# szellmann/icon-ray-tracing

Hardware: AMD Instinct MI355X
Metric: Mray/s + ms/frame at 1024², R2B07 ICON grid, 1/2/4/8 MI355X vs host CPU (higher is better)
Workload: dtype f32; 1 GPU; C3: R2B07 (1,310,720 cells) x 90 levels, 1024x1024, framing camera --camera 0 0 1.4e7 0 0 0 0 1 0 -fovy 60, 8 consecutive progressive frames (accumID) per step, woodcockTrackingWithAccel, default TF; records=3932160, width=1024, height=1024, transfer_function=default, sampler=user, accel=sphere, parallelism=single GPU, frames_per_launch=8, slot_table_bytes=0

## Files before the change

icon-ray-tracing_amd/csrc/irt_context.h:

```cpp
#pragma once

#include <hip/hip_runtime.h>

#include <cmath>
#include <vector>

#include "irt_internal.h"
#include "irt_kernels.h"

int irt_hip_failed(const char *call, hipError_t e, const char *file, int line);

#define IRT_HIP(call)                                                           \
  do {                                                                          \
    hipError_t e_ = (call);                                                     \
    if (e_ != hipSuccess) return irt_hip_failed(#call, e_, __FILE__, __LINE__); \
  } while (0)

struct LaunchSlot {
  hipEvent_t ev0 = nullptr, ev1 = nullptr;
  hipEvent_t evDone = nullptr;
  bool pending = false;
  bool marked = false;
  bool timed = false;
  bool block = false;
  hipStream_t stream = nullptr;
  long long launch = 0;
  size_t numWG = 0;
  long long costsOf = -1;
};

struct irt_context {
  int device = 0;
  hipStream_t stream = nullptr;
  irt_volume_info info{};
  uint32_t n = 0;
  int G = 0;
  uint4 *d_binHdr = nullptr;
  float4 *d_fat = nullptr;
  float4 *d_blocks = nullptr;
  irt::SlotTable slot;
  bool slotAlways = false;
  bool slotLazy = false;
  bool slotTried = false;
  bool slotSparse = false;
  double tfSamples = 0.0;
  double *d_tfStat = nullptr;
  size_t binEntries = 0;
  uint32_t numSph = 0;
  uint32_t numSphRec = 0;
  float *d_sphR = nullptr;
  uint32_t *d_sphOff = nullptr;
  uint2 *d_sphRec = nullptr;
  uint32_t *d_sphBits = nullptr;
  uint32_t *h_wgCounts = nullptr, *dh_wgCounts = nullptr;
  size_t wgCap = 0;
  bool lastBlock = false;
  bool wgCountsOn = true;
  bool statsOff = false;
  int countersProbe = 0;
  uint32_t *d_probeCounts = nullptr;
  size_t probeCap = 0;
  float4 *d_samples = nullptr;
  size_t sampleCap = 0;
  float *d_srgb = nullptr;
  float *d_valueRanges = nullptr;
  float *d_maxOp = nullptr;
  ushort4 *d_rects = nullptr;
  unsigned long long *d_updStat = nullptr;
  hipEvent_t evUpd = nullptr;
  bool updPending = false;
  bool gridBuilt = false;
  uint32_t *d_meta = nullptr;
  float *d_gridVR = nullptr;
  float *d_gridMaxOp = nullptr;
  uint32_t *d_gridBits = nullptr;
  int wG = 0;
  uint32_t *d_wOff = nullptr, *d_wRec = nullptr;
  float4 *d_wBox = nullptr, *d_wTrig = nullptr;
  size_t numMCs = 0;
  float4 *d_lut = nullptr;
  int lutCap = 0;
  int lutSize = 0;
  float tfLo = 0.f, tfHi = 1.f, opScale = 1.f;
  bool tfSet = false;
  static constexpr int kSlots = 32;
  static constexpr int kDoneEvery = 8;
  LaunchSlot ring[kSlots];
  long long launches = 0;
  static constexpr size_t kWgCountsMax = size_t(1) << 18;
  size_t wgCountsMax = kWgCountsMax;
  unsigned long long *d_counters = nullptr;
  unsigned long long *d_counterBuckets = nullptr;
  unsigned long long *h_counters = nullptr;
  unsigned long long *dh_counters = nullptr;
  hipStream_t lastStream = nullptr;
  int timingEvery = 8;
  float lastMs = 0.f;
  double timedMs = 0.0;
  long long timedLaunches = 0;
  irt_render_stats stats{};
  unsigned long long h_last[16] = {};
  irt_render_stats total{};
  long long totalLaunches = 0;
  size_t bytes = 0;
  const irt::VariantForms *forms = irt::forms_of(irt::kDefaultVariant);
  uint32_t *d_schedOrder = nullptr, *d_schedCost = nullptr;
  uint32_t *h_schedCost = nullptr, *h_schedOrder = nullptr;
  uint32_t schedSplit[2] = {0, 0};
  uint32_t lastNumSplit = 0;
  int splitLg = 2;
  float splitFactor = 1.f;
  bool splitFixed = false;
  int schedBuf = 0;
  long long schedSwitch = 0;
  size_t schedCap = 0;
  bool schedOn = false;
  bool schedFixed = false;
  int coopMaxLg = 0;
  int coopRamp = 1;
  int probeExit = 0;
  uint32_t *wgTrace = nullptr;
  bool chainOn = true;
  uint32_t *d_chainFlag = nullptr;
  size_t chainCap = 0;
  uint32_t chainEpoch = 1;
  uint32_t *h_chainFail = nullptr, *dh_chainFail = nullptr;
  long long chainFailLaunches = 0;
  uint32_t chainSpins = 0;
  int chainWithhold = -1;
  float4 *d_frameCams = nullptr;
  float4 *h_frameCams = nullptr;
  size_t frameCamCap = 0;
  irt::VoidCache voidCache;
  uint32_t *d_voidList = nullptr;
  uint32_t *h_voidList = nullptr;
  size_t voidCap = 0;
  long long voidOnDevice = 0;
  bool voidOnDeviceList = false;
  long long lastVoid = 0;
  long long lastWorkgroups = 0;
  irt::RenderPlan lastPlan{};
  bool queueOn = false;
  uint32_t *d_queue = nullptr;
  int numCU = 0;
  int queuePerCU = 0;
  int lastQueueWG = 0;
  int schedPolicy = 2;
  bool schedOrderValid = false;
  bool schedLastApplied = false;
  long long schedApplied = 0;
  long long schedKey[8] = {};
  long long schedSrc = -1;
  long long schedLastCopy = -1000;
  hipEvent_t evSample = nullptr;
  bool samplePending = false;
  hipStream_t sampleStream = nullptr;
  float *d_sampleTab = nullptr, *h_sampleTab = nullptr;
  size_t sampleTabCap = 0;
  hipEvent_t evSampleTab = nullptr;
  bool sampleTabBusy = false;
  std::vector<irt_overlay *> overlays;
  bool building = false;
  size_t expected = 0, received = 0;
  float bottomMin = INFINITY, bottomMax = -INFINITY;
  bool voids = false;
  bool variantFixed = false;
  irt_icon_cell *d_cells = nullptr;
  float4 *d_trig = nullptr;
  irt::VolumeAcc vacc{};
  size_t numRuns = 0;
  irt_icon_cell last{};
  struct Sphere {
    float r;
    uint32_t rec;
    int32_t nl;
  };
  std::vector<Sphere> sph;
  struct TileTable {
    std::vector<int32_t> ids;
    int32_t *dev;
  };
  std::vector<TileTable> tileTables;
};

template <typename T>
int dalloc(irt_context *c, T **p, size_t count) {
  *p = nullptr;
  if (count == 0) count = 1;
  IRT_HIP(hipMalloc((void **)p, count * sizeof(T)));
  c->bytes += count * sizeof(T);
  return IRT_OK;
}

template <typename T>
int upload(irt_context *c, T **p, const T *src, size_t count) {
  int rc = dalloc(c, p, count);
  if (rc) return rc;
  if (count) IRT_HIP(hipMemcpyAsync(*p, src, count * sizeof(T), hipMemcpyHostToDevice, c->stream));
  return IRT_OK;
}

int update_pending(const char *what);
int ensure_grid(irt_context *c);
hipError_t wait_slot(irt_context *c, int i);
int finish_slot(irt_context *c, int i);
int finish_stats(irt_context *c);
int tile_table(irt_context *c, const int32_t *ids, size_t n, int lo, int total, const int32_t **out);
hipError_t wait_samples(irt_context *c);
void free_sample_state(irt_context *c);
void free_overlays(irt_context *c);

namespace irt {
void frame_args(const irt_context *c, const irt_launch_params *lp, uint32_t *fb, irt_vec4f *accum, RenderArgs &A);
void scene_args(const irt_context *c, int mode, RenderArgs &A);
int sample_check(const irt_context *c, int mode, const char *what);
int sample_begin(irt_context *c, hipStream_t s);
int sample_end(irt_context *c, hipStream_t s);
int sample_tab_reserve(irt_context *c, size_t need);
int sample_tab_upload(irt_context *c, size_t need, hipStream_t s);
}
```

icon-ray-tracing_amd/csrc/irt_debug_hooks.hip:

```cpp

#include <hip/hip_runtime.h>
#include <string.h>

#include <algorithm>

#include "icon_rt_hip_debug.h"
#include "irt_context.h"
#include "irt_device.h"

using namespace irt;

namespace {
__global__ void k_debug_math(const float *a, const float *y, const float *x, int n, float *oa,
                             float *ot) {
  const int i = blockIdx.x * blockDim.x + threadIdx.x;
  if (i >= n) return;
  oa[i] = glibc_asinf(a[i]);
  ot[i] = glibc_atan2f(y[i], x[i]);
}
}

extern "C" int irt_debug_device_math(int device, const float *a, const float *y, const float *x,
                                     int n, float *oa, float *ot) {
  if (n <= 0 || !a || !y || !x || !oa || !ot) {
// ... 128 lines not shown

extern "C" int irt_debug_device_srgb(int device, const float *x, uint32_t *out, int n) {
  if (!x || !out || n < 0) {
    set_error("irt_debug_device_srgb: bad argument");
    return IRT_E_INVALID;
  }
  IRT_HIP(hipSetDevice(device));
  float th[256];
  srgb_thresholds(th);
  float *d = nullptr;
  const size_t m = 256 + 2 * (size_t)n;
  IRT_HIP(hipMalloc((void **)&d, m * sizeof(float)));
  hipError_t e = hipMemcpy(d, th, sizeof(th), hipMemcpyHostToDevice);
  e = e == hipSuccess ? hipMemcpy(d + 256, x, n * sizeof(float), hipMemcpyHostToDevice) : e;
  if (e == hipSuccess && n > 0) {
    hipLaunchKernelGGL(k_debug_srgb, dim3((n + 255) / 256), dim3(256), 0, 0, d, d + 256,
                       reinterpret_cast<uint32_t *>(d + 256 + n), n);
    e = hipGetLastError();
  }
  e = e == hipSuccess ? hipMemcpy(out, d + 256 + n, n * sizeof(uint32_t), hipMemcpyDeviceToHost) : e;
  (void)hipFree(d);
  if (e != hipSuccess) {
    set_error("irt_debug_device_srgb: %s", hipGetErrorString(e));
    return IRT_E_HIP;
  }
  return IRT_OK;
}

static int debug_locate(irt_context *c, const float *xyz, int n, int *found, float *value, bool wave) {
  if (!c || !xyz || !found || !value || n < 0) {
    set_error("irt_debug_locate: bad argument");
    return IRT_E_INVALID;
  }
  IRT_HIP(hipSetDevice(c->device));
  RenderArgs A;
  memset(&A, 0, sizeof(A));
  A.numCells = c->n;
  A.G = c->G;
  A.binHdr = c->d_binHdr;
  A.fat = c->d_fat;
  A.blocks = c->d_blocks;
  A.slots = c->slot.slots;
  A.slotBins = c->slot.bins;
  A.slotSubs = c->slot.subs;
  for (int k = 0; k < 3; ++k) A.slotEdge[k] = c->slot.edges[k];
  A.numSph = c->numSph;
  A.sphR = c->d_sphR;
  A.sphOff = c->d_sphOff;
  A.sphRec = c->d_sphRec;
  A.sphBits = c->d_sphBits;
  float *d = nullptr;
  IRT_HIP(hipMalloc((void **)&d, (size_t)std::max(n, 1) * 5 * sizeof(float)));
  hipError_t e = hipMemcpy(d, xyz, (size_t)n * 3 * sizeof(float), hipMemcpyHostToDevice);
  int *dFound = reinterpret_cast<int *>(d + 3 * (size_t)n);
  float *dValue = d + 4 * (size_t)n;
  if (e == hipSuccess) {
    launch_debug_locate(A, d, n, dFound, dValue, 0, wave);
    e = hipGetLastError();
  }
  e = e == hipSuccess ? hipMemcpy(found, dFound, (size_t)n * sizeof(int), hipMemcpyDeviceToHost) : e;
  e = e == hipSuccess ? hipMemcpy(value, dValue, (size_t)n * sizeof(float), hipMemcpyDeviceToHost) : e;
  (void)hipFree(d);
  if (e != hipSuccess) {
    set_error("irt_debug_locate: %s", hipGetErrorString(e));
    return IRT_E_HIP;
  }
  return IRT_OK;
}

extern "C" int irt_debug_locate(irt_context *c, const float *xyz, int n, int *found, float *value) {
  return debug_locate(c, xyz, n, found, value, false);
}

extern "C" int irt_debug_locate_wave(irt_context *c, const float *xyz, int n, int *found, float *value) {
  return debug_locate(c, xyz, n, found, value, true);
}

extern "C" int irt_debug_locate_sampler(irt_context *c, int mode, const float *xyz, int n, int *found,
                                        float *value) {
  if (!c || c->building || n < 0 || (n && (!xyz || !found || !value))) {
    set_error("irt_debug_locate_sampler: bad argument");
    return IRT_E_INVALID;
  }
  if (mode != IRT_MODE_CUBQL && mode != IRT_MODE_TRIANGLES) {
    set_error("irt_debug_locate_sampler: sampler mode %d is neither IRT_MODE_CUBQL nor IRT_MODE_TRIANGLES", mode);
    return IRT_E_INVALID;
  }
  if (c->updPending) return update_pending("irt_debug_locate_sampler");
  if (c->wG == 0 && c->n != 0) {
    set_error("irt_debug_locate_sampler: sampler mode %d needs irt_build_wedge_accel first", mode);
    return IRT_E_INVALID;
  }
  if (n == 0) return IRT_OK;
  IRT_HIP(hipSetDevice(c->device));
  RenderArgs A;
  memset(&A, 0, sizeof(A));
  A.numCells = c->n;
  A.sampler = mode;
  A.wG = c->wG;
  A.wOff = c->d_wOff;
  A.wRec = c->d_wRec;
  A.wBox = c->d_wBox;
  A.wTrig = c->d_wTrig;
  A.blocks = c->d_blocks;
  float *d = nullptr;
  IRT_HIP(hipMalloc((void **)&d, (size_t)n * 5 * sizeof(float)));
  hipError_t e = hipMemcpy(d, xyz, (size_t)n * 3 * sizeof(float), hipMemcpyHostToDevice);
  int *dFound = reinterpret_cast<int *>(d + 3 * (size_t)n);
  float *dValue = d + 4 * (size_t)n;
  if (e == hipSuccess) {
    launch_debug_locate_sampler(A, d, n, dFound, dValue, 0);
    e = hipGetLastError();
  }
  e = e == hipSuccess ? hipMemcpy(found, dFound, (size_t)n * sizeof(int), hipMemcpyDeviceToHost) : e;
  e = e == hipSuccess ? hipMemcpy(value, dValue, (size_t)n * sizeof(float), hipMemcpyDeviceToHost) : e;
  (void)hipFree(d);
  if (e != hipSuccess) {
    set_error("irt_debug_locate_sampler: %s", hipGetErrorString(e));
    return IRT_E_HIP;
  }
  return IRT_OK;
}

extern "C" int irt_debug_sched(irt_context *c, int *policy, int *lastApplied, long long *applied) {
  if (!c || !policy || !lastApplied || !applied) {
    set_error("irt_debug_sched: null argument");
    return IRT_E_INVALID;
  }
  *policy = c->schedOn ? c->schedPolicy : 0;
  *lastApplied = c->schedLastApplied ? 1 : 0;
  *applied = c->schedApplied;
  return IRT_OK;
}

extern "C" int irt_debug_counters(irt_context *c, unsigned long long *out16) {
  if (!c || !out16) {
    set_error("irt_debug_counters: null argument");
    return IRT_E_INVALID;
  }
  int rc = finish_stats(c);
  if (rc) return rc;
  memcpy(out16, c->h_last, 16 * sizeof(unsigned long long));
  return IRT_OK;
}

extern "C" int irt_debug_default_variant(void) { return kDefaultVariant; }
extern "C" int irt_debug_slot_use(const irt_context *c, double *tfSamples) {
  if (!c) return -1;
  if (tfSamples) *tfSamples = c->tfSamples;
  return c->slot.slots && (c->slotAlways || c->slotSparse) ? 1 : 0;
}

extern "C" long long irt_debug_void_use(const irt_context *c) { return c ? c->lastVoid : -1; }
extern "C" long long irt_debug_last_workgroups(const irt_context *c) { return c ? c->lastWorkgroups : -1; }

extern "C" int irt_debug_context_array(const irt_context *c, int which, void *dst, size_t capacity,
                                       size_t *bytes) {
  if (!c || !bytes || c->building) {
    set_error("irt_debug_context_array: null argument or context not built");
    return IRT_E_INVALID;
  }
  const void *src = nullptr;
  size_t n = 0;
  switch (which) {
    case IRT_DEBUG_ARRAY_BIN_HDR: src = c->d_binHdr; n = (size_t)6 * c->G * c->G * kBinHdrWords * 4; break;
    case IRT_DEBUG_ARRAY_FAT: src = c->d_fat; n = c->binEntries * kFatStride4 * 16; break;
    case IRT_DEBUG_ARRAY_BLOCKS: src = c->d_blocks; n = (size_t)c->n * kBlk4 * 16; break;
    case IRT_DEBUG_ARRAY_SPH_R: src = c->d_sphR; n = (size_t)c->numSph * 4; break;
    case IRT_DEBUG_ARRAY_SPH_OFF: src = c->d_sphOff; n = c->numSph ? ((size_t)c->numSph + 1) * 4 : 4; break;
    case IRT_DEBUG_ARRAY_SPH_REC: src = c->d_sphRec; n = (size_t)c->numSphRec * 8; break;
    case IRT_DEBUG_ARRAY_SPH_BITS: src = c->d_sphBits; n = (size_t)kSphBitWords * 4; break;
    case IRT_DEBUG_ARRAY_SLOTS: src = c->slot.slots; n = c->slot.bytes; break;
    case IRT_DEBUG_ARRAY_GRID_BITS: src = c->d_gridBits; n = c->gridBuilt ? (size_t)kGridBitWords * 4 : 0; break;
    default:
      set_error("irt_debug_context_array: unknown array %d", which);
      return IRT_E_INVALID;
  }
  *bytes = n;
  if (dst && capacity >= n && n) {
    IRT_HIP(hipSetDevice(c->device));
    IRT_HIP(hipStreamSynchronize(c->stream));
    IRT_HIP(hipMemcpy(dst, src, n, hipMemcpyDeviceToHost));
  }
  return IRT_OK;
}

extern "C" int irt_debug_get_variant(const irt_context *c) { return c ? c->forms->variant : -1; }

extern "C" int irt_debug_variants(int *out, int capacity) { return render_variants(out, capacity); }

extern "C" int irt_debug_set_queue(irt_context *c, int on) {
  if (!c) {
    set_error("irt_debug_set_queue: null context");
    return IRT_E_INVALID;
  }
  if (on && !render_queue_compiled()) {
    set_error("irt_debug_set_queue: persistent launches are compiled into the A/B library only "
              "(make VARIANTS=all, libicon_rt_hip_all.so)");
    return IRT_E_INVALID;
  }
  c->queueOn = on != 0;
  return IRT_OK;
}

extern "C" int irt_debug_set_wg_trace(irt_context *c, uint32_t *trace) {
  if (!c) {
    set_error("irt_debug_set_wg_trace: null context");
    return IRT_E_INVALID;
  }
  c->wgTrace = trace;
  return IRT_OK;
}

extern "C" long long irt_debug_launch_workgroups(const irt_context *c, int numTiles, int numFrames) {
  if (!c || numTiles < 0 || numFrames < 1) {
    set_error("irt_debug_launch_workgroups: bad argument");
    return -1;
  }
  return irt_debug_variant_workgroups(c->forms->variant, c->schedOn ? 1 : 0, numTiles, numFrames);
}

extern "C" long long irt_debug_variant_workgroups(int variant, int sched, int numTiles, int numFrames) {
  if (numTiles < 0 || numFrames < 1) {
    set_error("irt_debug_variant_workgroups: bad argument");
    return -1;
  }
  const int per = 256 / render_forms(variant).plain.threads;
  const size_t extra = sched && numFrames == 1 && per == 4 ? (size_t)kMaxSplit : 0;
  return (long long)((size_t)numTiles * 16 * per * numFrames + extra);
}

namespace {
int plan_out(const RenderPlan &P, int out[5]) {
  out[0] = P.form.id;
  out[1] = P.form.threads;
  out[2] = (int)P.grid.x;
  out[3] = (int)P.grid.y;
  out[4] = P.accumBlocks;
  return IRT_OK;
}
}

extern "C" int irt_debug_plan(int variant, int sampler, int accelMode, int flags, int numTiles, int numFrames,
                              uint32_t numSplit, uint32_t voidLive, uint32_t voidRow, int queueWG, int out[5]) {
  const VariantForms *F = forms_of(variant);
  if (!F || !out || numTiles < 0 || numFrames < 1) {
    set_error("irt_debug_plan: variant %d not compiled, or bad argument", variant);
    return IRT_E_INVALID;
  }
  alignas(16) static uint32_t set[4];
  RenderArgs A;
  memset(&A, 0, sizeof(A));
  A.sampler = sampler;
  A.accelMode = accelMode;
  A.numTiles = numTiles;
  A.numSamples = numFrames;
  A.numSplit = numSplit;
  A.voidLive = voidLive;
  A.voidRow = voidRow;
  if (flags & IRT_DEBUG_PLAN_SLOTS) A.slots = reinterpret_cast<const float4 *>(set);
  if (flags & IRT_DEBUG_PLAN_VOID_BITS) A.voidBits = set;
  if (flags & IRT_DEBUG_PLAN_VOID_LIST) A.voidList = set;
  if (flags & IRT_DEBUG_PLAN_QUEUE) A.queue = set;
  A.chain = (flags & IRT_DEBUG_PLAN_CHAIN) ? 1 : 0;
  return plan_out(plan_render(*F, A, queueWG), out);
}

extern "C" int irt_debug_last_plan(const irt_context *c, int out[5]) {
  if (!c || !out) {
    set_error("irt_debug_last_plan: null argument");
    return IRT_E_INVALID;
  }
  return plan_out(c->lastPlan, out);
}

extern "C" int irt_debug_sched_split(const irt_context *c, int *numSplit, int *splitLg) {
  if (!c || !numSplit || !splitLg) {
    set_error("irt_debug_sched_split: null argument");
    return IRT_E_INVALID;
  }
  *numSplit = (int)c->lastNumSplit;
  *splitLg = c->splitLg;
  return IRT_OK;
}

extern "C" int irt_debug_set_chain(irt_context *c, int on) {
  if (!c) {
    set_error("irt_debug_set_chain: null context");
    return IRT_E_INVALID;
  }
  c->chainOn = on != 0;
  return IRT_OK;
}

extern "C" int irt_debug_chain_errors(irt_context *c) {
  if (!c) {
    set_error("irt_debug_chain_errors: null context");
    return -1;
  }
  for (long long j = c->launches - irt_context::kSlots; j < c->launches; ++j) {
    if (j < 0) continue;
    const int rc = finish_slot(c, (int)(j % irt_context::kSlots));
    if (rc && rc != IRT_E_CHAIN) return -1;
  }
  return (int)c->chainFailLaunches;
}
// ... 25 lines not shown
```

icon-ray-tracing_amd/csrc/irt_device.h:

```cpp
#pragma once

#include <hip/hip_runtime.h>
#include <stdint.h>

#include "irt_common.h"
#include "irt_kernels.h"

#define IRT_FLT_MAX 3.402823466e+38f

namespace irt {

struct Ray {
  float ox, oy, oz, tmin, dx, dy, dz, tmax;
};

struct Counts {
  uint32_t inBox, locate, found, cand;
  uint32_t steps, deg, rounds;
  uint32_t hops, locRounds, candHist[4];
};

__device__ __forceinline__ int opaque_u(int v) {
  v = __builtin_amdgcn_readfirstlane(v);
  asm volatile("" : "+s"(v));
  return v;
}
__device__ __forceinline__ float opaque_u(float v) { return __builtin_bit_cast(float, opaque_u(__builtin_bit_cast(int, v))); }
__device__ __forceinline__ float dot3(float ax, float ay, float az, float bx, float by, float bz) {
  return ax * bx + ay * by + az * bz;
}

__device__ __forceinline__ bool recip_ok(float b) {
  const float ab = __builtin_fabsf(b);
  return ab >= 0x1p-100f && ab <= 0x1p100f;
}
__device__ __forceinline__ double recip_d(float b) {
  const double r0 = (double)__builtin_amdgcn_rcpf(b);
  const double e = __builtin_fma(-(double)b, r0, 1.0);
  return __builtin_fma(r0, __builtin_fma(e, e, e), r0);
}
__device__ __forceinline__ float div_recip(float a, double r) { return (float)((double)a * r); }

__device__ __forceinline__ bool box_test(const Ray &r, const RenderArgs &A, float &t0, float &t1) {
  float lx, ly, lz, hx, hy, hz;
  if (recip_ok(r.dx) && recip_ok(r.dy) && recip_ok(r.dz)) {
    const double rx = recip_d(r.dx), ry = recip_d(r.dy), rz = recip_d(r.dz);
    lx = div_recip(A.bmin.x - r.ox, rx);
    ly = div_recip(A.bmin.y - r.oy, ry);
    lz = div_recip(A.bmin.z - r.oz, rz);
    hx = div_recip(A.bmax.x - r.ox, rx);
    hy = div_recip(A.bmax.y - r.oy, ry);
    hz = div_recip(A.bmax.z - r.oz, rz);
  } else {
    lx = (A.bmin.x - r.ox) / r.dx, ly = (A.bmin.y - r.oy) / r.dy, lz = (A.bmin.z - r.oz) / r.dz;
    hx = (A.bmax.x - r.ox) / r.dx, hy = (A.bmax.y - r.oy) / r.dy, hz = (A.bmax.z - r.oz) / r.dz;
  }
  const float nx = fminf(lx, hx), ny = fminf(ly, hy), nz = fminf(lz, hz);
  const float fx = fmaxf(lx, hx), fy = fmaxf(ly, hy), fz = fmaxf(lz, hz);
  t0 = fmaxf(r.tmin, fmaxf(fmaxf(nx, ny), nz));
  t1 = fminf(r.tmax, fminf(fminf(fx, fy), fz));
  return t0 < t1;
}

__device__ __forceinline__ bool intersect_sphere(const Ray &r, float radius, float &tnear, float &tfar) {
  const float A = dot3(r.dx, r.dy, r.dz, r.dx, r.dy, r.dz);
  const float B = dot3(r.dx, r.dy, r.dz, r.ox, r.oy, r.oz) * 2.f;
  const float C = dot3(r.ox, r.oy, r.oz, r.ox, r.oy, r.oz) - radius * radius;
  float d = B * B - 4.f * A * C;
  if (d < 0.f) return false;
  d = sqrtf(d);
  const float q = B < 0.f ? -0.5f * (B - d) : -0.5f * (B + d);
  const float t1 = q / A;
  const float t2 = C / q;
  tnear = fminf(t1, t2);
  tfar = fmaxf(t1, t2);
  return true;
}
__device__ __forceinline__ void intersect_spheres(const Ray &r, float radiusA, float radiusB, bool &hitA,
                                                  float &nearA, float &farA, bool &hitB, float &nearB,
                                                  float &farB) {
  const float A = dot3(r.dx, r.dy, r.dz, r.dx, r.dy, r.dz);
  const float B = dot3(r.dx, r.dy, r.dz, r.ox, r.oy, r.oz) * 2.f;
  const float OO = dot3(r.ox, r.oy, r.oz, r.ox, r.oy, r.oz);
  const bool okA = recip_ok(A);
  const double rA = okA ? recip_d(A) : 0.0;
  auto one = [&](float radius, float &tnear, float &tfar) {
    const float C = OO - radius * radius;
    float d = B * B - 4.f * A * C;
    if (d < 0.f) return false;
    d = sqrtf(d);
    const float q = B < 0.f ? -0.5f * (B - d) : -0.5f * (B + d);
    float t1, t2;
    if (okA && recip_ok(q)) {
      t1 = div_recip(q, rA);
      t2 = div_recip(C, recip_d(q));
    } else {
      t1 = q / A;
      t2 = C / q;
    }
    tnear = fminf(t1, t2);
    tfar = fmaxf(t1, t2);
    return true;
  };
  hitA = one(radiusA, nearA, farA);
  hitB = one(radiusB, nearB, farB);
}

__device__ __forceinline__ int project_axis(float s, float lo, float hi, int dim) {
  return f2i_x86((s - lo) / (hi - lo) * (float)(dim - 1));
}

__device__ __forceinline__ float div_uniform(float a, double invB) {
  return (float)((double)a * invB);
}
__device__ __forceinline__ int project_axis_inv(float s, float lo, double invSize, int dim) {
  return f2i_x86(div_uniform(s - lo, invSize) * (float)(opaque_u(dim) - 1));
}

__device__ __forceinline__ int wrap_coord(int c, int d) {
  if ((unsigned)c < (unsigned)d) return c;
  if (c >= -d && c < 2 * d) return c < 0 ? c + d : c - d;
  d = opaque_u(d);
  const int m = c % d;
  return m < 0 ? m + d : m;
}

__device__ __forceinline__ void to_spherical(float x, float y, float z, float &r, float &lat,
                                             float &lon) {
  r = sqrtf(dot3(x, y, z, x, y, z));
  lat = glibc_asinf(z / r);
  lon = glibc_atan2f(y, x);
}

constexpr float kLatErr = 1.0e-6f;
constexpr float kLonErr = 2.0e-6f;

__device__ __forceinline__ float fast_asin(float x) {
  const float a = __builtin_fabsf(x);
  const bool big = a >= 0.5f;
  const float t = big ? (1.f - a) * 0.5f : a * a;
  const float s = big ? __builtin_amdgcn_sqrtf(t) : a;
  const float p = t * __builtin_fmaf(
                          t, __builtin_fmaf(t, __builtin_fmaf(t, __builtin_fmaf(t, 4.216630880e-2f, 2.417951451e-2f),
                                                                4.547037598e-2f),
                                            7.495297643e-2f),
                          1.666675248e-1f);
  const float r = __builtin_fmaf(s, p, s);
  const float v = big ? __builtin_fmaf(-2.f, r, 1.57079637050628662109375f) : r;
  return __builtin_copysignf(v, x);
}
__device__ __forceinline__ float fast_atan(float q) {
  const bool big = q > 2.414213562373095f, mid = q > 0.4142135623730950f;
  const float num = big ? -1.f : (mid ? q - 1.f : q);
  const float den = big ? q : (mid ? q + 1.f : 1.f);
  const float x = num * __builtin_amdgcn_rcpf(den);
  const float base = big ? 1.57079637050628662109375f : (mid ? 0.785398185253143310546875f : 0.f);
  const float z = x * x;
  const float p = __builtin_fmaf(
      __builtin_fmaf(__builtin_fmaf(__builtin_fmaf(8.05374449538e-2f, z, -1.38776856032e-1f), z, 1.99777106478e-1f),
                     z, -3.33329491539e-1f),
      z * x, x);
  return base + p;
}
__device__ __forceinline__ bool fast_atan2(float y, float x, float &lon) {
  const float ax = __builtin_fabsf(x), ay = __builtin_fabsf(y);
  const float q = ay * __builtin_amdgcn_rcpf(ax);
  const bool ok = ax >= 0x1p-100f && ax <= 0x1p100f && ay >= 0x1p-100f && ay <= 0x1p100f && q >= 0x1p-58f &&
                  q <= 0x1p58f;
  const float z = fast_atan(q);
  const float pi = 3.1415927410e+00f, pi_lo = -8.7422776573e-08f;
  lon = y < 0.f ? (x < 0.f ? (z - pi_lo) - pi : -z) : (x < 0.f ? pi - (z - pi_lo) : z);
  return ok;
}
__device__ __forceinline__ bool cell_certified(float v, float err, float lo, double invSize, int dim, int &cell) {
  const int c0 = project_axis_inv(v - err, lo, invSize, dim), c1 = project_axis_inv(v + err, lo, invSize, dim);
  cell = c0;
  return c0 == c1 && v == v;
}
__device__ __forceinline__ int sign_certified(float a, float b, float err) {
  const float d = b - a, m = 2.f * err + 2.4e-7f;
  return d > m ? 1 : (-d > m ? -1 : 0);
}

__device__ __forceinline__ uint32_t make_8bit(float f) {
  return (uint32_t)fminf(255.f, fmaxf(0.f, (float)f2i_x86(f * 256.f)));
}

__device__ __forceinline__ uint32_t srgb_byte(const float *th, float x) {
  const float over = th[0];
  const float s = x <= 0.0031308f
                      ? 12.92f * x
                      : 1.055f * __builtin_amdgcn_exp2f(__builtin_amdgcn_logf(x) * (1.f / 2.4f)) - 0.055f;
  int b = (int)fminf(255.f, fmaxf(0.f, s * 256.f));
  const float up = th[b < 255 ? b + 1 : 255], at = th[b];
  if (b < 255 && up <= x) {
    ++b;
    while (b < 255 && th[b + 1] <= x) ++b;
  } else if (b > 0 && !(at <= x)) {
    --b;
    while (b > 0 && !(th[b] <= x)) --b;
  }
  return x >= over ? 0u : (uint32_t)b;
}

}
```

icon-ray-tracing_amd/csrc/irt_internal.h:

```cpp
#pragma once

#include <stddef.h>
#include <stdint.h>

#include <string>
#include <vector>

#include "icon_rt_hip.h"
#include "irt_common.h"

namespace irt {

void set_error(const char *fmt, ...) __attribute__((format(printf, 1, 2)));
void clear_error();


struct HostScene {
  size_t n = 0;
  irt_volume_info info{};
  std::vector<float> hv;
  std::vector<float> trig;
  std::vector<float> planes;
  std::vector<float> rng;
  std::vector<uint32_t> meta;
  std::vector<float> blocks;
  int G = 0;
  std::vector<uint32_t> offsets;
  std::vector<uint32_t> entryRec;
  std::vector<uint32_t> entrySub;
  std::vector<uint32_t> binHdr;
  std::vector<float> fat;
  size_t binEntries = 0;
  std::vector<float> sphR;
  std::vector<uint32_t> sphOff, sphRec, sphBits;
};

int build_bins(HostScene &S, int threads);
int locator_resolution(size_t numRuns);
float record_value_host(const HostScene &s, uint32_t rec, uint32_t path, float r);
int locate_bins_host(const HostScene &s, float px, float py, float pz, float &value,
                     uint32_t *record, uint32_t *tested);

int build_scene(const irt_icon_cell *cells, size_t n, HostScene &out, int threads = 0);


void compute_volume_info(const irt_icon_cell *cells, size_t n, irt_volume_info &info);
struct VolumeAcc {
  float vlo[3], vhi[3], slo[3], shi[3], dlo, dhi;
  size_t n;
};
void corner_trig(const irt_icon_cell &c, float *t12);
void cell_bounds(const irt_icon_cell &c, const float *t12, float lo[3], float hi[3]);
void volume_acc_init(VolumeAcc &a);
void volume_acc_add(VolumeAcc &a, const irt_icon_cell &c, const float blo[3], const float bhi[3]);
void volume_acc_merge(VolumeAcc &a, const VolumeAcc &b);
void volume_acc_finish(const VolumeAcc &a, irt_volume_info &info);

const std::vector<float> &logf_table();

void srgb_thresholds(float th[256]);

int sample_host(const HostScene &s, uint32_t rec, float px, float py, float pz, float &value);
int locate_host(const HostScene &s, float px, float py, float pz, float &value,
                uint32_t *record);

struct WedgeScene {
  int G = 0;
  std::vector<float> trig;
  std::vector<float> box;
  std::vector<uint32_t> offsets;
  std::vector<uint32_t> recs;
};
int build_wedges(const irt_icon_cell *cells, size_t n, WedgeScene &W, int threads = 0);
bool wedge_locate_host(const WedgeScene &W, const irt_icon_cell *cells, float px, float py,
                       float pz, float &value);
bool triangle_locate_host(const WedgeScene &W, const irt_icon_cell *cells, float px, float py,
                          float pz, float &value, uint32_t *record);

int default_threads();

inline bool update_range_ok(size_t first, size_t n, size_t numCells) {
  return first <= numCells && n <= numCells - first;
}

constexpr uint64_t kSampleMaxPoints = uint64_t(1) << 36;
void latlon_trig(const float *lat, int numLat, const float *lon, int numLon, float *latCS, float *lonCS);
int latlon_args(const char *what, const float *lat, int numLat, const float *lon, int numLon,
                const float *radius, int numLevels, size_t *total);

int levels_args(const char *what, const float *radius, int numLevels);
void levels_order(const float *radius, int numLevels, float *sorted, int32_t *index);

int column_weights(const char *what, const float *weight, int numLevels);
int column_levels_args(const char *what, const float *radius, const float *weight, int numLevels);

constexpr size_t kSectionTrigSplit = 1 << 14;
void section_trig(const float *lat, const float *lon, int numColumns, float *tab);
int section_args(const char *what, const float *lat, const float *lon, int numColumns, const float *radius,
                 int numLevels, size_t *total);

int hist_args(const char *what, irt_box1f valueRange, int numBins, int weighting, const float *bandEdges,
              int numBands);

uint32_t sched_order(const uint32_t *cost, int numBlocks, int tilesX, int tileStride, int policy,
                     int splitLg, float splitFactor, int numCU, bool wavewg, size_t cap,
                     uint32_t maxSplit, uint32_t *out);

struct VoidRequest {
  float cam[12];
  float bmin[3], bmax[3];
  float rOuter, rInner;
  int W, H, tileBegin, tileStride, numTiles;
  int raygen, accelMode, mode;
  const int32_t *tileList;
};
inline VoidRequest void_request(const irt_launch_params &lp, const irt_volume_info &info, int W, int H, int tileBegin,
                                int tileStride, int numTiles, const int32_t *tileList) {
  VoidRequest q;
  const irt_vec3f *cam[4] = {&lp.org, &lp.dir_00, &lp.dir_du, &lp.dir_dv};
  for (int k = 0; k < 4; ++k) {
    q.cam[3 * k] = cam[k]->x;
    q.cam[3 * k + 1] = cam[k]->y;
    q.cam[3 * k + 2] = cam[k]->z;
  }
  q.bmin[0] = info.bounds.lower.x, q.bmin[1] = info.bounds.lower.y, q.bmin[2] = info.bounds.lower.z;
  q.bmax[0] = info.bounds.upper.x, q.bmax[1] = info.bounds.upper.y, q.bmax[2] = info.bounds.upper.z;
  q.rOuter = info.sphericalBounds.upper.x;
  q.rInner = info.sphericalBounds.lower.x;
  q.W = W, q.H = H, q.tileBegin = tileBegin, q.tileStride = tileStride, q.numTiles = numTiles;
  q.raygen = lp.raygen, q.accelMode = lp.accelMode, q.mode = lp.mode;
  q.tileList = tileList;
  return q;
}
inline size_t void_words(int numTiles) { return ((size_t)(numTiles > 0 ? numTiles : 0) * 64 + 31) / 32; }
struct VoidLists {
  std::vector<uint32_t> items;
  uint32_t live = 0, count = 0;
};
constexpr uint32_t kVoidEmpty = ~0u;
inline uint32_t void_row(uint32_t count, int F) {
  return (uint32_t)((((uint64_t)count + (uint64_t)F - 1) / (uint64_t)F + 7) & ~(uint64_t)7);
}
uint32_t void_packets(const VoidRequest &q, uint32_t *bits, VoidLists *lists = nullptr);
struct VoidCache {
  std::vector<unsigned char> key;
  std::vector<uint32_t> bits;
  VoidLists lists;
  uint32_t count = 0;
  bool keyed = false, valid = false;
  long long generation = 0;
  bool lookup(const VoidRequest &q, bool defer = false);
};

int synth_open(int rootN, int bisections, int levels, float topHeight, float noise, uint32_t seed,
               float terrainHeight,
               void **gen, size_t *total);
void synth_fill(const void *gen, size_t first, size_t count, irt_icon_cell *out);
void synth_close(void *gen);

}
```

icon-ray-tracing_amd/csrc/irt_kernels.h:

```cpp
#pragma once

#include <hip/hip_runtime.h>
#include <stdint.h>

#include "icon_rt_hip.h"

namespace irt {

struct RenderArgs {
  float3 org, dir00, du, dv;
  int accumID;
  float accumW;
  float3 amb;
  float ambRad;
  float unitDistance;
  int raygen;
  float3 bmin, bmax;
  int3 dims;
  float3 sbLo, sbHi;
  const float *maxOp;
  int accelMode;
  const float *gridMaxOp;
  const uint32_t *gridBits;
  int sampler;
  int wG;
  const uint32_t *wOff, *wRec;
  const float4 *wBox;
  const float4 *wTrig;
  float tfLo, tfHi, opacityScale;
  double invTf;
  double invSb[3];
  const float4 *lut;
  int lutSize;
  uint32_t numCells;
  int G;
  const float *srgbTh;
  int W, H;
  uint32_t *fb;
  float4 *accum;
  int packed;
  int tileBegin, tileStride, numTiles, tilesX;
  const int32_t *tileList;
  unsigned long long *counters;
  unsigned long long *counterBuckets;
  const uint4 *binHdr;
  const float4 *fat;
  const float4 *blocks;
  uint32_t numSph;
  const float *sphR;
  const uint32_t *sphOff;
  const uint2 *sphRec;
  const uint32_t *sphBits;
  uint32_t *wgCounts;
  int numSamples;
  const uint32_t *schedOrder;
  uint32_t *schedCost;
  float4 *sampleBuf;
  int coopMaxLg;
  int coopRamp;
  int probeExit;
  uint32_t *queue;
  uint32_t numPackets;
  int chain;
  const float4 *frameCams;
  uint32_t chainEpoch;
  uint32_t *chainFlag;
  uint32_t *chainFail;
  uint32_t chainSpins;
  int chainWithhold;

  uint32_t *wgTrace;
  const uint32_t *splitList;
  const uint32_t *splitMask;
  uint32_t numSplit;
  const float4 *slots;
  float slotEdge[3];
  int slotBins;
  int slotSubs;
  const uint32_t *voidBits;
  const uint32_t *voidList;
  uint32_t voidLive, voidRow, voidCount;
};
constexpr int kQueueLine = 32;
constexpr uint32_t kChainSpinsDefault = 1u << 20;
constexpr int kQueueWords = 9 * kQueueLine;

constexpr int kCnt = 8;

enum : int {
  OPT_WEDGE = 16384,
  OPT_GRID = 8192,
  OPT_STATS = 32768,
  OPT_SERIAL = 65536,
  OPT_SCAN1 = 131072,
  OPT_TIMING = 524288,
  OPT_WAVEWG = 4194304,
  OPT_LEAN = 2097152,
  OPT_QUEUE = 16777216,
  OPT_FASTSPH = 33554432,
  OPT_SPLIT = 8,
  OPT_DPPSCAN = 32,
  OPT_DMATAB = 67108864,
  OPT_NOMISS = 262144,
  OPT_VOIDLOC = 1073741824,
  OPT_NOVOIDRUN = 2,
  OPT_NOHOLESKIP = 4,
  OPT_SLOT = 128,
  OPT_VOID = 16,
  OPT_VLIST = 64,
};
constexpr int OPT_MONO = 4096;
constexpr int kDefaultVariant = 73405728;
constexpr int kNoMissBit = OPT_NOMISS;
constexpr uint32_t kMaxSplit = 4096;
constexpr int kVoidLocBit = OPT_VOIDLOC;
constexpr int kSamplerVariant = ((kDefaultVariant & ~OPT_MONO) & ~(0xF00 | OPT_WAVEWG | OPT_LEAN)) | OPT_WEDGE;
inline int scene_variant(bool holes) { return holes ? kDefaultVariant | kVoidLocBit : kDefaultVariant | kNoMissBit; }

typedef void (*RenderKernel)(RenderArgs);
struct KernelForm {
  RenderKernel fn;
  int id;
  int threads;
};
struct VariantForms {
  int variant;
  KernelForm plain, split, slot, slotSplit, voidBits, voidList, queue;
  KernelForm grid, wedge, wedgeGrid;
};
const VariantForms *forms_of(int variant);
inline const VariantForms &render_forms(int variant) {
  const VariantForms *f = forms_of(variant);
  return f ? *f : *forms_of(kDefaultVariant);
}
int render_variants(int *out, int cap);
bool render_queue_compiled();

inline bool render_sphere_path(const RenderArgs &A) {
  return A.sampler == IRT_MODE_USER_GEOM && A.accelMode != IRT_ACCEL_GRID;
}
inline bool render_split_ok(const VariantForms &F, const RenderArgs &A) {
  return render_sphere_path(A) && F.split.fn != nullptr;
}
inline bool render_void_ok(const VariantForms &F, const RenderArgs &A) {
  return render_sphere_path(A) && F.voidBits.fn != nullptr && !A.slots && !A.queue && !A.numSplit && !A.schedOrder;
}
inline bool render_queue_ok(const VariantForms &F, const RenderArgs &A) {
  return render_sphere_path(A) && F.queue.fn != nullptr;
}
int render_queue_wgs(const VariantForms &F, int numCU, int numBlocks);

struct RenderPlan {
  KernelForm form;
  dim3 grid;
  size_t workgroups;
  int accumBlocks;
};
RenderPlan plan_render(const VariantForms &F, const RenderArgs &A, int queueWG);
void launch_render(const RenderArgs &A, const RenderPlan &plan, hipStream_t s);
void prewarm_render(const VariantForms &F, hipStream_t s);
void launch_debug_locate(const RenderArgs &A, const float *xyz, int n, int *found, float *value,
                         hipStream_t s, bool wave);
void launch_debug_locate_sampler(const RenderArgs &A, const float *xyz, int n, int *found, float *value,
                                 hipStream_t s);
void launch_shell_init(float *valueRanges, size_t numMCs, hipStream_t s);
void launch_shell_build(const irt_icon_cell *cells, size_t n, int3 dims, float3 lo, float3 hi,
                        float *valueRanges, ushort4 *rects, hipStream_t s);
void launch_value_scatter(const float *d_values, size_t first, size_t n, float4 *blocks, hipStream_t s);
void launch_shell_rebuild(const float4 *blocks, const uint32_t *meta, const ushort4 *rects, size_t n,
                          int3 dims, float *valueRanges, unsigned long long *stat, hipStream_t s);
void launch_grid_build(const float4 *blocks, const uint32_t *meta, const float4 *trig, size_t n,
                       float3 lo, float3 hi, float *valueRanges, hipStream_t s);
void launch_grid_bits(const float *maxOp, uint32_t *bits, hipStream_t s);
void launch_accept_stat(const float *valueRanges, const float *maxOp, size_t numMCs, const float4 *lut, int size,
                        float lo, float hi, double *out, hipStream_t s);
void launch_max_opacities(const float *valueRanges, size_t numMCs, const float4 *lut, int size,
                          float lo, float hi, float *maxOp, hipStream_t s);
void launch_clear(uint32_t *fb, float4 *accum, size_t n, hipStream_t s);
constexpr int kCounterBuckets = 64;
void launch_stats_out(const unsigned long long *cur, unsigned long long *host,
                      unsigned long long *next, unsigned long long *buckets, hipStream_t s);
void launch_copy_u32(const uint32_t *src, uint32_t *dst, size_t n, hipStream_t s);
struct DeviceScene {
  float4 *blocks = nullptr;
  uint32_t *meta = nullptr;
  uint4 *binHdr = nullptr;
  float4 *fat = nullptr;
  size_t entries = 0, binEntries = 0, bigCells = 0, bytes = 0;
};
int build_scene_device(const irt_icon_cell *d_cells, const float4 *d_trig, size_t n, size_t numRuns,
                       int G, hipStream_t s, DeviceScene &out);
struct SlotTable {
  float4 *slots = nullptr;
  int bins = 0;
  int subs = 0;
  float edges[3] = {0.f, 0.f, 0.f};
  size_t bytes = 0;
  const char *skipped = nullptr;
};
constexpr size_t kSlotAutoHdrBytes = (size_t)256 << 20;
int build_slots_device(const uint32_t *hdr, const float4 *fat, uint32_t numCells, size_t maxBytes, int subs,
                       size_t autoBytes, hipStream_t s, SlotTable &out);
void launch_unpack(const uint32_t *gathered, int numRanks, int maxTiles, int W, int H,
                   uint32_t *fb, hipStream_t s, const int32_t *table = nullptr);

}
```

icon-ray-tracing_amd/csrc/irt_launch.hip:

```cpp

#include <hip/hip_runtime.h>
#include <string.h>

#include <algorithm>
#include <initializer_list>

#include "irt_context.h"

using namespace irt;


int tile_table(irt_context *c, const int32_t *ids, size_t n, int lo, int total, const int32_t **out) {
  for (size_t k = 0; k < n; ++k)
    if (ids[k] < lo || ids[k] >= total) {
      set_error("tile id %d at %zu outside [%d, %d)", ids[k], k, lo, total);
      return IRT_E_INVALID;
    }
  for (auto &t : c->tileTables)
    if (t.ids.size() == n && std::equal(t.ids.begin(), t.ids.end(), ids)) {
      *out = t.dev;
      return IRT_OK;
    }
  if (c->tileTables.size() >= 64) {
    IRT_HIP(hipDeviceSynchronize());
// ... 340 lines not shown
                         I.sphericalBounds.upper.z - I.sphericalBounds.lower.z};
    for (int k = 0; k < 3; ++k) A.invSb[k] = 1.0 / (double)sz[k];
  }
  A.coopMaxLg = c->coopMaxLg;
  A.coopRamp = c->coopRamp;
  A.probeExit = c->probeExit;
  A.wgTrace = c->wgTrace;
  A.numCells = c->n;
  A.G = c->G;
  A.counters = c->d_counters + 16 * L.slot;
  A.binHdr = c->d_binHdr;
  A.fat = c->d_fat;
  A.blocks = c->d_blocks;
  A.slots = c->slotAlways || c->slotSparse ? c->slot.slots : nullptr;
  A.slotBins = c->slot.bins;
  A.slotSubs = c->slot.subs;
  for (int k = 0; k < 3; ++k) A.slotEdge[k] = c->slot.edges[k];
  A.numSph = c->numSph;
  A.sphR = c->d_sphR;
  A.sphOff = c->d_sphOff;
  A.sphRec = c->d_sphRec;
  A.sphBits = c->d_sphBits;
}

int claim_slot(irt_context *c, Launch &L) {
  for (int i = 0; i < kSlots; ++i)
    if (c->ring[i].pending && c->h_chainFail[i]) {
      int rc = finish_slot(c, i);
      if (rc) return rc;
    }
  if (c->ring[L.slot].pending) {
    int rc = finish_slot(c, L.slot);
    if (rc) return rc;
  }
  hipStream_t s = L.s;
  if (c->launches > 0 && s != c->lastStream) {
    const int prev = (int)((c->launches - 1) % kSlots);
    if (c->ring[prev].pending) {
      const hipEvent_t e = done_event(c, prev);
      if (e) IRT_HIP(hipStreamWaitEvent(s, e, 0));
    }
  }
  c->lastStream = s;
  return IRT_OK;
}

void decide_queue(irt_context *c, int numFrames, Launch &L) {
  RenderArgs &A = L.A;
  L.queued = c->queueOn && L.numTiles > 0 && whole_kernel(c) && render_queue_ok(*c->forms, A);
  L.queueWG = 0;
  if (!L.queued) return;
  A.queue = c->d_queue + (size_t)kQueueWords * L.slot;
  A.numPackets = (uint32_t)L.numTiles * 64u * (uint32_t)numFrames;
  L.queueWG = c->queuePerCU > 0 ? std::min(c->queuePerCU * c->numCU, L.numTiles * 16 * numFrames)
                                : render_queue_wgs(*c->forms, c->numCU, L.numTiles * 16 * numFrames);
  c->lastQueueWG = L.queueWG;
}

int decide_sched(irt_context *c, const irt_launch_params *lp, const RenderRequest &r, Launch &L) {
  RenderArgs &A = L.A;
  const int numBlocks = L.numTiles * 16;
  L.copyCosts = false;
  if (!(c->schedOn && r.numFrames == 1 && numBlocks > 0 && !A.tileList && !L.queued)) return IRT_OK;
  int rc = sched_prepare(c, numBlocks, r.W, r.H, r.packed, r.tileBegin, r.tileStride, L.numTiles, lp,
                         render_split_ok(*c->forms, A), L.s);
  if (rc) return rc;
  const uint32_t *ob = c->d_schedOrder + (size_t)c->schedBuf * sched_stride(c->schedCap);
  A.schedOrder = c->schedOrderValid ? ob : nullptr;
  if (c->schedOrderValid && c->schedSplit[c->schedBuf] && render_split_ok(*c->forms, A) && whole_kernel(c)) {
    A.splitList = ob + c->schedCap;
    A.splitMask = ob + c->schedCap + kMaxSplit;
    A.numSplit = c->schedSplit[c->schedBuf];
  }
  L.copyCosts = c->launches - c->schedLastCopy >= 8;
  if (L.copyCosts) {
    uint32_t *dh = nullptr;
    IRT_HIP(hipHostGetDevicePointer((void **)&dh, c->h_schedCost + (size_t)L.slot * 4 * c->schedCap, 0));
    A.schedCost = dh;
  } else {
    A.schedCost = c->d_schedCost;
  }
  return IRT_OK;
}

void decide_chain(const irt_context *c, const RenderRequest &r, Launch &L) {
  RenderArgs &A = L.A;
  const uint64_t outPixels = r.packed ? (uint64_t)L.numTiles * 4096u : (uint64_t)r.W * (uint64_t)r.H;
  A.chain = r.numFrames > 1 && chain_capable(c, L.queued) && outPixels * 16u <= 0x7FFFFFFFull ? 1 : 0;
  A.numSamples = r.numFrames;
}

int choose_counters(irt_context *c, Launch &L) {
  RenderArgs &A = L.A;
  const bool useWG = c->wgCountsOn && L.numWG <= c->wgCountsMax;
  if (useWG && L.numWG > c->wgCap) {
    bool failed = false;
    int rc = grow(c, Retire::Slots, L.s, &c->wgCap, L.numWG,
                  {{(void **)&c->h_wgCounts, [](size_t n) { return n * kSlots * kCnt * sizeof(uint32_t); }, true}},
                  &failed);
    if (rc) return rc;
    if (!failed && hipHostGetDevicePointer((void **)&c->dh_wgCounts, c->h_wgCounts, 0) != hipSuccess) {
      (void)hipGetLastError();
      (void)hipHostFree(c->h_wgCounts);
      c->h_wgCounts = nullptr;
      c->wgCap = 0;
      failed = true;
    }
    if (failed) {
      c->dh_wgCounts = nullptr;
      c->wgCountsOn = false;
    }
  }
  A.wgCounts = useWG && c->wgCountsOn ? c->dh_wgCounts + (size_t)L.slot * c->wgCap * kCnt : nullptr;
  if (c->countersProbe == 1 || c->statsOff) {
    A.wgCounts = nullptr;
    if (!stats_variant(c)) A.counters = nullptr;
  } else if (c->countersProbe == 2) {
    if (L.numWG > c->probeCap) {
      int rc = grow(c, Retire::Stream, L.s, &c->probeCap, L.numWG,
                    {{(void **)&c->d_probeCounts, [](size_t n) { return n * kCnt * sizeof(uint32_t); }, false}}, nullptr);
      if (rc) return rc;
    }
    A.wgCounts = c->d_probeCounts;
  }
  return IRT_OK;
}

int setup_chain(irt_context *c, int numFrames, Launch &L) {
  RenderArgs &A = L.A;
  if (!A.chain) return IRT_OK;
  const size_t words = (size_t)L.numTiles * 16 * 4;
  if (words > c->chainCap || c->chainEpoch > 0xF0000000u - (uint32_t)numFrames) {
    if (words > c->chainCap) {
      int rc = grow(c, Retire::SlotsThenStream, L.s, &c->chainCap, words,
                    {{(void **)&c->d_chainFlag, [](size_t n) { return n * sizeof(uint32_t); }, false}}, nullptr);
      if (rc) return rc;
    }
    IRT_HIP(hipMemsetAsync(c->d_chainFlag, 0, c->chainCap * sizeof(uint32_t), L.s));
    c->chainEpoch = 1;
  }
  A.chainFlag = c->d_chainFlag;
  c->h_chainFail[L.slot] = 0;
  A.chainFail = c->dh_chainFail + L.slot;
  A.chainSpins = c->chainSpins ? c->chainSpins : kChainSpinsDefault;
  A.chainWithhold = c->chainWithhold;
  A.chainEpoch = c->chainEpoch;
  c->chainEpoch += (uint32_t)numFrames;
  return IRT_OK;
}

int prepare_void(irt_context *c, const irt_launch_params *lp, const RenderRequest &r, Launch &L) {
  RenderArgs &A = L.A;
  c->lastVoid = 0;
  if (!(A.chain && !r.seq && r.numFrames > 1 && r.numFrames <= 65535 && L.numTiles > 0 &&
        c->chainWithhold < 0 && c->probeExit == 0 && !stats_variant(c) &&
        lp->raygen == IRT_RAYGEN_WITH_ACCEL && lp->accelMode == IRT_ACCEL_SPHERE &&
        render_void_ok(*c->forms, A)))
    return IRT_OK;
  c->voidCache.lookup(void_request(*lp, c->info, r.W, r.H, r.tileBegin, r.tileStride, L.numTiles, r.tileList), true);
  const VoidLists &vl = c->voidCache.lists;
  if (!c->voidCache.count || vl.items.empty()) return IRT_OK;
  const bool list = c->forms->voidList.fn != nullptr &&
                    (size_t)vl.live + void_row(vl.count, r.numFrames) < (size_t)L.numTiles * 64;
  const size_t words = list ? vl.items.size() : void_words(L.numTiles);
  if (words > c->voidCap) {
    int rc = grow(c, Retire::SlotsThenStream, L.s, &c->voidCap, words,
                  {{(void **)&c->d_voidList, [](size_t n) { return n * sizeof(uint32_t); }, false},
                   {(void **)&c->h_voidList, [](size_t n) { return kSlots * n * sizeof(uint32_t); }, true}},
                  nullptr);
    c->voidOnDevice = 0;
    if (rc) return rc;
  }
  if (c->voidOnDevice != c->voidCache.generation || c->voidOnDeviceList != list) {
    uint32_t *h = c->h_voidList + (size_t)L.slot * c->voidCap;
    memcpy(h, list ? vl.items.data() : c->voidCache.bits.data(), words * sizeof(uint32_t));
    c->voidOnDeviceList = list;
    IRT_HIP(hipMemcpyAsync(c->d_voidList, h, words * sizeof(uint32_t), hipMemcpyHostToDevice, L.s));
    c->voidOnDevice = c->voidCache.generation;
  }
  if (list) {
    A.voidList = c->d_voidList;
    A.voidLive = vl.live;
    A.voidRow = void_row(vl.count, r.numFrames);
    A.voidCount = vl.count;
  } else {
    A.voidBits = c->d_voidList;
  }
  c->lastVoid = c->voidCache.count;
  return IRT_OK;
}

int stage_sequence(irt_context *c, const RenderRequest &r, Launch &L) {
  RenderArgs &A = L.A;
  if (!r.seq) return IRT_OK;
  if (!A.chain) {
    set_error("irt_render_sequence: needs chained frames (a cooperative variant, IRT_CHAIN on)");
    return IRT_E_INVALID;
  }
  const int numFrames = r.numFrames;
  if ((size_t)numFrames > c->frameCamCap) {
    int rc = grow(c, Retire::SlotsThenStream, L.s, &c->frameCamCap, (size_t)numFrames,
                  {{(void **)&c->d_frameCams, [](size_t n) { return n * 4 * sizeof(float4); }, false},
                   {(void **)&c->h_frameCams, [](size_t n) { return kSlots * n * 4 * sizeof(float4); }, true}},
                  nullptr);
    if (rc) return rc;
  }
  float4 *h = c->h_frameCams + (size_t)L.slot * c->frameCamCap * 4;
  for (int k = 0; k < numFrames; ++k) {
    const irt_launch_params &q = r.seq[k];
    h[4 * k + 0] = make_float4(q.org.x, q.org.y, q.org.z, __builtin_bit_cast(float, q.accumID));
    h[4 * k + 1] = make_float4(q.dir_00.x, q.dir_00.y, q.dir_00.z, 0.f);
    h[4 * k + 2] = make_float4(q.dir_du.x, q.dir_du.y, q.dir_du.z, 0.f);
    h[4 * k + 3] = make_float4(q.dir_dv.x, q.dir_dv.y, q.dir_dv.z, 0.f);
  }
  IRT_HIP(hipMemcpyAsync(c->d_frameCams, h, (size_t)numFrames * 4 * sizeof(float4), hipMemcpyHostToDevice, L.s));
  A.frameCams = c->d_frameCams;
  return IRT_OK;
}

int ensure_samples(irt_context *c, int numFrames, Launch &L) {
  if (numFrames > 1 && !L.A.chain) {
    const size_t need = (size_t)L.numTiles * 4096 * (size_t)numFrames;
    if (need > c->sampleCap) {
      int rc = grow(c, Retire::Stream, L.s, &c->sampleCap, need,
                    {{(void **)&c->d_samples, [](size_t n) { return n * sizeof(float4); }, false}}, nullptr);
      if (rc) return rc;
    }
  }
  L.A.sampleBuf = c->d_samples;
  return IRT_OK;
}

int launch_and_commit(irt_context *c, Launch &L) {
  RenderArgs &A = L.A;
  hipStream_t s = L.s;
  LaunchSlot &r = c->ring[L.slot];
  c->schedLastApplied = A.schedOrder != nullptr;
  c->lastNumSplit = A.numSplit;
  c->lastWorkgroups = L.numTiles > 0 ? (long long)L.numWG : 0;
  c->lastPlan = L.plan;
  c->schedApplied += c->schedLastApplied ? 1 : 0;
  A.counterBuckets = A.counters && !A.wgCounts ? c->d_counterBuckets + (size_t)L.slot * kCounterBuckets * 8 : nullptr;
  const bool block = A.counters && (!A.wgCounts || stats_variant(c));
  if (block && !c->lastBlock) IRT_HIP(hipMemsetAsync(A.counters, 0, 16 * sizeof(unsigned long long), s));
  r.timed = c->launches % c->timingEvery == 0;
  if (r.timed) IRT_HIP(hipEventRecord(r.ev0, s));
  if (L.numTiles > 0) launch_render(A, L.plan, s);
  IRT_HIP(hipGetLastError());
  if (r.timed) IRT_HIP(hipEventRecord(r.ev1, s));
  if (block) {
    launch_stats_out(A.counters, c->dh_counters + 16 * L.slot,
                     c->d_counters + 16 * ((c->launches + 1) % kSlots), A.counterBuckets, s);
    IRT_HIP(hipGetLastError());
  }
  r.block = block;
  c->lastBlock = block;
  r.numWG = (A.wgCounts && c->countersProbe == 0 && !c->statsOff && L.numTiles > 0) ? L.numWG : 0;
  r.costsOf = -1;
  if (L.copyCosts) {
    r.costsOf = c->launches;
    c->schedLastCopy = c->launches;
  }
  r.stream = s;
  r.launch = c->launches;
  r.marked = c->launches % irt_context::kDoneEvery == irt_context::kDoneEvery - 1 || L.copyCosts;
  if (r.marked) IRT_HIP(hipEventRecord(r.evDone, s));
  r.pending = true;
  ++c->launches;
  return IRT_OK;
}

int render_impl(irt_context *c, const irt_launch_params *lp, const RenderRequest &r, uint32_t *fb,
                irt_vec4f *accum, int *numTilesOut, void *stream) {
  int rc = validate(c, lp, r, fb, accum);
  if (rc) return rc;
  IRT_HIP(hipSetDevice(c->device));
  if (lp->accelMode == IRT_ACCEL_GRID && (rc = ensure_grid(c))) return rc;
  Launch L;
  memset(&L.A, 0, sizeof(L.A));
  L.s = (hipStream_t)stream;
  L.slot = (int)(c->launches % kSlots);
  if ((rc = resolve_tiles(c, r, L))) return rc;
  if (numTilesOut) *numTilesOut = L.numTiles;
  fill_args(c, lp, fb, accum, L);
  if ((rc = claim_slot(c, L))) return rc;
  decide_queue(c, r.numFrames, L);
  if ((rc = decide_sched(c, lp, r, L))) return rc;
  decide_chain(c, r, L);
  if ((rc = prepare_void(c, lp, r, L))) return rc;
  L.plan = plan_render(*c->forms, L.A, L.queueWG);
  L.numWG = L.plan.workgroups;
  if ((rc = choose_counters(c, L)) || (rc = setup_chain(c, r.numFrames, L)) ||
      (rc = stage_sequence(c, r, L)) ||
      (rc = ensure_samples(c, r.numFrames, L)))
    return rc;
  return launch_and_commit(c, L);
}

RenderRequest whole_frame(int W, int H, int numFrames) { return {W, H, 0, 0, 1, nullptr, 0, numFrames, nullptr}; }
RenderRequest strided_tiles(int W, int H, int tileBegin, int tileStride, int numFrames) {
  return {W, H, 1, tileBegin, tileStride, nullptr, 0, numFrames, nullptr};
}
RenderRequest listed_tiles(int W, int H, const int32_t *tiles, int numTiles, int numFrames) {
  static const int32_t none = 0;
  return {W, H, 1, 0, 1, numTiles > 0 ? tiles : &none, numTiles, numFrames, nullptr};
}

int render_sequence(irt_context *c, const irt_launch_params *lps, int numFrames, int W, int H,
                    const int32_t *tiles, int numTiles, uint32_t *fb, irt_vec4f *accum, void *stream) {
  if (!c || !lps || numFrames < 1 || numTiles < 0 || (numTiles > 0 && !tiles)) {
    set_error("irt_render_sequence: bad argument");
    return IRT_E_INVALID;
  }
  const size_t fixed = offsetof(irt_launch_params, ambientColor);
  for (int k = 1; k < numFrames; ++k)
    if (memcmp((const char *)&lps[k] + fixed, (const char *)&lps[0] + fixed, sizeof(irt_launch_params) - fixed)) {
      set_error("irt_render_sequence: frame %d differs from frame 0 in more than the camera and accumID", k);
      return IRT_E_INVALID;
    }
  const bool chainable = chain_capable(c, c->queueOn);
  RenderRequest r = tiles ? listed_tiles(W, H, tiles, numTiles, 1) : whole_frame(W, H, 1);
  if (numFrames == 1 || !chainable) {
    for (int k = 0; k < numFrames; ++k) {
      int rc = render_impl(c, &lps[k], r, fb, accum, nullptr, stream);
      if (rc) return rc;
    }
    return IRT_OK;
  }
  r.numFrames = numFrames;
  r.seq = lps;
  return render_impl(c, &lps[0], r, fb, accum, nullptr, stream);
}

}


extern "C" {

int irt_clear_frame(irt_context *c, uint32_t *fb, irt_vec4f *accum, size_t n, void *stream) {
  if (!c) {
    set_error("irt_clear_frame: null context");
// ... 147 lines not shown
```

icon-ray-tracing_amd/csrc/irt_raygen.h:

```cpp
#pragma once

#include "irt_tracer.h"

namespace irt {

struct Pixel {
  int x, y;
  size_t outIdx;
  bool active;
};
__device__ __forceinline__ Pixel pixel_of(const RenderArgs &A, uint32_t blkU, int tid) {
  const int blk = (int)__builtin_amdgcn_readfirstlane(blkU);
  const int k = blk >> 4, sub = blk & 15;
  const int wave = tid >> 6, lane = tid & 63;
  const int lx = ((sub & 3) << 4) | ((wave & 1) << 3) | (lane & 7);
  const int ly = ((sub >> 2) << 4) | ((wave >> 1) << 3) | (lane >> 3);
  const int tileId = !A.tileList ? A.tileBegin + k * A.tileStride : (k < A.numTiles ? (int)scalar_word(A.tileList, (uint32_t)k) : 0);
  const int tx = tileId % A.tilesX, ty = tileId / A.tilesX;
  Pixel p;
  p.x = tx * 64 + lx;
  p.y = ty * 64 + ly;
  p.active = k < A.numTiles && p.x < A.W && p.y < A.H;
  p.outIdx = A.packed ? (size_t)k * 4096 + ly * 64 + lx : (size_t)p.x + (size_t)A.W * p.y;
  return p;
// ... 283 lines not shown
                                             int tid, int accumID, float4 *sampleOut) {
  uint32_t st;
  float dx, dy, dz;
  gen_ray(A, accumID, px.x, px.y, st, dx, dy, dz);
  const Ray ray = {A.org.x, A.org.y, A.org.z, 0.f, dx, dy, dz, 1e10f};
  float t0, t1;
  if (!box_test(ray, A, t0, t1)) {
    if (sampleOut) *sampleOut = make_float4(0.f, 0.f, 0.f, kNoSample);
    return;
  }
  T.count(1);
  float cr = 0.f, cg = 0.f, cb = 0.f, alpha = 0.f;
  const bool ae = A.raygen == 1;
  float rlo0 = t0, rhi0 = t1, rlo1 = __builtin_inff(), rhi1 = -__builtin_inff();
  int numRanges = 1;
  if (!ae) {
    float st1 = 0.f, st2 = 0.f, st3 = 0.f, st4 = 0.f;
    const bool s1 = intersect_sphere(ray, A.sbHi.x, st1, st4);
    const bool s2 = intersect_sphere(ray, A.sbLo.x, st2, st3);
    numRanges = 0;
    if ((s1 || s2) && !(st4 < t0)) {
      numRanges = 2;
      if (s1 && !s2) {
        rlo0 = st1; rhi0 = st4;
      } else if (t0 < st2) {
        rlo0 = st1; rhi0 = st2;
        rlo1 = st3; rhi1 = st4;
      } else {
        rlo0 = st3; rhi0 = st4;
      }
    }
  }
  if constexpr ((OPT & OPT_GRID) != 0) {
    if (!ae) {
      render_grid(A, T, ray, t0, t1, st, cr, cg, cb, alpha);
      numRanges = 0;
    }
  }
  const float sceneEPS = A.sbLo.x * 1e-6f;
  for (int i = 0; i < numRanges; ++i) {
    const float lower = i ? rlo1 : rlo0, upper = i ? rhi1 : rhi0;
    if (upper <= lower) break;
    const bool lastRange = ae || i == 1 || rhi1 <= rlo1;
    int cx = 0, cy = 0, cz = 0;
    if (!ae) {
      const float e1 = lower + sceneEPS;
      float r1, la1, lo1;
      to_spherical(ray.ox + ray.dx * e1, ray.oy + ray.dy * e1, ray.oz + ray.dz * e1, r1, la1, lo1);
      cx = project_axis(r1, A.sbLo.x, A.sbHi.x, A.dims.x);
      cy = project_axis(la1, A.sbLo.y, A.sbHi.y, A.dims.y);
      cz = project_axis(lo1, A.sbLo.z, A.sbHi.z, A.dims.z);
      if (!lastRange) lds_st16(&s_entry[tid], make_float4(r1, la1, lo1, 0.f));
    }
    const float tnx = upper, tny = 0.f, tnz = 0.f;
    float t = lower;
    for (int iter = 0; iter < (1 << 22); ++iter) {
      float tt1 = IRT_FLT_MAX;
      if (ae) {
        tt1 = upper;
      } else {
        if (tnx < tt1 && tnx >= t) tt1 = tnx;
        if (tny < tt1 && tny >= t) tt1 = tny;
        if (tnz < tt1 && tnz >= t) tt1 = tnz;
      }
      const bool zeroLen = tt1 == t;
      if (zeroLen && lastRange) break;
      if constexpr ((OPT & OPT_STATS) != 0) T.cnt.deg += zeroLen ? 1u : 0u;
      float maj = 1.f;
      if (!ae) {
        const uint32_t leaf = (uint32_t)wrap_coord(cz, A.dims.z) * (uint32_t)A.dims.x * (uint32_t)A.dims.y +
                              (uint32_t)wrap_coord(cy, A.dims.y) * (uint32_t)A.dims.x +
                              (uint32_t)wrap_coord(cx, A.dims.x);
        maj = A.maxOp[leaf];
      }
      bool fast = false;
      if (zeroLen) {
        const float q = maj / A.unitDistance;
        const uint32_t nx = lcg_next(st);
        if (!(maj > 0.f)) {
          fast = true;
        } else if (q > 0.f && q <= 1e30f && (nx & 0x00FFFFFFu) != 0u) {
          st = nx;
          fast = true;
        }
      }
      if (!fast) {
        float4 s = make_float4(0.f, 0.f, 0.f, 0.f);
        const bool counted = !zeroLen;
        const float tw = T.woodcock(ray.dx, ray.dy, ray.dz, t, tt1, st, maj, s, counted);
        if (!zeroLen && (ae || (tw > t && tw < tt1))) {
          cr = s.x * A.amb.x * A.ambRad;
          cg = s.y * A.amb.y * A.ambRad;
          cb = s.z * A.amb.z * A.ambRad;
          alpha = s.w > 0.f ? 1.f : 0.f;
          i = 2;
          break;
        }
      }
      if (lastRange) break;
      int4 dd;
      if (iter == 0) {
        const float e2 = upper - sceneEPS;
        float r2, la2, lo2;
        to_spherical(ray.ox + ray.dx * e2, ray.oy + ray.dy * e2, ray.oz + ray.dz * e2, r2, la2, lo2);
        const float4 en = lds_ld16(&s_entry[tid]);
        const float r1 = en.x, la1 = en.y, lo1 = en.z;
        const int sx = r1 < r2 ? 1 : -1, sy = la1 < la2 ? 1 : -1, sz = lo1 < lo2 ? 1 : -1;
        dd.x = (sx > 0 ? 1 : 0) | (sy > 0 ? 2 : 0) | (sz > 0 ? 4 : 0);
        dd.y = (int)((uint32_t)project_axis(r2, A.sbLo.x, A.sbHi.x, A.dims.x) + (uint32_t)sx);
        dd.z = (int)((uint32_t)project_axis(la2, A.sbLo.y, A.sbHi.y, A.dims.y) + (uint32_t)sy);
        dd.w = (int)((uint32_t)project_axis(lo2, A.sbLo.z, A.sbHi.z, A.dims.z) + (uint32_t)sz);
        s_dda[tid] = dd;
      } else {
        dd = s_dda[tid];
      }
      const float t_closest = fminf(fminf(tnx, tny), tnz);
      if (tnx == t_closest) {
        cx += (dd.x & 1) ? 1 : -1;
        if (cx == dd.y) break;
      }
      if (tny == t_closest) {
        cy += (dd.x & 2) ? 1 : -1;
        if (cy == dd.z) break;
      }
      if (tnz == t_closest) {
        cz += (dd.x & 4) ? 1 : -1;
        if (cz == dd.w) break;
      }
      t = t_closest;
    }
  }
  if (sampleOut)
    *sampleOut = make_float4(cr, cg, cb, alpha);
  else
    write_pixel(A, px.outIdx, cr, cg, cb, alpha, s_th);
}

__device__ __forceinline__ bool spherical_fast(const RenderArgs &A, float x, float y, float z, float &r, float &la,
                                               float &lo, int &cy, int &cz) {
  r = sqrtf(dot3(x, y, z, x, y, z));
  la = fast_asin(z / r);
  const bool okLon = fast_atan2(y, x, lo);
  const bool okY = cell_certified(la, kLatErr, A.sbLo.y, A.invSb[1], A.dims.y, cy);
  const bool okZ = cell_certified(lo, kLonErr, A.sbLo.z, A.invSb[2], A.dims.z, cz);
  return okY && okZ && okLon;
}


template <int OPT>
__device__ __forceinline__ void render_pixel_coop(const RenderArgs &A, Tracer<OPT> &T, const Pixel &px,
                                                  const float *s_th, int4 *s_dda, float4 *s_entry,
                                                  float4 *s_acc, CoopWave &W, ScanWave *SW, const uint2 *jmp,
                                                  int tid, int accumID, uint32_t blk, int pwave, int frame,
                                                  int partSel = -1) {
  constexpr bool kRecompute = ((OPT >> 8) & 15) >= 5;
  const int ptid = pwave * 64 + (tid & 63);
  const int wbase = __builtin_amdgcn_readfirstlane(tid) & ~63;
  auto tid_late = [&]() { return kRecompute ? (opaque_u(wbase) | (int)__lane_id()) : tid; };
  auto ptid_late = [&]() {
    if constexpr (!kRecompute) return ptid;
    int lane = (int)__lane_id();
    asm volatile("" : "+v"(lane));
    if (partSel >= 0) {
      const int ps = opaque_u(partSel), pn = 64 >> (ps & 255);
      lane = ((ps >> 8) * pn) | (lane & (pn - 1));
    }
    return (opaque_u(pwave) << 6) | lane;
  };
  const bool toSample = A.numSamples > 1 && !A.chain;
  const bool chainLate = A.chain && frame > 0;
  uint32_t chainSeen = 0u;
  if (chainLate)
    chainSeen = __hip_atomic_load(A.chainFlag + (size_t)blk * 4u + (uint32_t)pwave, __ATOMIC_RELAXED,
                                  __HIP_MEMORY_SCOPE_AGENT);
  float4 *const slot0 = kRecompute || !toSample
                            ? nullptr
                            : A.sampleBuf + (size_t)frame * A.numTiles * 4096u + (size_t)blk * 256u + (size_t)ptid;
  auto sample_slot = [&]() {
    if constexpr (!kRecompute) return slot0;
    return A.sampleBuf + (size_t)opaque_u(frame) * opaque_u(A.numTiles) * 4096u + (size_t)opaque_u((int)blk) * 256u +
           (size_t)ptid_late();
  };
  enum : int { kRange, kLeaf, kWait, kDone, kGrid, kGridNext };
  constexpr bool kFastSph = (OPT & OPT_FASTSPH) != 0;
  constexpr bool grid = (OPT & OPT_GRID) != 0;
  const bool ae = A.raygen == 1;
  uint32_t st = 0;
  float dx = 1.f, dy = 1.f, dz = 1.f;
  float rlo0 = 0.f, rhi0 = 0.f, rlo1 = __builtin_inff(), rhi1 = -__builtin_inff();
  int numRanges = 0, phase = kDone;
  bool inBox = false;
  float t0box = 0.f, t1box = 0.f;
  if (px.active) {
    gen_ray(A, accumID, px.x, px.y, st, dx, dy, dz, frame);
    const float3 O = cam_org(A, frame);
    const Ray ray = {O.x, O.y, O.z, 0.f, dx, dy, dz, 1e10f};
    float t0, t1;
    const bool boxHit = box_test(ray, A, t0, t1);
#ifdef IRT_PROBE_BUILD
    if (A.probeExit == 30) {
#pragma nounroll
      for (int k = 0; k < 50; ++k) asm volatile("v_nop\n v_nop\n v_nop\n v_nop" ::: "memory");
    }
#endif
    if (A.probeExit == 3) {
      if (boxHit && t0 == -1.2345f) A.fb[0] = 0u;
      return;
    }
    if (boxHit) {
      inBox = true;
      phase = kRange;
      t0box = t0;
      t1box = t1;
      if (!toSample && !chainLate && (OPT & OPT_LEAN) == 0)
        __builtin_amdgcn_global_load_lds((const void *)(A.accum + px.outIdx),
                                         (__attribute__((address_space(3))) void *)(s_acc + (tid & ~63)),
                                         16, 0, kRecompute ? 2 : 0);
      rlo0 = t0;
      rhi0 = t1;
      numRanges = 1;
      if (!ae) {
        float st1 = 0.f, st2 = 0.f, st3 = 0.f, st4 = 0.f;
        bool s1, s2;
        intersect_spheres(ray, A.sbHi.x, A.sbLo.x, s1, st1, st4, s2, st2, st3);
        numRanges = 0;
        if ((s1 || s2) && !(st4 < t0)) {
          numRanges = 2;
          if (s1 && !s2) {
            rlo0 = st1; rhi0 = st4;
          } else if (t0 < st2) {
            rlo0 = st1; rhi0 = st2;
            rlo1 = st3; rhi1 = st4;
          } else {
            rlo0 = st3; rhi0 = st4;
          }
        }
      }
    } else if (toSample) {
      *sample_slot() = make_float4(0.f, 0.f, 0.f, kNoSample);
    }
  }
  const bool chainReady = !chainLate || __builtin_amdgcn_readfirstlane(chainSeen) == A.chainEpoch + (uint32_t)frame;
  if ((OPT & OPT_LEAN) == 0 && chainLate && chainReady && inBox)
    __builtin_amdgcn_global_load_lds((const void *)(A.accum + px.outIdx),
                                     (__attribute__((address_space(3))) void *)(s_acc + (tid & ~63)), 16, 0, 16);
  int gcx = 0, gcy = 0, gcz = 0, gsteps = 0, gdirs = 0;
  float gtnx = 0.f, gtny = 0.f, gtnz = 0.f, gdx = 0.f, gdy = 0.f, gdz = 0.f, gtmax = 0.f, grtmin = 0.f,
        gtc0 = 0.f, gtc1 = 0.f;
  if constexpr (grid) {
    if (phase == kRange && !ae) {
      const float rtmin = t0box, rtmax = t1box;
      const int D = kGridDim;
      const float3 O = cam_org(A, frame);
      const float ox = O.x + rtmin * dx, oy = O.y + rtmin * dy, oz = O.z + rtmin * dz;
      gtmax = rtmax - rtmin;
      grtmin = rtmin;
      const float rx = 1.f / dx, ry = 1.f / dy, rz = 1.f / dz;
      const float lx = (A.bmin.x - ox) * rx, ly = (A.bmin.y - oy) * ry, lz = (A.bmin.z - oz) * rz;
      const float hx = (A.bmax.x - ox) * rx, hy = (A.bmax.y - oy) * ry, hz = (A.bmax.z - oz) * rz;
      float nx = fminf(lx, hx), ny = fminf(ly, hy), nz = fminf(lz, hz);
      const float fx = fmaxf(lx, hx), fy = fmaxf(ly, hy), fz = fmaxf(lz, hz);
      if (dx == 0.f) nx = IRT_FLT_MAX;
      if (dy == 0.f) ny = IRT_FLT_MAX;
      if (dz == 0.f) nz = IRT_FLT_MAX;
      gcx = project_on_grid(ox, A.bmin.x, A.bmax.x, D);
      gcy = project_on_grid(oy, A.bmin.y, A.bmax.y, D);
      gcz = project_on_grid(oz, A.bmin.z, A.bmax.z, D);
      gdx = fmaxf(0.f, (fx - nx) / (float)D);
      gdy = fmaxf(0.f, (fy - ny) / (float)D);
      gdz = fmaxf(0.f, (fz - nz) / (float)D);
      gdirs = (dx > 0.f ? 1 : 0) | (dy > 0.f ? 2 : 0) | (dz > 0.f ? 4 : 0);
      gtnx = dx > 0.f ? nx + (float)(gcx + 1) * gdx : nx + (float)(D - gcx) * gdx;
      gtny = dy > 0.f ? ny + (float)(gcy + 1) * gdy : ny + (float)(D - gcy) * gdy;
      gtnz = dz > 0.f ? nz + (float)(gcz + 1) * gdz : nz + (float)(D - gcz) * gdz;
      phase = kGrid;
    }
  }
  auto sceneEPS = [&]() {
    const RenderArgs &SA = fresh_args();
    return opaque_u(SA.sbLo.x) * 1e-6f;
  };
  int i = 0, iter = 0, cx = 0, cy = 0, cz = 0;
  float t = 0.f, upper = 0.f, tt1 = 0.f, maj = 0.f;
  bool lastRange = true, zeroLen = false, hit = false;
  bool miss = false;
  bool first = true;
  auto next_leaf = [&]() {
    const RenderArgs &SA = fresh_args();
    if (lastRange) {
      ++i;
      phase = kRange;
      return;
    }
    const float tnx = upper, tny = 0.f, tnz = 0.f;
    int4 dd;
    if (iter == 0) {
      const float e2 = upper - sceneEPS();
      float r2, la2, lo2;
      int cy2 = 0, cz2 = 0;
      bool ok2 = false;
      const float3 O = cam_org(SA, frame);
      if constexpr (kFastSph)
        ok2 = spherical_fast(A, O.x + dx * e2, O.y + dy * e2, O.z + dz * e2, r2, la2, lo2, cy2, cz2);
      else
        to_spherical(O.x + dx * e2, O.y + dy * e2, O.z + dz * e2, r2, la2, lo2);
      const float4 en = lds_ld16(&s_entry[tid_late()]);
      const float r1 = en.x;
      const int sx = r1 < r2 ? 1 : -1;
      int sy, sz;
      if constexpr (!kFastSph) {
        sy = en.y < la2 ? 1 : -1;
        sz = en.z < lo2 ? 1 : -1;
        cy2 = project_axis_inv(la2, SA.sbLo.y, SA.invSb[1], SA.dims.y);
        cz2 = project_axis_inv(lo2, SA.sbLo.z, SA.invSb[2], SA.dims.z);
      } else {
        sy = sign_certified(en.y, la2, kLatErr);
        sz = sign_certified(en.z, lo2, kLonErr);
      }
      if (kFastSph && (!ok2 || sy == 0 || sz == 0)) {
        float la1 = 0.f, lo1 = 0.f;
#pragma nounroll
        for (int k = 0; k < 2; ++k) {
          const float e = k == 0 ? en.w + sceneEPS() : upper - sceneEPS();
          float rr, la, lo;
          to_spherical(O.x + dx * e, O.y + dy * e, O.z + dz * e, rr, la, lo);
          if (k == 0) {
            la1 = la;
            lo1 = lo;
          } else {
            la2 = la;
            lo2 = lo;
          }
        }
        sy = la1 < la2 ? 1 : -1;
        sz = lo1 < lo2 ? 1 : -1;
        cy2 = project_axis_inv(la2, SA.sbLo.y, SA.invSb[1], SA.dims.y);
        cz2 = project_axis_inv(lo2, SA.sbLo.z, SA.invSb[2], SA.dims.z);
      }
      dd.x = (sx > 0 ? 1 : 0) | (sy > 0 ? 2 : 0) | (sz > 0 ? 4 : 0);
      dd.y = (int)((uint32_t)project_axis_inv(r2, SA.sbLo.x, SA.invSb[0], SA.dims.x) + (uint32_t)sx);
      dd.z = (int)((uint32_t)cy2 + (uint32_t)sy);
      dd.w = (int)((uint32_t)cz2 + (uint32_t)sz);
      lds_st16(&s_entry[tid_late()], __builtin_bit_cast(float4, dd));
    } else {
      dd = __builtin_bit_cast(int4, lds_ld16(&s_entry[tid_late()]));
    }
    const float t_closest = fminf(fminf(tnx, tny), tnz);
    bool stop = false;
    if (tnx == t_closest) {
      cx += (dd.x & 1) ? 1 : -1;
      stop = cx == dd.y;
    }
    if (!stop && tny == t_closest) {
      cy += (dd.x & 2) ? 1 : -1;
      stop = cy == dd.z;
    }
    if (!stop && tnz == t_closest) {
      cz += (dd.x & 4) ? 1 : -1;
      stop = cz == dd.w;
    }
    t = t_closest;
    if (stop || ++iter >= (1 << 22)) {
      ++i;
      phase = kRange;
    } else {
      phase = kLeaf;
    }
  };
  while (true) {
    if constexpr (grid) {
      const int D = kGridDim;
      constexpr int NB = kGridDim / kGridBlock;
      while (phase == kGrid || phase == kGridNext) {
        if (phase == kGridNext) {
          const float tmn = fminf(fminf(gtnx, gtny), gtnz);
          bool out = false;
          if (gtnx == tmn) {
            gtnx += gdx;
            gcx += (gdirs & 1) ? 1 : -1;
            out = gcx == ((gdirs & 1) ? D : -1);
          }
          if (!out && gtny == tmn) {
            gtny += gdy;
            gcy += (gdirs & 2) ? 1 : -1;
            out = gcy == ((gdirs & 2) ? D : -1);
          }
          if (!out && gtnz == tmn) {
            gtnz += gdz;
            gcz += (gdirs & 4) ? 1 : -1;
            out = gcz == ((gdirs & 4) ? D : -1);
          }
          gtc0 = gtc1;
// ... 226 lines not shown
```

icon-ray-tracing_amd/csrc/irt_render.hip:

```cpp

#include <initializer_list>

#include "irt_raygen.h"

namespace irt {

constexpr int kQueueXcds = 8;
struct QueueCursor {
  int cur;
  uint32_t dead;
};
__device__ __forceinline__ uint32_t queue_take(uint32_t *Q, uint32_t numBlocksAll, QueueCursor &c) {
  while (c.dead != (1u << kQueueXcds) - 1u) {
    const uint32_t x = (uint32_t)c.cur;
    const uint32_t limit = numBlocksAll > x ? 4u * ((numBlocksAll - x + kQueueXcds - 1) / kQueueXcds) : 0u;
    uint32_t v = 0xFFFFFFFFu;
    if (__lane_id() == 0) {
      uint32_t *q = Q + (size_t)x * kQueueLine;
      if (__hip_atomic_load(q, __ATOMIC_RELAXED, __HIP_MEMORY_SCOPE_AGENT) < limit) v = atomicAdd(q, 1u);
    }
    v = __builtin_amdgcn_readfirstlane(v);
    if (v < limit) return ((v >> 2) * kQueueXcds + x) * 4u + (v & 3u);
    c.dead |= 1u << x;
    c.cur = (c.cur + 1) & (kQueueXcds - 1);
  }
  return 0xFFFFFFFFu;
}
__device__ __forceinline__ void queue_done(uint32_t *Q) {
  if (__lane_id() == 0) {
    __threadfence();
    const uint32_t waves = gridDim.x * (blockDim.x >> 6);
    if (atomicAdd(&Q[kQueueXcds * kQueueLine], 1u) == waves - 1u) {
      for (int x = 0; x <= kQueueXcds; ++x)
        __hip_atomic_store(&Q[(size_t)x * kQueueLine], 0u, __ATOMIC_RELAXED, __HIP_MEMORY_SCOPE_AGENT);
    }
  }
}

template <int OPT>
__global__ void __launch_bounds__((OPT & OPT_WAVEWG) ? 64 : 256,
                                  ((OPT >> 8) & 15) ? ((OPT >> 8) & 15) : 1)
    k_render(RenderArgs A) {
  constexpr bool lean = (OPT & OPT_LEAN) != 0;
  constexpr bool wavewg = (OPT & OPT_WAVEWG) != 0;
  constexpr int kWpg = wavewg ? 1 : 4;
  constexpr bool split = kWpg < 4;
  static_assert(!split || (lean && Tracer<OPT>::kCoop), "one-wave workgroups: lean, cooperative kernels");
  constexpr int kT = 64 * kWpg;
  constexpr int kW = kT / 64;
  __shared__ float s_th[lean ? 1 : 256];
  __shared__ uint32_t s_cnt[kCnt];
  __shared__ LogfTab s_logf[16];
  __shared__ uint32_t s_sph[lean ? 1 : kSphBitWords];
  __shared__ int4 s_dda[split ? 1 : 256];
  __shared__ float4 s_entry[kT];
  __shared__ CoopWave s_coop[kW];
  __shared__ ScanWave s_scan[Tracer<OPT>::kWaveScan ? kW : 1];
  __shared__ float4 s_acc[lean ? 1 : 256];
  __shared__ uint2 s_jmp[kLcgJumps];
  const int tid = threadIdx.x;
  if (A.wgTrace && tid == 0) {
    uint32_t *w = A.wgTrace + 4 * (blockIdx.y * gridDim.x + blockIdx.x);
    w[0] = (uint32_t)__builtin_amdgcn_s_memrealtime();
    w[2] = __builtin_amdgcn_s_getreg((31 << 11) | 4);
    w[3] = __builtin_amdgcn_s_getreg((15 << 11) | 20);
  }
  if (A.probeExit == 1) return;
  constexpr bool kVoid = (OPT & OPT_VOID) != 0;
  constexpr bool kList = kVoid && (OPT & OPT_VLIST) != 0;
  static_assert(kVoid || (OPT & OPT_VLIST) == 0, "OPT_VLIST: a form of the OPT_VOID kernels");
  uint32_t vitem = 0u;
  static_assert(!kVoid || (wavewg && lean && Tracer<OPT>::kCoop &&
                           (OPT & (OPT_SPLIT | OPT_SLOT | OPT_STATS | OPT_TIMING | OPT_QUEUE | OPT_GRID | OPT_WEDGE)) == 0),
                "void packets: the default kernels' plain grid form");
  if constexpr (kVoid && !kList) {
    const RenderArgs &VA = fresh_args();
    const uint32_t vb = blockIdx.x, vwave = (vb >> 3) & 3u;
    const uint32_t vblk = ((vb >> 5) << 3) | (vb & 7u), vpkt = vblk * 4u + vwave;
    uint32_t isVoid = VA.voidBits ? (scalar_word(VA.voidBits, vpkt >> 5) >> (vpkt & 31u)) & 1u : 0u;
    asm volatile("" : "+s"(isVoid));
    if (isVoid) {
      void_packet(VA, vblk, (int)vwave, blockIdx.y == 0, 1u);
      return;
    }
  }
  if constexpr (kList) {
    const RenderArgs &VA = fresh_args();
    const uint32_t vx = blockIdx.x, vlive = VA.voidLive;
    const uint32_t j = blockIdx.y * VA.voidRow + (vx - vlive);
    const bool inVoid = vx >= vlive, none = inVoid && j >= VA.voidCount;
    const uint32_t w = scalar_word(VA.voidList, none ? 0u : inVoid ? vlive + j : vx);
    vitem = __builtin_amdgcn_readfirstlane(none ? ~0u : w);
    uint32_t leave = __builtin_amdgcn_readfirstlane(inVoid || vitem == ~0u ? 1u : 0u);
    asm volatile("" : "+s"(leave));
    if (leave) {
      const bool some = vitem != ~0u;
      void_packet(VA, some ? vitem >> 2 : 0u, (int)(some ? vitem & 3u : 0u), some, some ? (uint32_t)VA.numSamples : 0u);
      return;
    }
  }
  uint64_t tStart = 0;
  if constexpr ((OPT & OPT_TIMING) != 0) tStart = __builtin_amdgcn_s_memtime();
  constexpr bool dmaTab = (OPT & OPT_DMATAB) != 0 && kT == 64 && Tracer<OPT>::kCoop;
  if constexpr (dmaTab) {
    typedef __attribute__((address_space(3))) void *LdsPtr;
    const char *jt = reinterpret_cast<const char *>(&kLcgJumpTab.ma[0][0]);
    static_assert(sizeof(kLcgJumpTab.ma) == kLcgJumps * 8 && kLcgJumps * 8 <= 64 * 16 + 16, "jump table: 65 chunks");
    __builtin_amdgcn_global_load_lds((const void *)(jt + 16 * tid), (LdsPtr)s_jmp, 16, 0, 0);
    if (tid == 0)
      __builtin_amdgcn_global_load_lds((const void *)(jt + 1024), (LdsPtr)(reinterpret_cast<char *>(s_jmp) + 1024), 16, 0, 0);
    static_assert(sizeof(LogfTab) == 16, "logf table: one chunk per entry");
    if (tid < 16) __builtin_amdgcn_global_load_lds((const void *)(kLogfTab + tid), (LdsPtr)s_logf, 16, 0, 0);
  }
  const float th = lean ? 0.f : A.srgbTh[tid];
  const LogfTab lt = dmaTab ? LogfTab{0.0, 0.0} : kLogfTab[tid & 15];
  uint32_t sph[kSphBitWords / 256];
  if (!lean && A.numSph) {
#pragma unroll
    for (int k = 0; k < kSphBitWords / 256; ++k) sph[k] = A.sphBits[tid + 256 * k];
  }
  uint2 jmpv[(kLcgJumps + kT - 1) / kT];
#pragma unroll
  for (int k = 0; k < (kLcgJumps + kT - 1) / kT; ++k) {
    const int j = tid + kT * k;
    jmpv[k] = make_uint2(0u, 0u);
    if (!dmaTab && Tracer<OPT>::kCoop && j < kLcgJumps) jmpv[k] = make_uint2(kLcgJumpTab.ma[j][0], kLcgJumpTab.ma[j][1]);
  }
#pragma unroll
  for (int k = 0; k < (kLcgJumps + kT - 1) / kT; ++k) {
    const int j = tid + kT * k;
    if (!dmaTab && Tracer<OPT>::kCoop && j < kLcgJumps) *reinterpret_cast<uvec2 *>(&s_jmp[j]) = __builtin_bit_cast(uvec2, jmpv[k]);
  }
  if constexpr (!lean) s_th[tid] = th;
  if (!dmaTab && tid < 16) s_logf[tid] = lt;
  if (!lean && A.numSph) {
#pragma unroll
    for (int k = 0; k < kSphBitWords / 256; ++k) s_sph[tid + 256 * k] = sph[k];
  }
  if (tid < kCnt) s_cnt[tid] = 0;
  __shared__ uint32_t s_done;
  if (tid == 0) s_done = 0;
  __shared__ uint32_t s_gbits[(OPT & OPT_GRID) ? kGridBitWords : 1];
  if constexpr ((OPT & OPT_GRID) != 0) {
#pragma unroll
    for (int k = 0; k < kGridBitWords / 256; ++k) s_gbits[tid + 256 * k] = A.gridBits[tid + 256 * k];
  }
  if constexpr (dmaTab)
    __builtin_amdgcn_wave_barrier();
  else
    __syncthreads();
  if (A.probeExit == 2) return;
  Tracer<OPT> T{{}, A, s_logf, lean ? A.sphBits : s_sph, s_cnt, {0, 0, 0, 0, 0, 0, 0}};
  T.s_gbits = s_gbits;
  const float *th_p = lean ? A.srgbTh : s_th;
  constexpr uint32_t kNwb = 4 / kWpg;
  uint32_t bx = blockIdx.x;
  int partSel = -1;
  uint32_t splitP = 0u;
  bool emptyItem = false;
  constexpr bool splitOk = wavewg && (OPT & OPT_SPLIT) != 0;
  if constexpr (splitOk) {
    if (bx < A.numSplit) {
      const uint32_t item = scalar_word(A.splitList, bx);
      emptyItem = item == ~0u;
      partSel = emptyItem ? 0 : (int)((((item >> 4) & 15u) << 8) | (item & 15u));
      splitP = emptyItem ? 0u : item >> 8;
    } else {
      bx -= A.numSplit;
    }
  }
  const uint32_t wg = split ? (((bx >> 3) / kNwb) << 3) | (bx & 7u) : bx;
  const int wwave = kList ? (int)(vitem & 3u) : partSel >= 0 ? (int)(splitP & 3u)
                                  : split ? (int)(((bx >> 3) % kNwb) * kWpg) : 0;
  const int ptid = split ? wwave * 64 + tid : tid;
  if constexpr ((OPT & OPT_TIMING) != 0) {
    T.tLast = tStart;
    T.tmark(0);
  }
  const uint64_t c0 = A.schedCost ? wall_clock64() : 0;
  const uint32_t blk = kList ? vitem >> 2 : partSel >= 0 ? splitP >> 2 : A.schedOrder ? scalar_word(A.schedOrder, wg) : wg;
  const uint32_t pkt = blk * 4u + (uint32_t)wwave;
  const bool splitAway = splitOk && partSel < 0 && ((scalar_word(A.splitMask, pkt >> 5) >> (pkt & 31u)) & 1u);
  uint32_t launched = 0u;
  bool pxActive = false;
  if constexpr (Tracer<OPT>::kCoop) {
    constexpr bool queued = (OPT & OPT_QUEUE) != 0;
    static_assert(!queued || (!split && (OPT & (OPT_STATS | OPT_TIMING)) == 0),
                  "persistent launches: 256-thread workgroups, no per-wave statistics");
    const uint32_t perFrame = (uint32_t)A.numTiles * 16u;
    const uint32_t blocksAll = perFrame * (uint32_t)A.numSamples;
    QueueCursor qc = {(int)(blockIdx.x & (kQueueXcds - 1)), 0u};
    uint32_t p = queued ? queue_take(A.queue, blocksAll, qc) : 0u;
    bool more = !queued || p != 0xFFFFFFFFu;
    while (more) {
      uint32_t pblk = blk, nx = 0u;
      int pw = wwave + (tid >> 6), frame = (int)blockIdx.y;
      if constexpr (queued) {
        const uint32_t g = p >> 2;
        frame = A.numSamples > 1 ? (int)(g / perFrame) : 0;
        pblk = g - (uint32_t)frame * perFrame;
        pw = (int)(p & 3u);
      }
      pblk = __builtin_amdgcn_readfirstlane(pblk);
      pw = __builtin_amdgcn_readfirstlane(pw);
      frame = __builtin_amdgcn_readfirstlane(frame);
      int ltid = tid;
      if constexpr (queued) {
        asm volatile("" : "+v"(ltid));
        typedef const __attribute__((address_space(4))) RenderArgs *KArgs;
        KArgs kp = (KArgs)__builtin_amdgcn_kernarg_segment_ptr();
        asm volatile("" : "+s"(kp));
        const RenderArgs &AL = *(const RenderArgs *)kp;
        Tracer<OPT> TL{{}, AL, s_logf, lean ? AL.sphBits : s_sph, s_cnt, {0, 0, 0, 0, 0, 0, 0}};
        TL.s_gbits = s_gbits;
        const Pixel ppx = pixel_of(AL, pblk, pw * 64 + (ltid & 63));
        launched += (uint32_t)__popcll(__ballot(ppx.active));
        render_pixel_coop<OPT>(AL, TL, ppx, lean ? AL.srgbTh : s_th, s_dda, s_entry, s_acc, s_coop[ltid >> 6],
                               &s_scan[Tracer<OPT>::kWaveScan ? ltid >> 6 : 0], s_jmp, ltid, AL.accumID + frame,
                               pblk, pw, frame);
        TL.flush_coop();
      } else {
        const int pl = partSel & 255, pn = 64 >> pl;
        Pixel ppx = pixel_of(A, pblk, pw * 64 + (partSel < 0 ? (ltid & 63) : ((partSel >> 8) * pn) | (ltid & (pn - 1))));
        if (partSel >= 0) ppx.active = ppx.active && (ltid & 63) < pn;
        if (splitAway || emptyItem) ppx.active = false;
        launched += (uint32_t)__popcll(__ballot(ppx.active));
        T.frame = frame;
        render_pixel_coop<OPT>(A, T, ppx, th_p, s_dda, s_entry, s_acc, s_coop[ltid >> 6],
                               &s_scan[Tracer<OPT>::kWaveScan ? ltid >> 6 : 0], s_jmp, ltid, cam_accum_id(A, frame),
                               pblk, pw, frame, partSel);
        if (A.chain && frame < A.numSamples - 1 && frame != A.chainWithhold) {
#ifdef IRT_PROBE_BUILD
          if (A.probeExit != 16)
#endif
            asm volatile("s_waitcnt vmcnt(0)" ::: "memory");
          if (__lane_id() == 0)
            __hip_atomic_store(A.chainFlag + (size_t)pblk * 4u + (uint32_t)pw, A.chainEpoch + (uint32_t)frame + 1u,
                               __ATOMIC_RELAXED, __HIP_MEMORY_SCOPE_AGENT);
        }
      }
      if constexpr (queued) nx = queue_take(A.queue, blocksAll, qc);
      p = nx;
      more = queued && p != 0xFFFFFFFFu;
    }
    if constexpr (queued) queue_done(A.queue);
    T.flush_coop();
  }
  else {
    const Pixel px = pixel_of(A, blk, ptid);
    float4 *slot = A.numSamples > 1 ? A.sampleBuf + (size_t)blockIdx.y * gridDim.x * blockDim.x + blk * 256u + ptid
                                    : nullptr;
    if (px.active) render_pixel<OPT>(A, T, px, th_p, s_dda, s_entry, tid, A.accumID + (int)blockIdx.y, slot);
    pxActive = px.active;
    launched = (uint32_t)__popcll(__ballot(px.active));
  }
  if constexpr ((OPT & OPT_TIMING) != 0) {
    T.tmark(8);
    if ((tid & 63) == 0) {
      for (int k = 0; k < TimeAccOn::kTimeRegions; ++k)
        atomicAdd(&A.counters[5 + k], (unsigned long long)T.tAcc[k]);
      atomicAdd(&A.counters[14], (unsigned long long)(__builtin_amdgcn_s_memtime() - tStart));
      atomicAdd(&A.counters[15], 1ull);
    }
  }
  if constexpr ((OPT & OPT_STATS) != 0) {
    uint32_t ss = T.cnt.steps, sm = T.cnt.steps, ds = T.cnt.deg, dm = T.cnt.deg;
    for (int off = 32; off > 0; off >>= 1) {
      ss += __shfl_down(ss, off, 64);
      sm = max(sm, (uint32_t)__shfl_down(sm, off, 64));
      ds += __shfl_down(ds, off, 64);
      dm = max(dm, (uint32_t)__shfl_down(dm, off, 64));
    }
    const uint32_t d = T.cnt.steps;
    const int bkt = d == 0 ? 0 : (d <= 2 ? 1 : (d <= 5 ? 2 : 3));
    uint32_t hist[4];
    for (int k = 0; k < 4; ++k)
      hist[k] = T.kCoop ? Tracer<OPT>::wave_sum(T.cnt.candHist[k])
                        : (uint32_t)__popcll(__ballot(pxActive && bkt == k));
    if ((tid & 63) == 0) {
      atomicAdd(&A.counters[5], (unsigned long long)ss);
      atomicAdd(&A.counters[6], (unsigned long long)sm);
      atomicAdd(&A.counters[7], (unsigned long long)(T.kCoop ? T.cnt.hops : ds));
      atomicAdd(&A.counters[8], (unsigned long long)(T.kCoop ? T.cnt.locRounds : dm));
      atomicMax(&A.counters[9], (unsigned long long)sm);
      atomicMax(&A.counters[10], (unsigned long long)dm);
      atomicAdd(&A.counters[11], (unsigned long long)T.cnt.rounds);
      for (int k = 0; k < 4; ++k)
        if (hist[k]) atomicAdd(&A.counters[12 + k], (unsigned long long)hist[k]);
    }
  }
  if (A.counters || A.schedCost || A.wgTrace) {
    const int lane = (int)__lane_id();
    if (A.counters && lane == 0 && launched) atomicAdd(&s_cnt[0], launched);
    uint32_t prev = 0;
    if (lane == 0)
      prev = __hip_atomic_fetch_add(&s_done, 1u, __ATOMIC_ACQ_REL, __HIP_MEMORY_SCOPE_WORKGROUP);
    prev = (uint32_t)__shfl((int)prev, 0, 64);
    if (prev == (blockDim.x >> 6) - 1u) {
      if (A.counters) flush_counters(A, s_cnt, lane);
      if (A.schedCost && lane == 0 && (wavewg || wwave == 0) && !splitAway && !emptyItem) {
        uint64_t dt = wall_clock64() - c0;
        if (partSel >= 0) dt <<= (partSel & 255);
        A.schedCost[pkt] = dt > 0xFFFFFFFFull ? 0xFFFFFFFFu : (uint32_t)dt;
      }
      if (A.wgTrace && lane == 0)
        A.wgTrace[4 * (blockIdx.y * gridDim.x + blockIdx.x) + 1] = (uint32_t)__builtin_amdgcn_s_memrealtime();
    }
  }
}

__global__ void __launch_bounds__(256) k_accumulate(RenderArgs A) {
  __shared__ float s_th[256];
  s_th[threadIdx.x] = A.srgbTh[threadIdx.x];
  __syncthreads();
  const uint32_t gid = blockIdx.x * 256u + threadIdx.x;
  const Pixel px = pixel_of(A, blockIdx.x, (int)threadIdx.x);
  if (!px.active) return;
  const size_t lanes = (size_t)gridDim.x * 256u;
  float4 a = A.accum[px.outIdx];
  bool wrote = false;
  for (int k = 0; k < A.numSamples; ++k) {
    const float4 c = A.sampleBuf[(size_t)k * lanes + gid];
    if (c.w == kNoSample) continue;
    const float w = 1.f / (float)(A.accumID + k + 1);
    a.x = w * c.x + (1.f - w) * a.x;
    a.y = w * c.y + (1.f - w) * a.y;
    a.z = w * c.z + (1.f - w) * a.z;
    a.w = w * c.w + (1.f - w) * a.w;
    wrote = true;
  }
  if (!wrote) return;
  A.accum[px.outIdx] = a;
  A.fb[px.outIdx] = srgb_byte(s_th, a.x) + (srgb_byte(s_th, a.y) << 8) +
                    (srgb_byte(s_th, a.z) << 16) + (make_8bit(a.w) << 24);
}

__global__ void __launch_bounds__(256) k_debug_locate(RenderArgs A, const float *xyz, int n,
                                                      int *found, float *value) {
  __shared__ uint32_t s_sph[kSphBitWords];
  __shared__ uint32_t s_cnt[kCnt];
  for (int i = threadIdx.x; i < kSphBitWords; i += 256) s_sph[i] = A.numSph ? A.sphBits[i] : 0u;
  if (threadIdx.x < kCnt) s_cnt[threadIdx.x] = 0;
  __syncthreads();
  Tracer<kDefaultVariant & ~OPT_MONO> T{{}, A, nullptr, s_sph, s_cnt, {0, 0, 0, 0, 0, 0, 0}};
  const int j = (int)(blockIdx.x * 256 + threadIdx.x);
  if (j < n) {
    float v = 0.f;
    found[j] = T.locate(xyz[3 * j], xyz[3 * j + 1], xyz[3 * j + 2], v) ? 1 : 0;
    value[j] = v;
  }
}

template <int O>
__global__ void __launch_bounds__(256) k_debug_locate_wave(RenderArgs A, const float *xyz, int n,
                                                           int *found, float *value) {
  __shared__ uint32_t s_sph[kSphBitWords];
  __shared__ uint32_t s_cnt[kCnt];
  __shared__ CoopWave s_coop[4];
  __shared__ ScanWave s_scan[4];
  for (int i = threadIdx.x; i < kSphBitWords; i += 256) s_sph[i] = A.numSph ? A.sphBits[i] : 0u;
  if (threadIdx.x < kCnt) s_cnt[threadIdx.x] = 0;
  __syncthreads();
  Tracer<O> T{{}, A, nullptr, s_sph, s_cnt, {0, 0, 0, 0, 0, 0, 0}};
  static_assert(Tracer<O>::kWaveScan, "the default kernel scans wave-wide");
  const int j = (int)(blockIdx.x * 256 + threadIdx.x);
  const bool want = j < n;
  float x = 0.f, y = 0.f, z = 0.f;
  if (want) {
    x = xyz[3 * j];
    y = xyz[3 * j + 1];
    z = xyz[3 * j + 2];
  }
  float v = 0.f;
  const bool f = T.locate_wave(want, x, y, z, v, s_coop[threadIdx.x >> 6], s_scan[threadIdx.x >> 6]);
  if (want) {
    found[j] = f ? 1 : 0;
    value[j] = v;
  }
}

void launch_debug_locate(const RenderArgs &A, const float *xyz, int n, int *found, float *value,
                         hipStream_t s, bool wave) {
  if (n <= 0) return;
// ... 157 lines not shown
```

icon-ray-tracing_amd/host/irt_debug.cpp:

```cpp

#include <math.h>
#include <vector>
#include <string.h>

#include "icon_rt_hip_debug.h"
#include "irt_internal.h"

using namespace irt;

struct irt_debug_scene {
  HostScene s;
  std::vector<irt_icon_cell> cells;
  WedgeScene w;
};

struct irt_debug_void_cache {
  VoidCache c;
};

extern "C" {

float irt_debug_asinf(float x) { return glibc_asinf(x); }
float irt_debug_atan2f(float y, float x) { return glibc_atan2f(y, x); }
int irt_debug_f2i(float x) { return f2i_x86(x); }
// ... 61 lines not shown
    if (record) *record = r;
  }
  return hit;
}

int irt_debug_scene_values(const irt_debug_scene *s, uint32_t rec, float r, float *out2) {
  if (!s || !out2 || rec >= s->s.n) return IRT_E_INVALID;
  const float *hv = &s->s.hv[(size_t)rec * kHV];
  int32_t nl;
  memcpy(&nl, hv + 63, 4);
  out2[0] = hv[32 + find_height(hv, nl, r)];
  out2[1] = record_value_host(s->s, rec,
                              record_path(s->s.meta[rec], s->s.rng[2 * (size_t)rec],
                                          s->s.rng[2 * (size_t)rec + 1], r), r);
  return IRT_OK;
}

int irt_debug_scene_candidates(const irt_debug_scene *s, irt_vec3f p, uint32_t *records,
                               int capacity) {
  if (!s || s->s.G == 0) return 0;
  const uint32_t cell = cubemap_cell(p.x, p.y, p.z, s->s.G);
  const uint32_t b = s->s.offsets[cell], e = s->s.offsets[cell + 1];
  int k = 0;
  for (uint32_t i = b; i < e; ++i, ++k)
    if (records && k < capacity) records[k] = s->s.entryRec[i];
  return k;
}

int irt_debug_scene_planes(const irt_debug_scene *s, uint32_t record, float *out12) {
  if (!s || !out12 || record >= s->s.n) return IRT_E_INVALID;
  memcpy(out12, &s->s.planes[12 * (size_t)record], 12 * sizeof(float));
  return IRT_OK;
}

void irt_debug_scene_free(irt_debug_scene *s) { delete s; }

int irt_debug_scene_array(const irt_debug_scene *s, int which, void *dst, size_t capacity,
                          size_t *bytes) {
  if (!s || !bytes) {
    set_error("irt_debug_scene_array: null argument");
    return IRT_E_INVALID;
  }
  const HostScene &S = s->s;
  std::vector<uint32_t> rec;
  const void *src = nullptr;
  size_t n = 0;
  switch (which) {
    case IRT_DEBUG_ARRAY_BIN_HDR: src = S.binHdr.data(); n = S.binHdr.size() * 4; break;
    case IRT_DEBUG_ARRAY_FAT: src = S.fat.data(); n = S.fat.size() * 4; break;
    case IRT_DEBUG_ARRAY_BLOCKS: src = S.blocks.data(); n = S.blocks.size() * 4; break;
    case IRT_DEBUG_ARRAY_SPH_R: src = S.sphR.data(); n = S.sphR.size() * 4; break;
    case IRT_DEBUG_ARRAY_SPH_OFF: src = S.sphOff.data(); n = S.sphOff.size() * 4; break;
    case IRT_DEBUG_ARRAY_SPH_REC:
      for (uint32_t r : S.sphRec) {
        int32_t nl;
        memcpy(&nl, &S.hv[(size_t)r * kHV + 63], 4);
        rec.push_back(r);
        rec.push_back((uint32_t)nl);
      }
      src = rec.data();
      n = rec.size() * 4;
      break;
    case IRT_DEBUG_ARRAY_SPH_BITS: src = S.sphBits.data(); n = S.sphBits.size() * 4; break;
    default:
      set_error("irt_debug_scene_array: unknown array %d", which);
      return IRT_E_INVALID;
  }
  *bytes = n;
  if (dst && capacity >= n && n) memcpy(dst, src, n);
  return IRT_OK;
}

int irt_debug_scene_locate_wedge(irt_debug_scene *s, irt_vec3f p, float *value) {
  if (!s || !value) return IRT_E_INVALID;
  if (s->w.G == 0) {
    set_error("irt_debug_scene_locate_wedge: call irt_debug_scene_build_wedges first");
    return IRT_E_INVALID;
  }
  return wedge_locate_host(s->w, s->cells.data(), p.x, p.y, p.z, *value) ? 1 : 0;
}

int irt_debug_scene_build_wedges(irt_debug_scene *s, const irt_icon_cell *cells, size_t n) {
  if (!s || (n && !cells) || n != s->s.n) {
    set_error("irt_debug_scene_build_wedges: cells do not match the scene");
    return IRT_E_INVALID;
  }
  s->cells.assign(cells, cells + n);
  return build_wedges(cells, n, s->w);
}

int irt_debug_scene_locate_triangle(irt_debug_scene *s, irt_vec3f p, float *value,
                                    uint32_t *record) {
  if (!s || !value) return IRT_E_INVALID;
  if (s->w.G == 0) {
    set_error("irt_debug_scene_locate_triangle: call irt_debug_scene_build_wedges first");
    return IRT_E_INVALID;
  }
  return triangle_locate_host(s->w, s->cells.data(), p.x, p.y, p.z, *value, record) ? 1 : 0;
}

int irt_debug_intersect_wedge(const float *v24, irt_vec3f p, float *value) {
  WV4 V[6];
  memcpy(V, v24, sizeof(V));
  float v = 0.f;
  const bool hit = intersect_wedge(v, p.x, p.y, p.z, V);
  if (hit) *value = v;
  return hit ? 1 : 0;
}

int irt_debug_sched_order(const uint32_t *cost, int numBlocks, int tilesX, int tileStride, int policy,
                          int splitLg, float splitFactor, int numCU, int wavewg, size_t capacity,
                          uint32_t maxSplit, uint32_t *out, uint32_t *numSplit) {
  if (!cost || !out || !numSplit || numBlocks < 0 || numBlocks % 16 || (size_t)numBlocks > capacity ||
      splitLg < 0 || splitLg > 3 || maxSplit % 8) {
    set_error("irt_debug_sched_order: bad argument");
    return IRT_E_INVALID;
  }
  *numSplit = sched_order(cost, numBlocks, tilesX, tileStride, policy, splitLg, splitFactor, numCU,
                          wavewg != 0, capacity, maxSplit, out);
  return IRT_OK;
}

irt_debug_void_cache *irt_debug_void_cache_create(void) { return new irt_debug_void_cache(); }
void irt_debug_void_cache_free(irt_debug_void_cache *cache) { delete cache; }

int irt_debug_void_packets(irt_debug_void_cache *cache, const irt_launch_params *lp, const irt_volume_info *info,
                           int W, int H, int tileBegin, int tileStride, const int32_t *tileList, int listCount,
                           uint32_t *bits, size_t capacity, uint32_t *numVoid, long long *computations) {
  if (!lp || !info || !numVoid || W <= 0 || H <= 0 || tileBegin < 0 || tileStride <= 0 || listCount < 0) {
    set_error("irt_debug_void_packets: bad argument");
    return IRT_E_INVALID;
  }
  const int total = ((W + 63) / 64) * ((H + 63) / 64);
  const int numTiles = tileList ? listCount : tileBegin < total ? (total - tileBegin + tileStride - 1) / tileStride : 0;
  for (int k = 0; tileList && k < listCount; ++k)
    if (tileList[k] < 0 || tileList[k] >= total) {
      set_error("irt_debug_void_packets: tile id %d at %d outside [0, %d)", tileList[k], k, total);
      return IRT_E_INVALID;
    }
  if (void_words(numTiles) > capacity || (!bits && capacity)) {
    set_error("irt_debug_void_packets: %zu words needed", void_words(numTiles));
    return IRT_E_INVALID;
  }
  const VoidRequest q = void_request(*lp, *info, W, H, tileBegin, tileStride, numTiles, tileList);
  VoidCache local;
  VoidCache &vc = cache ? cache->c : local;
  vc.lookup(q);
  if (void_words(numTiles)) memcpy(bits, vc.bits.data(), void_words(numTiles) * sizeof(uint32_t));
  *numVoid = vc.count;
  if (computations) *computations = vc.generation;
  return IRT_OK;
}

int irt_debug_void_lists(irt_debug_void_cache *cache, const irt_launch_params *lp, const irt_volume_info *info,
                         int W, int H, int tileBegin, int tileStride, const int32_t *tileList, int listCount,
                         int numFrames, uint32_t *items, size_t capacity, uint32_t *numLive, uint32_t *voidPerRow,
                         uint32_t *numVoid) {
  if (!lp || !info || !numLive || !voidPerRow || !numVoid || W <= 0 || H <= 0 || tileBegin < 0 || tileStride <= 0 ||
      listCount < 0 || numFrames < 1) {
    set_error("irt_debug_void_lists: bad argument");
    return IRT_E_INVALID;
  }
  const int total = ((W + 63) / 64) * ((H + 63) / 64);
  const int numTiles = tileList ? listCount : tileBegin < total ? (total - tileBegin + tileStride - 1) / tileStride : 0;
  for (int k = 0; tileList && k < listCount; ++k)
    if (tileList[k] < 0 || tileList[k] >= total) {
      set_error("irt_debug_void_lists: tile id %d at %d outside [0, %d)", tileList[k], k, total);
      return IRT_E_INVALID;
    }
  const VoidRequest q = void_request(*lp, *info, W, H, tileBegin, tileStride, numTiles, tileList);
  VoidCache local;
  VoidCache &vc = cache ? cache->c : local;
  vc.lookup(q);
  const VoidLists &vl = vc.lists;
  *numLive = vl.live;
  *numVoid = vl.count;
  *voidPerRow = vl.count ? void_row(vl.count, numFrames) : 0u;
  if (!items) return IRT_OK;
  const size_t need = (size_t)vl.live + (size_t)numFrames * *voidPerRow;
  if (need > capacity) {
    set_error("irt_debug_void_lists: %zu words needed", need);
    return IRT_E_INVALID;
  }
  std::copy(vl.items.begin(), vl.items.begin() + vl.live, items);
  for (size_t j = 0; j < (size_t)numFrames * *voidPerRow; ++j)
    items[vl.live + j] = j < vl.count ? vl.items[vl.live + j] : kVoidEmpty;
  return IRT_OK;
}

}
```

icon-ray-tracing_amd/host/irt_void.cpp:

```cpp

#include <math.h>
#include <string.h>

#include <algorithm>
#include <vector>

#include "irt_internal.h"

namespace irt {

namespace {

struct V3 {
  double x, y, z;
};
V3 operator+(V3 a, V3 b) { return {a.x + b.x, a.y + b.y, a.z + b.z}; }
V3 operator*(double s, V3 a) { return {s * a.x, s * a.y, s * a.z}; }
double dot(V3 a, V3 b) { return a.x * b.x + a.y * b.y + a.z * b.z; }
double norm(V3 a) { return sqrt(dot(a, a)); }
double abs1(V3 a) { return fabs(a.x) + fabs(a.y) + fabs(a.z); }

bool hits_box(V3 org, V3 d, const double lo[3], const double hi[3]) {
  const double o[3] = {org.x, org.y, org.z}, dd[3] = {d.x, d.y, d.z};
  double t0 = 0.0, t1 = INFINITY;
  for (int k = 0; k < 3; ++k) {
    if (dd[k] == 0.0) {
      if (!(o[k] > lo[k] && o[k] < hi[k])) return false;
      continue;
    }
    const double a = (lo[k] - o[k]) / dd[k], b = (hi[k] - o[k]) / dd[k];
    t0 = std::max(t0, std::min(a, b));
    t1 = std::min(t1, std::max(a, b));
  }
  return t0 < t1;
}

struct View {
  V3 org, d00, du, dv, axis;
  double uu, vv, uv;
  double m0, mu, mv;
  double cosN, sinN;
  V3 dir(double a, double b) const { return d00 + a * du + b * dv; }
};
struct Rect {
  double a0, a1, b0, b1;
};
enum { kUnbounded = -2, kCentreHits = -1, kUndecided = 0, kClear = 1, kAllHit = 2 };

int sphere_rect(const View &v, const Rect &r, double &delta) {
  const double ha = 0.5 * (r.a1 - r.a0), hb = 0.5 * (r.b1 - r.b0);
  const V3 c = v.dir(r.a0 + ha, r.b0 + hb);
  const double lc = norm(c), h = sqrt(ha * ha * v.uu + hb * hb * v.vv + 2.0 * ha * hb * v.uv), dmin = lc - h;
  if (!(lc > 0.0) || !(h < 0.16 * lc)) return kUnbounded;
  delta = 8.0 * ldexp(1.0, -24) * (v.m0 + r.a1 * v.mu + r.b1 * v.mv) / dmin + 4e-5;
  const double ct = dot(c, v.axis) / lc, x0 = 1.01 * h / dmin, x = x0 + delta + 1e-9;
  if (ct > v.cosN + v.sinN * x0) return kAllHit;
  if (!(ct < v.cosN)) return kCentreHits;
  const double L = v.cosN * (1.0 - 0.5 * x * x) - v.sinN * x;
  return ct < L && ct > -L ? kClear : kUndecided;
}
bool sphere_clear(const View &v, const Rect &r, int depth) {
  double delta;
  const int res = sphere_rect(v, r, delta);
  if (res != kUndecided || depth == 3) return res == kClear;
  const double am = 0.5 * (r.a0 + r.a1), bm = 0.5 * (r.b0 + r.b1);
  return sphere_clear(v, {r.a0, am, r.b0, bm}, depth + 1) && sphere_clear(v, {am, r.a1, r.b0, bm}, depth + 1) &&
         sphere_clear(v, {r.a0, am, bm, r.b1}, depth + 1) && sphere_clear(v, {am, r.a1, bm, r.b1}, depth + 1);
}

}

uint32_t void_packets(const VoidRequest &q, uint32_t *bits, VoidLists *lists) {
  memset(bits, 0, void_words(q.numTiles) * sizeof(uint32_t));
  if (lists) *lists = VoidLists();
  if (q.raygen != IRT_RAYGEN_WITH_ACCEL || q.accelMode != IRT_ACCEL_SPHERE || q.mode != IRT_MODE_USER_GEOM) return 0;
  if (q.W <= 0 || q.H <= 0 || q.tileStride <= 0 || q.tileBegin < 0) return 0;
  for (int k = 0; k < 12; ++k)
    if (!std::isfinite(q.cam[k])) return 0;
  for (int k = 0; k < 3; ++k)
    if (!std::isfinite(q.bmin[k]) || !std::isfinite(q.bmax[k])) return 0;
  const double R = q.rOuter, r = q.rInner;
  if (!std::isfinite(R) || !std::isfinite(r) || !(r >= 0.0) || !(R >= r) || !(R > 0.0)) return 0;
  const V3 org = {q.cam[0], q.cam[1], q.cam[2]}, d00 = {q.cam[3], q.cam[4], q.cam[5]},
           du = {q.cam[6], q.cam[7], q.cam[8]}, dv = {q.cam[9], q.cam[10], q.cam[11]};
  const double eps = ldexp(1.0, -19);
  const double P = norm(org);
  if (!(P > 1.001 * R) || !(eps * P * P <= 0.01 * R * R)) return 0;
  const double need = asin(sqrt((R / P) * (R / P) + eps));
  const V3 axis = (-1.0 / P) * org;
  double T = 0.0;
  for (int k = 0; k < 8; ++k) {
    const V3 cnr = {(k & 1) ? q.bmax[0] : q.bmin[0], (k & 2) ? q.bmax[1] : q.bmin[1], (k & 4) ? q.bmax[2] : q.bmin[2]};
    T = std::max(T, norm(cnr + (-1.0) * org));
  }
  if (!(T < 1e9)) return 0;
  const View v = {org, d00, du, dv, axis, dot(du, du), dot(dv, dv), fabs(dot(du, dv)), abs1(d00), abs1(du), abs1(dv),
                  cos(need), sin(need)};
  const int tilesX = (q.W + 63) / 64, total = tilesX * ((q.H + 63) / 64);
  uint32_t count = 0;
  std::vector<uint32_t> res[8], voids;
  auto in_box = [&](double a0, double a1, double b0, double b1, double delta) {
    const double s = T * (delta + 4e-7);
    double blo[3], bhi[3];
    for (int j = 0; j < 3; ++j) {
      blo[j] = (double)q.bmin[j] + s;
      bhi[j] = (double)q.bmax[j] - s;
      if (!(blo[j] < bhi[j])) return false;
    }
    return hits_box(org, v.dir(a0, b0), blo, bhi) && hits_box(org, v.dir(a1, b0), blo, bhi) &&
           hits_box(org, v.dir(a0, b1), blo, bhi) && hits_box(org, v.dir(a1, b1), blo, bhi);
  };
  for (int k = 0; k < q.numTiles; ++k) {
    const int tileId = q.tileList ? q.tileList[k] : q.tileBegin + k * q.tileStride;
    if (tileId < 0 || tileId >= total) continue;
    const int tx0 = (tileId % tilesX) * 64, ty0 = (tileId / tilesX) * 64;
    double delta = 0.0;
    const Rect tile = {tx0 + 0.5, std::min(tx0 + 64, q.W) + 0.5, ty0 + 0.5, std::min(ty0 + 64, q.H) + 0.5};
    const int whole = sphere_rect(v, tile, delta);
    if (whole == kAllHit && !lists) continue;
    const bool tileVoid = whole == kClear && in_box(tile.a0, tile.a1, tile.b0, tile.b1, delta);
    for (int j = 0; j < 64; ++j) {
      const size_t p = (size_t)k * 64 + j;
      const int sub = j >> 2, wave = j & 3;
      const int x0 = tx0 + (((sub & 3) << 4) | ((wave & 1) << 3)), y0 = ty0 + (((sub >> 2) << 4) | ((wave >> 1) << 3));
      if (x0 >= q.W || y0 >= q.H) continue;
      bool isVoid = tileVoid;
      if (!tileVoid && whole != kAllHit) {
        const Rect r = {x0 + 0.5, std::min(x0 + 8, q.W) + 0.5, y0 + 0.5, std::min(y0 + 8, q.H) + 0.5};
        double pd = 0.0;
        isVoid = !(sphere_rect(v, r, pd) < 0 || pd == 0.0) && sphere_clear(v, r, 0) && in_box(r.a0, r.a1, r.b0, r.b1, pd);
      }
      if (!isVoid) {
        if (lists) res[(p >> 2) & 7].push_back((uint32_t)p);
        continue;
      }
      bits[p >> 5] |= 1u << (p & 31);
      if (lists) voids.push_back((uint32_t)p);
      ++count;
    }
  }
  if (lists && count) {
    size_t len = 0;
    for (const auto &r : res) len = std::max(len, r.size());
    lists->live = (uint32_t)(8 * len);
    lists->count = count;
    lists->items.assign(8 * len + voids.size(), kVoidEmpty);
    for (size_t x = 0; x < 8; ++x)
      for (size_t k = 0; k < res[x].size(); ++k) lists->items[8 * k + x] = res[x][k];
    std::copy(voids.begin(), voids.end(), lists->items.begin() + 8 * len);
  }
  return count;
}

bool VoidCache::lookup(const VoidRequest &q, bool defer) {
  std::vector<unsigned char> k(sizeof(VoidRequest) + (q.tileList ? (size_t)std::max(q.numTiles, 0) * sizeof(int32_t) : 0));
  VoidRequest flat = q;
  flat.tileList = q.tileList ? reinterpret_cast<const int32_t *>(1) : nullptr;
  memcpy(k.data(), &flat, sizeof(flat));
  if (q.tileList && q.numTiles > 0) memcpy(k.data() + sizeof(flat), q.tileList, (size_t)q.numTiles * sizeof(int32_t));
  const bool same = keyed && k == key;
  if (same && valid) return false;
  if (!same) {
    key.swap(k);
    keyed = true;
    valid = false;
    count = 0;
    if (defer) return false;
  }
  bits.assign(void_words(q.numTiles), 0u);
  count = void_packets(q, bits.data(), &lists);
  valid = true;
  ++generation;
  return true;
}

}
```

icon-ray-tracing_amd/python/irt.py:

```python
from __future__ import annotations

import ctypes as C
import os
from dataclasses import dataclass

import numpy as np

PKG_DIR = os.path.dirname(os.path.dirname(os.path.abspath(__file__)))
LIB_PATH = os.environ.get("IRT_LIB_PATH") or os.path.join(PKG_DIR, "libicon_rt_hip.so")

CELL_DTYPE = np.dtype(
    [("lat", "<f4", (3,)), ("lon", "<f4", (3,)), ("numLayers", "<i4"),
     ("height", "<f4", (32,)), ("value", "<f4", (32,))], align=False)
assert CELL_DTYPE.itemsize == 284

RAYGEN_WITH_ACCEL = 0
RAYGEN_AE = 1
ACCEL_SPHERE = 0
ACCEL_GRID = 1
MODE_USER_GEOM = 0
MODE_TRIANGLES = 1
MODE_CUBQL = 2
MAX_LEVELS = 16
LEVELS_BACK = 1
# ... 242 lines not shown
        raise IrtError(f"render_levels: radius[{bad[0]}] = {r[bad[0]]} is not finite and positive", E_INVALID)
    return r


def levels_order(radii):
    r = np.ascontiguousarray(radii, dtype=np.float32).reshape(-1)
    out, idx = np.zeros(r.size, np.float32), np.zeros(r.size, np.int32)
    _check(lib().irt_levels_order(_ptr(r), r.size, _ptr(out), _ptr(idx)), "irt_levels_order")
    return out, idx


def _weights(weight, levels: int):
    if weight is None:
        return None
    w = np.ascontiguousarray(weight, dtype=np.float32).reshape(-1)
    if w.size != levels:
        raise IrtError(f"{w.size} weights for {levels} levels", E_INVALID)
    return w


def column_reduce(value, found, weight=None, miss: float = float("nan")) -> dict:
    value = np.ascontiguousarray(value, dtype=np.float32)
    found = np.ascontiguousarray(found, dtype=np.uint8)
    if value.ndim < 1 or value.shape != found.shape:
        raise IrtError(f"column_reduce: value {value.shape} and found {found.shape} differ", E_INVALID)
    levels, shape = value.shape[0], value.shape[1:]
    w = _weights(weight, levels)
    out = {k: np.zeros(shape, t) for k, t in COLUMN_OUTPUTS.items()}
    _check(lib().irt_column_reduce(_ptr(value), _ptr(found), levels, int(np.prod(shape, dtype=np.int64)),
                                   _ptr(w) if w is not None else None, float(miss),
                                   ColumnOut(**{k: a.ctypes.data for k, a in out.items()})), "irt_column_reduce")
    return out


def _hist_args(weighting, band_edges):
    w = HIST_WEIGHTINGS.get(weighting, weighting)
    if not isinstance(w, (int, np.integer)):
        raise IrtError(f"histogram: weighting {weighting!r} is none of {sorted(HIST_WEIGHTINGS)}", E_INVALID)
    if band_edges is None:
        return int(w), None, 1
    e = np.ascontiguousarray(band_edges, dtype=np.float32).reshape(-1)
    if e.size < 2:
        raise IrtError(f"histogram: {e.size} band edges (at least 2)", E_INVALID)
    return int(w), e, e.size - 1


def histogram_cells(cells, value_range, bins: int, weighting="count", band_edges=None) -> dict:
    cells = np.ascontiguousarray(cells, dtype=CELL_DTYPE)
    w, e, bands = _hist_args(weighting, band_edges)
    out = {"bins": np.zeros((bands, max(int(bins), 0)), np.uint64), "tails": np.zeros((bands, 3), np.uint64),
           "outside": np.zeros(1, np.uint64)}
    _check(lib().irt_histogram_cells(_ptr(cells), cells.size, box1(*value_range), int(bins), w,
                                     _ptr(e) if e is not None else None, bands,
                                     HistogramOut(**{k: a.ctypes.data for k, a in out.items()})), "irt_histogram_cells")
    return out


def _segments(seg) -> np.ndarray:
    seg = np.ascontiguousarray(seg, dtype=SEGMENT_DTYPE).reshape(-1)
    assert SEGMENT_DTYPE.itemsize == 64
    return seg


def overlay_styles(styles):
    styles = list(styles)
    arr = (OverlayStyle * max(len(styles), 1))()
    for k, (rgba, w) in enumerate(styles):
        arr[k] = OverlayStyle(Vec4(*(float(x) for x in rgba)), float(w))
    return arr, len(styles)


def overlay_segments(lat, lon, first=None, max_arc: float = 0.0174533, style: int = 0) -> np.ndarray:
    lat = np.ascontiguousarray(lat, dtype=np.float32).reshape(-1)
    lon = np.ascontiguousarray(lon, dtype=np.float32).reshape(-1)
    if lat.size != lon.size:
        raise IrtError(f"overlay_segments: {lat.size} lat for {lon.size} lon", E_INVALID)
    first = np.ascontiguousarray([0, lat.size] if first is None else first, dtype=np.int32).reshape(-1)
    if first.size < 1 or (first.size > 1 and int(first[-1]) > lat.size):
        raise IrtError(f"overlay_segments: first ends at {first[-1] if first.size else None} of {lat.size} points",
                       E_INVALID)
    n = C.c_size_t()
    args = (_ptr(lat), _ptr(lon), _ptr(first), first.size - 1, float(max_arc), int(style))
    _check(lib().irt_overlay_segments(*args, None, 0, C.byref(n)), "irt_overlay_segments")
    out = np.zeros(n.value, SEGMENT_DTYPE)
    _check(lib().irt_overlay_segments(*args, _ptr(out), out.size, C.byref(n)), "irt_overlay_segments")
    return out


def graticule(step_lat: float, step_lon: float, max_arc: float = 0.0174533, style: int = 0) -> np.ndarray:
    n = C.c_size_t()
    args = (float(step_lat), float(step_lon), float(max_arc), int(style))
    _check(lib().irt_graticule(*args, None, 0, C.byref(n)), "irt_graticule")
    out = np.zeros(n.value, SEGMENT_DTYPE)
    _check(lib().irt_graticule(*args, _ptr(out), out.size, C.byref(n)), "irt_graticule")
    return out


def overlay_bins(segments, max_half_width: float, bins_per_edge: int):
    seg = _segments(segments)
    N = int(bins_per_edge)
    if not 1 <= N <= OVERLAY_MAX_BINS:
        raise IrtError(f"overlay_bins: binsPerEdge {N} is outside [1, {OVERLAY_MAX_BINS}]", E_INVALID)
    start = np.zeros(6 * N * N + 1, np.uint32)
    n = C.c_size_t()
    _check(lib().irt_overlay_bins(_ptr(seg), seg.size, float(max_half_width), N, _ptr(start), None, 0, C.byref(n)),
           "irt_overlay_bins")
    lists = np.zeros(n.value, np.uint32)
    _check(lib().irt_overlay_bins(_ptr(seg), seg.size, float(max_half_width), N, _ptr(start), _ptr(lists), lists.size,
                                  C.byref(n)), "irt_overlay_bins")
    return start, lists


def overlay_cover(segments, styles, u, bins=None, bins_per_edge: int = 0) -> np.ndarray:
    seg = _segments(segments)
    st, ns = overlay_styles(styles)
    u = np.ascontiguousarray(u, dtype=np.float32)
    if u.ndim < 1 or u.shape[-1] != 3:
        raise IrtError(f"overlay_cover: u of shape {u.shape} (..., 3)", E_INVALID)
    out = np.full(u.shape[:-1], -2, np.int32)
    start, lists = bins if bins is not None else (None, None)
    _check(lib().irt_overlay_cover(_ptr(seg), seg.size, st, ns, _ptr(start) if start is not None else None,
                                   _ptr(lists) if lists is not None else None, int(bins_per_edge), _ptr(u),
                                   out.size, _ptr(out)), "irt_overlay_cover")
    return out


def overlay_width(lp: LaunchParams, height: int, surface_radius: float, pixels: float) -> float:
    if int(height) < 1:
        raise IrtError("overlay_width: height must be positive", E_INVALID)
    w = C.c_float()
    _check(lib().irt_overlay_width(C.byref(lp), float(surface_radius), float(pixels), C.byref(w)), "irt_overlay_width")
    return float(w.value)


def vec3(v) -> Vec3:
    return Vec3(float(v[0]), float(v[1]), float(v[2]))


def box1(lo, hi) -> Box1:
    return Box1(float(lo), float(hi))


def default_kernel_id(ctx=None) -> int:
    L = lib()
    if ctx is not None:
        L.irt_debug_get_variant.argtypes = [C.c_void_p]
        v = int(L.irt_debug_get_variant(ctx._h)) & ~4096
        d = int(L.irt_debug_default_variant())
        L.irt_debug_slot_use.argtypes = [C.c_void_p, C.c_void_p]
        if v in ((d & ~4096), (d | 262144) & ~4096, (d | 1073741824) & ~4096) and L.irt_debug_slot_use(ctx._h, None) == 1:
            v |= 128
        elif ctx.void_use() > 0:
            v |= 16
        return v
    return int(L.irt_debug_default_variant()) & ~4096


PLAN_SLOTS, PLAN_VOID_BITS, PLAN_VOID_LIST, PLAN_QUEUE, PLAN_CHAIN = 1, 2, 4, 8, 16


def plan(variant: int, sampler: int = 0, accel: int = 0, flags: int = 0, tiles: int = 1, frames: int = 1,
         num_split: int = 0, void_live: int = 0, void_row: int = 0, queue_wg: int = 0) -> tuple:
    L = lib()
    L.irt_debug_plan.argtypes = [C.c_int] * 6 + [C.c_uint32] * 3 + [C.c_int, C.POINTER(C.c_int)]
    out = (C.c_int * 5)()
    _check(L.irt_debug_plan(variant, sampler, accel, flags, tiles, frames, num_split, void_live, void_row,
                            queue_wg, out), "irt_debug_plan")
    return tuple(out)


def variant_workgroups(variant: int, sched: bool, num_tiles: int, frames: int = 1) -> int:
    L = lib()
    L.irt_debug_variant_workgroups.argtypes = [C.c_int] * 4
    L.irt_debug_variant_workgroups.restype = C.c_longlong
    n = L.irt_debug_variant_workgroups(variant, 1 if sched else 0, num_tiles, frames)
    if n < 0:
        raise IrtError("irt_debug_variant_workgroups failed")
    return n


def synth_grid(root_n: int, bisections: int, levels: int, top_height: float = 75e3,
               noise: float = 0.0, seed: int = 1234, terrain: float = 0.0) -> np.ndarray:
    n = C.c_size_t()
    _check(lib().irt_synth_grid_terrain(root_n, bisections, levels, top_height, noise, seed, terrain,
                                        None, 0, C.byref(n)), "irt_synth_grid")
    cells = np.zeros(n.value, dtype=CELL_DTYPE)
    _check(lib().irt_synth_grid_terrain(root_n, bisections, levels, top_height, noise, seed, terrain,
                                        _ptr(cells), n.value, C.byref(n)), "irt_synth_grid")
    return cells


def load_ic(path: str, max_num_cells: int = -1) -> np.ndarray:
    n = C.c_size_t()
    _check(lib().irt_load_ic(path.encode(), max_num_cells, None, 0, C.byref(n)), "irt_load_ic")
    cells = np.zeros(n.value, dtype=CELL_DTYPE)
    _check(lib().irt_load_ic(path.encode(), max_num_cells, _ptr(cells), n.value, C.byref(n)),
           "irt_load_ic")
    return cells


class ConvertOpts(C.Structure):
    _fields_ = [("hgridFile", C.c_char_p), ("hsurfFile", C.c_char_p),
                ("hhlFiles", C.POINTER(C.c_char_p)), ("numHhlFiles", C.c_int),
                ("dataFiles", C.POINTER(C.c_char_p)), ("numDataFiles", C.c_int),
                ("varName", C.c_char_p), ("maxLayers", C.c_int)]


def convert_icon(hgrid: str, hsurf: str, hhl: list, data: list, var: str = "pres",
                 max_layers: int = 5) -> np.ndarray:
    hp = (C.c_char_p * max(len(hhl), 1))(*[f.encode() for f in hhl])
    dp = (C.c_char_p * max(len(data), 1))(*[f.encode() for f in data])
    o = ConvertOpts(hgrid.encode(), hsurf.encode(), hp, len(hhl), dp, len(data), var.encode(),
                    max_layers)
    n = C.c_size_t()
    _check(lib().irt_convert_icon(C.byref(o), None, 0, C.byref(n)), "irt_convert_icon")
    cells = np.zeros(n.value, dtype=CELL_DTYPE)
    _check(lib().irt_convert_icon(C.byref(o), _ptr(cells), n.value, C.byref(n)),
           "irt_convert_icon")
    return cells


def convert_icon_umesh(hgrid: str, hsurf: str, hhl: list, data: list, path: str,
                       var: str = "pres", max_layers: int = 5):
    hp = (C.c_char_p * max(len(hhl), 1))(*[f.encode() for f in hhl])
    dp = (C.c_char_p * max(len(data), 1))(*[f.encode() for f in data])
    o = ConvertOpts(hgrid.encode(), hsurf.encode(), hp, len(hhl), dp, len(data), var.encode(),
                    max_layers)
    nv, nw = C.c_size_t(), C.c_size_t()
    _check(lib().irt_convert_icon_umesh(C.byref(o), path.encode(), C.byref(nv), C.byref(nw)),
           "irt_convert_icon_umesh")
    return nv.value, nw.value


def read_umesh(path: str) -> dict:
    raw = open(path, "rb").read()
    pos = 0

    def u64():
        nonlocal pos
        v = int(np.frombuffer(raw, np.uint64, 1, pos)[0])
        pos += 8
        return v

    def arr(dtype, width):
        nonlocal pos
        n = u64()
        a = np.frombuffer(raw, dtype, n * width, pos).reshape(n, width) if width > 1 else \
            np.frombuffer(raw, dtype, n, pos)
        pos += a.nbytes
        return a

    out = {"magic": u64(), "vertices": arr(np.float32, 3), "scalars": arr(np.float32, 1)}
    for name, w in (("triangles", 3), ("quads", 4), ("tets", 4), ("pyrs", 5),
                    ("wedges", 6), ("hexes", 8)):
        out[name] = arr(np.int32, w)
    if pos != len(raw):
        raise ValueError(f"{path}: {len(raw) - pos} trailing bytes")
    return out


def save_ic(path: str, cells: np.ndarray):
    cells = np.ascontiguousarray(cells, dtype=CELL_DTYPE)
    _check(lib().irt_save_ic(path.encode(), _ptr(cells), cells.size), "irt_save_ic")


def filter_cells(cells: np.ndarray, lat_range=(-np.inf, np.inf), lon_range=(-np.inf, np.inf)):
    out = np.array(cells, dtype=CELL_DTYPE, copy=True)
    n = C.c_size_t()
    _check(lib().irt_filter_cells(_ptr(out), out.size, box1(*lat_range), box1(*lon_range),
                                  C.byref(n)), "irt_filter_cells")
    return out[: n.value].copy()


def _latlon_arrays(lat, lon, radius):
    return tuple(np.ascontiguousarray(a, dtype=np.float32).reshape(-1) for a in (lat, lon, radius))


def latlon_points(lat, lon, radius) -> np.ndarray:
    lat, lon, radius = _latlon_arrays(lat, lon, radius)
    xyz = np.zeros((radius.size, lat.size, lon.size, 3), np.float32)
    _check(lib().irt_latlon_points(_ptr(lat), lat.size, _ptr(lon), lon.size, _ptr(radius),
                                   radius.size, _ptr(xyz)), "irt_latlon_points")
    return xyz


def _section_arrays(lat, lon, radius):
    lat, lon, radius = _latlon_arrays(lat, lon, radius)
    if lat.size != lon.size:
        raise IrtError(f"a section's columns are (lat, lon) pairs: {lat.size} lat for {lon.size} lon", E_INVALID)
    return lat, lon, radius


def section_points(lat, lon, radius) -> np.ndarray:
    lat, lon, radius = _section_arrays(lat, lon, radius)
    xyz = np.zeros((radius.size, lat.size, 3), np.float32)
    _check(lib().irt_section_points(_ptr(lat), _ptr(lon), lat.size, _ptr(radius), radius.size, _ptr(xyz)),
           "irt_section_points")
    return xyz


def great_circle(lat0: float, lon0: float, lat1: float, lon1: float, n: int):
    n = int(n)
    lat, lon = np.zeros(max(n, 0), np.float32), np.zeros(max(n, 0), np.float32)
    arc = C.c_double()
    _check(lib().irt_great_circle(float(lat0), float(lon0), float(lat1), float(lon1), n, _ptr(lat), _ptr(lon),
                                  C.byref(arc)), "irt_great_circle")
    return lat, lon, arc.value


def sample_admits(x: float, y: float, z: float) -> bool:
    return lib().irt_debug_sample_admits(C.c_float(x), C.c_float(y), C.c_float(z)) == 1


def volume_info(cells: np.ndarray) -> VolumeInfo:
    cells = np.ascontiguousarray(cells, dtype=CELL_DTYPE)
    info = VolumeInfo()
    _check(lib().irt_compute_volume_info(_ptr(cells), cells.size, C.byref(info)),
           "irt_compute_volume_info")
    return info


def default_transfunc(data_range) -> tuple[np.ndarray, tuple[float, float]]:
    lut = np.zeros((300, 4), dtype=np.float32)
    vr = Box1()
    _check(lib().irt_default_transfunc(box1(*data_range), _ptr(lut), C.byref(vr)),
           "irt_default_transfunc")
    return lut, (vr.lower, vr.upper)


def resample_lut(src: np.ndarray, n: int) -> np.ndarray:
    src = np.ascontiguousarray(src, dtype=np.float32).reshape(-1, 4)
    dst = np.zeros((n, 4), dtype=np.float32)
    _check(lib().irt_resample_lut(_ptr(src), src.shape[0], _ptr(dst), n), "irt_resample_lut")
    return dst


def camera_view_all(bounds: Box3, img_w: int, img_h: int, fovy_deg: float = 90.0) -> LaunchParams:
    lp = LaunchParams()
    _check(lib().irt_camera_view_all(bounds, fovy_deg, img_w, img_h, C.byref(lp)),
           "irt_camera_view_all")
    return lp


def camera_look_at(vp, vi, vu, fovy_deg: float, img_w: int, img_h: int) -> LaunchParams:
    lp = LaunchParams()
    _check(lib().irt_camera_look_at(vec3(vp), vec3(vi), vec3(vu), fovy_deg, img_w, img_h,
                                    C.byref(lp)), "irt_camera_look_at")
    return lp


def num_tiles(w: int, h: int) -> int:
    return lib().irt_num_tiles(w, h)


def deal_tiles(lp: LaunchParams, info: VolumeInfo, w: int, h: int, ranks: int,
               rank0_extra: float = 0.0) -> np.ndarray:
    m = C.c_int()
    _check(lib().irt_deal_tiles(C.byref(lp), C.byref(info), w, h, ranks, rank0_extra, None, 0,
                                C.byref(m)), "irt_deal_tiles")
    table = np.full((ranks, m.value), -1, np.int32)
    _check(lib().irt_deal_tiles(C.byref(lp), C.byref(info), w, h, ranks, rank0_extra,
                                _ptr(table), table.size, C.byref(m)), "irt_deal_tiles")
    return table


class VoidCache:

    def __init__(self):
        L = lib()
        L.irt_debug_void_cache_create.restype = C.c_void_p
        L.irt_debug_void_cache_free.argtypes = [C.c_void_p]
        L.irt_debug_void_cache_free.restype = None
        self._h = C.c_void_p(L.irt_debug_void_cache_create())
        self.computations = 0

    def packets(self, lp, info, w, h, tile_begin=0, tile_stride=1, tiles=None):
        out = void_packets(lp, info, w, h, tile_begin, tile_stride, tiles, cache=self)
        return out

    def __del__(self):
        if getattr(self, "_h", None):
            lib().irt_debug_void_cache_free(self._h)
            self._h = None


def void_packets(lp: LaunchParams, info: VolumeInfo, w: int, h: int, tile_begin: int = 0,
                 tile_stride: int = 1, tiles=None, cache: VoidCache = None) -> np.ndarray:
    L = lib()
    L.irt_debug_void_packets.argtypes = [C.c_void_p, C.POINTER(LaunchParams), C.POINTER(VolumeInfo), C.c_int,
                                         C.c_int, C.c_int, C.c_int, C.c_void_p, C.c_int, C.c_void_p,
                                         C.c_size_t, C.POINTER(C.c_uint32), C.POINTER(C.c_longlong)]
    total = num_tiles(w, h)
    t = None if tiles is None else np.ascontiguousarray(tiles, dtype=np.int32)
    nt = len(t) if t is not None else (max(0, (total - tile_begin + tile_stride - 1) // tile_stride)
                                       if tile_begin < total else 0)
    bits = np.zeros(max(2 * nt, 1), np.uint32)
    n, comp = C.c_uint32(), C.c_longlong()
    _check(L.irt_debug_void_packets(cache._h if cache else None, C.byref(lp), C.byref(info), w, h, tile_begin,
                                    tile_stride, _ptr(t) if t is not None else None, nt if t is not None else 0,
                                    _ptr(bits), bits.size, C.byref(n), C.byref(comp)), "irt_debug_void_packets")
    if cache:
        cache.computations = comp.value
    out = ((bits[:2 * nt, None] >> np.arange(32, dtype=np.uint32)[None, :]) & 1).astype(bool).reshape(-1)
    assert int(out.sum()) == n.value
    return out


def void_lists(lp: LaunchParams, info: VolumeInfo, w: int, h: int, frames: int, tile_begin: int = 0,
               tile_stride: int = 1, tiles=None, cache: VoidCache = None):
    L = lib()
    L.irt_debug_void_lists.argtypes = [C.c_void_p, C.POINTER(LaunchParams), C.POINTER(VolumeInfo), C.c_int, C.c_int,
                                       C.c_int, C.c_int, C.c_void_p, C.c_int, C.c_int, C.c_void_p, C.c_size_t,
                                       C.POINTER(C.c_uint32), C.POINTER(C.c_uint32), C.POINTER(C.c_uint32)]
    t = None if tiles is None else np.ascontiguousarray(tiles, dtype=np.int32)
    live, row, n = C.c_uint32(), C.c_uint32(), C.c_uint32()

    def call(items):
        _check(L.irt_debug_void_lists(cache._h if cache else None, C.byref(lp), C.byref(info), w, h, tile_begin,
                                      tile_stride, _ptr(t) if t is not None else None, len(t) if t is not None else 0,
                                      frames, _ptr(items) if items is not None else None,
                                      items.size if items is not None else 0, C.byref(live), C.byref(row), C.byref(n)),
               "irt_debug_void_lists")

    call(None)
    if n.value == 0:
        return None
    items = np.zeros(live.value + frames * row.value, np.uint32)
    call(items)
    return items[:live.value].copy(), items[live.value:].reshape(frames, row.value).copy()


@dataclass
class FrameSetup:
    lp: LaunchParams
    lut: np.ndarray
    value_range: tuple[float, float]
    opacity_scale: float
    info: VolumeInfo


FRAMING_CAMERA = ((0.0, 0.0, 1.4e7), (0.0, 0.0, 0.0), (0.0, 1.0, 0.0), 60.0)


def setup_frame(cells: np.ndarray, width: int, height: int, camera=None,
                camera_div=None, raygen: int = RAYGEN_WITH_ACCEL, info: VolumeInfo = None) -> FrameSetup:
    if info is None:
        info = volume_info(cells)
    lut, vr = default_transfunc((info.dataRange.lower, info.dataRange.upper))
    dw, dh = camera_div if camera_div is not None else (width, height)
    if camera is None:
        lp = camera_view_all(info.bounds, dw, dh)
    else:
        vp, vi, vu, fovy = camera
        lp = camera_look_at(vp, vi, vu, fovy, dw, dh)
    lp.accumID = 0
    lp.ambientColor = Vec3(1.0, 1.0, 1.0)
    lp.ambientRadiance = 1.0
    lp.unitDistance = info.unitDistance
    lp.raygen = raygen
    return FrameSetup(lp=lp, lut=lut, value_range=vr, opacity_scale=1.0, info=info)


SCENE_ARRAYS = {"bin_hdr": 0, "fat": 1, "blocks": 2, "sph_r": 3, "sph_off": 4, "sph_rec": 5,
                "sph_bits": 6}
CONTEXT_ARRAYS = {"slots": 7, "grid_bits": 8}


def _array(fn, h, name):
    which = SCENE_ARRAYS[name] if name in SCENE_ARRAYS else CONTEXT_ARRAYS[name]
    n = C.c_size_t()
    _check(fn(h, which, None, 0, C.byref(n)), "scene array")
    out = np.zeros(max(n.value, 1), np.uint8)
    _check(fn(h, which, _ptr(out), n.value, C.byref(n)), "scene array")
    return out[:n.value]


def check_update_values(values) -> np.ndarray:
    if not isinstance(values, np.ndarray) or values.dtype != np.float32:
        raise TypeError("update_values: values must be a float32 numpy array")
    if values.ndim != 2 or values.shape[1] != 32:
        raise ValueError(f"update_values: values must have shape (n, 32), not {values.shape}")
    if not values.flags.c_contiguous:
        raise ValueError("update_values: values must be C-contiguous")
    return values


class Context:

    def __init__(self, cells: np.ndarray = None, device: int = 0, _handle=None):
        if _handle is None:
            cells = np.ascontiguousarray(cells, dtype=CELL_DTYPE)
            _handle = C.c_void_p()
            _check(lib().irt_create(_ptr(cells), cells.size, device, C.byref(_handle)),
                   "irt_create")
        self._h = _handle
        self.device = device
        self.info = VolumeInfo()
        _check(lib().irt_get_volume_info(self._h, C.byref(self.info)), "irt_get_volume_info")

    @classmethod
    def synth(cls, root_n: int, bisections: int, levels: int, device: int = 0,
              top_height: float = 75e3, noise: float = 0.0, seed: int = 1234,
              terrain: float = 0.0) -> "Context":
        h = C.c_void_p()
        _check(lib().irt_create_synth_terrain(root_n, bisections, levels, top_height, noise, seed,
                                              terrain, device, C.byref(h)), "irt_create_synth")
        return cls(device=device, _handle=h)

    @classmethod
    def from_file(cls, path: str, max_num_cells: int = -1, device: int = 0) -> "Context":
        h = C.c_void_p()
        _check(lib().irt_create_from_file(path.encode(), max_num_cells, device, C.byref(h)),
               "irt_create_from_file")
        return cls(device=device, _handle=h)

    @classmethod
    def streamed(cls, chunks, num_cells: int, device: int = 0) -> "Context":
        h = C.c_void_p()
        _check(lib().irt_create_begin(num_cells, device, C.byref(h)), "irt_create_begin")
        try:
            for ch in chunks:
                ch = np.ascontiguousarray(ch, dtype=CELL_DTYPE)
                _check(lib().irt_create_append(h, _ptr(ch), ch.size), "irt_create_append")
            _check(lib().irt_create_end(h), "irt_create_end")
        except Exception:
            lib().irt_destroy(h)
            raise
        return cls(device=device, _handle=h)

    def array(self, name: str) -> np.ndarray:
        return _array(lib().irt_debug_context_array, self._h, name)

    def array_bytes(self, name: str) -> int:
        which = SCENE_ARRAYS[name] if name in SCENE_ARRAYS else CONTEXT_ARRAYS[name]
        n = C.c_size_t()
        _check(lib().irt_debug_context_array(self._h, which, None, 0, C.byref(n)), "scene array")
        return n.value

    def close(self):
        if getattr(self, "_h", None):
            lib().irt_destroy(self._h)
            self._h = None

    def __del__(self):
        try:
            self.close()
        except Exception:
            pass

    def __enter__(self):
        return self

    def __exit__(self, *a):
        self.close()

    def set_transfunc(self, lut: np.ndarray, value_range, opacity_scale: float = 1.0):
        lut = np.ascontiguousarray(lut, dtype=np.float32).reshape(-1, 4)
        _check(lib().irt_set_transfunc(self._h, _ptr(lut), lut.shape[0], box1(*value_range),
                                       float(opacity_scale)), "irt_set_transfunc")

    def update_values(self, values: np.ndarray, first: int = 0):
        values = check_update_values(values)
        _check(lib().irt_update_values(self._h, int(first), values.shape[0], _ptr(values)),
               "irt_update_values")

    def update_values_device(self, ptr: int, n: int, first: int = 0, stream: int = 0):
        _check(lib().irt_update_values_device(self._h, int(first), int(n), C.c_void_p(ptr),
                                              C.c_void_p(stream)), "irt_update_values_device")

    def end_update(self):
        _check(lib().irt_update_values_end(self._h), "irt_update_values_end")
        _check(lib().irt_get_volume_info(self._h, C.byref(self.info)), "irt_get_volume_info")

    def set_statistics(self, on: bool):
        L = lib()
        L.irt_set_statistics.argtypes = [C.c_void_p, C.c_int]
        _check(L.irt_set_statistics(self._h, 1 if on else 0), "irt_set_statistics")

    def set_queue(self, on: bool):
        L = lib()
        L.irt_debug_set_queue.argtypes = [C.c_void_p, C.c_int]
        _check(L.irt_debug_set_queue(self._h, 1 if on else 0), "irt_debug_set_queue")

    def set_wg_trace(self, ptr: int):
        L = lib()
        L.irt_debug_set_wg_trace.argtypes = [C.c_void_p, C.c_void_p]
        _check(L.irt_debug_set_wg_trace(self._h, C.c_void_p(ptr or None)), "irt_debug_set_wg_trace")

    def set_chain(self, on: bool):
        L = lib()
        L.irt_debug_set_chain.argtypes = [C.c_void_p, C.c_int]
        _check(L.irt_debug_set_chain(self._h, 1 if on else 0), "irt_debug_set_chain")

    def chain_errors(self) -> int:
        L = lib()
        L.irt_debug_chain_errors.argtypes = [C.c_void_p]
        n = L.irt_debug_chain_errors(self._h)
        if n < 0:
            raise IrtError("irt_debug_chain_errors failed")
        return n

    def set_chain_fault(self, spins: int, withhold_frame: int = -1):
        L = lib()
        L.irt_debug_set_chain_fault.argtypes = [C.c_void_p, C.c_uint32, C.c_int]
        _check(L.irt_debug_set_chain_fault(self._h, spins, withhold_frame), "irt_debug_set_chain_fault")

    def sched_split(self):
        L = lib()
        L.irt_debug_sched_split.argtypes = [C.c_void_p, C.POINTER(C.c_int), C.POINTER(C.c_int)]
        n, lg = C.c_int(), C.c_int()
        _check(L.irt_debug_sched_split(self._h, C.byref(n), C.byref(lg)), "irt_debug_sched_split")
        return n.value, lg.value

    def void_use(self) -> int:
        L = lib()
        if not hasattr(L, "irt_debug_void_use"):
            return 0
        L.irt_debug_void_use.argtypes = [C.c_void_p]
        L.irt_debug_void_use.restype = C.c_longlong
        return L.irt_debug_void_use(self._h)

    def last_workgroups(self) -> int:
        L = lib()
        L.irt_debug_last_workgroups.argtypes = [C.c_void_p]
        L.irt_debug_last_workgroups.restype = C.c_longlong
        return L.irt_debug_last_workgroups(self._h)

    def last_plan(self) -> tuple:
        L = lib()
        L.irt_debug_last_plan.argtypes = [C.c_void_p, C.POINTER(C.c_int)]
        out = (C.c_int * 5)()
        _check(L.irt_debug_last_plan(self._h, out), "irt_debug_last_plan")
        return tuple(out)

    def launch_workgroups(self, num_tiles: int, frames: int = 1) -> int:
        L = lib()
        L.irt_debug_launch_workgroups.argtypes = [C.c_void_p, C.c_int, C.c_int]
        L.irt_debug_launch_workgroups.restype = C.c_longlong
        n = L.irt_debug_launch_workgroups(self._h, num_tiles, frames)
        if n < 0:
            raise IrtError("irt_debug_launch_workgroups failed")
        return n

    def queue(self) -> bool:
        L = lib()
        L.irt_debug_get_queue.argtypes = [C.c_void_p]
        return L.irt_debug_get_queue(self._h) == 1

    def clear(self, fb_ptr: int, accum_ptr: int, num_pixels: int, stream: int = 0):
        _check(lib().irt_clear_frame(self._h, C.c_void_p(fb_ptr), C.c_void_p(accum_ptr),
                                     num_pixels, C.c_void_p(stream)), "irt_clear_frame")

    def render(self, lp: LaunchParams, width: int, height: int, fb_ptr: int, accum_ptr: int,
               stream: int = 0):
        _check(lib().irt_render(self._h, C.byref(lp), width, height, C.c_void_p(fb_ptr),
                                C.c_void_p(accum_ptr), C.c_void_p(stream)), "irt_render")

    def render_tiles(self, lp: LaunchParams, width: int, height: int, tile_begin: int,
                     tile_stride: int, fb_ptr: int, accum_ptr: int, stream: int = 0) -> int:
        n = C.c_int()
        _check(lib().irt_render_tiles(self._h, C.byref(lp), width, height, tile_begin,
                                      tile_stride, C.c_void_p(fb_ptr), C.c_void_p(accum_ptr),
                                      C.byref(n), C.c_void_p(stream)), "irt_render_tiles")
        return n.value

    def render_sequence(self, lps, width: int, height: int, fb_ptr: int, accum_ptr: int,
                        stream: int = 0):
        arr = (LaunchParams * len(lps))(*lps)
        _check(lib().irt_render_sequence(self._h, arr, len(lps), width, height, C.c_void_p(fb_ptr),
                                         C.c_void_p(accum_ptr), C.c_void_p(stream)),
               "irt_render_sequence")

    def render_tile_list_sequence(self, lps, width: int, height: int, tiles, fb_tiles_ptr: int,
                                  accum_tiles_ptr: int, stream: int = 0):
        arr = (LaunchParams * len(lps))(*lps)
        t = np.ascontiguousarray(tiles, dtype=np.int32)
        L = lib()
        L.irt_render_tile_list_sequence.argtypes = [C.c_void_p, C.POINTER(LaunchParams), C.c_int, C.c_int, C.c_int,
                                                    C.c_void_p, C.c_int, C.c_void_p, C.c_void_p, C.c_void_p]
        _check(L.irt_render_tile_list_sequence(self._h, arr, len(lps), width, height, _ptr(t), t.size,
                                               C.c_void_p(fb_tiles_ptr), C.c_void_p(accum_tiles_ptr),
                                               C.c_void_p(stream)), "irt_render_tile_list_sequence")

    def render_accumulate(self, lp: LaunchParams, width: int, height: int, num_frames: int,
                          fb_ptr: int, accum_ptr: int, stream: int = 0):
        _check(lib().irt_render_accumulate(self._h, C.byref(lp), width, height, num_frames,
                                           C.c_void_p(fb_ptr), C.c_void_p(accum_ptr),
                                           C.c_void_p(stream)), "irt_render_accumulate")

    def render_tiles_accumulate(self, lp: LaunchParams, width: int, height: int, tile_begin: int,
                                tile_stride: int, num_frames: int, fb_ptr: int, accum_ptr: int,
                                stream: int = 0) -> int:
        n = C.c_int()
        _check(lib().irt_render_tiles_accumulate(self._h, C.byref(lp), width, height, tile_begin,
                                                 tile_stride, num_frames, C.c_void_p(fb_ptr),
                                                 C.c_void_p(accum_ptr), C.byref(n),
                                                 C.c_void_p(stream)), "irt_render_tiles_accumulate")
        return n.value

    def render_tile_list(self, lp: LaunchParams, width: int, height: int, tiles, num_frames: int,
                         fb_tiles_ptr: int, accum_tiles_ptr: int, stream: int = 0):
        t = np.ascontiguousarray(tiles, dtype=np.int32)
        _check(lib().irt_render_tile_list(self._h, C.byref(lp), width, height, _ptr(t), t.size,
                                          num_frames, C.c_void_p(fb_tiles_ptr),
                                          C.c_void_p(accum_tiles_ptr), C.c_void_p(stream)),
               "irt_render_tile_list")

    def unpack_tile_table(self, gathered_ptr: int, table: np.ndarray, width: int, height: int,
                          fb_ptr: int, stream: int = 0):
        t = np.ascontiguousarray(table, dtype=np.int32)
        _check(lib().irt_unpack_tile_table(self._h, C.c_void_p(gathered_ptr), t.shape[0], t.shape[1],
                                           _ptr(t), width, height, C.c_void_p(fb_ptr),
                                           C.c_void_p(stream)), "irt_unpack_tile_table")

    def unpack_tiles(self, gathered_ptr: int, num_ranks: int, max_tiles: int, width: int,
                     height: int, fb_ptr: int, stream: int = 0):
        _check(lib().irt_unpack_tiles(self._h, C.c_void_p(gathered_ptr), num_ranks, max_tiles,
                                      width, height, C.c_void_p(fb_ptr), C.c_void_p(stream)),
               "irt_unpack_tiles")

    def stats(self) -> RenderStats:
        st = RenderStats()
        _check(lib().irt_get_render_stats(self._h, C.byref(st)), "irt_get_render_stats")
        return st

    def stats_total(self) -> tuple[RenderStats, int]:
        st = RenderStats()
        n = C.c_longlong()
        _check(lib().irt_get_render_stats_total(self._h, C.byref(st), C.byref(n)),
               "irt_get_render_stats_total")
        return st, n.value

    def reset_stats_total(self):
        _check(lib().irt_reset_render_stats_total(self._h), "irt_reset_render_stats_total")

    def set_timing_interval(self, every: int):
        _check(lib().irt_set_timing_interval(self._h, int(every)), "irt_set_timing_interval")

    def build_wedge_accel(self, cells: np.ndarray):
        cells = np.ascontiguousarray(cells, dtype=CELL_DTYPE)
        _check(lib().irt_build_wedge_accel(self._h, _ptr(cells), cells.size),
               "irt_build_wedge_accel")

    def sample_points(self, xyz_ptr: int, n: int, value_ptr: int, found_ptr: int = 0,
                      mode: int = MODE_USER_GEOM, miss: float = float("nan"), stream: int = 0):
        _check(lib().irt_sample_points(self._h, int(mode), C.c_void_p(xyz_ptr), int(n),
                                       C.c_void_p(value_ptr), C.c_void_p(found_ptr), float(miss),
                                       C.c_void_p(stream)), "irt_sample_points")

    def sample_latlon(self, lat, lon, radius, value_ptr: int, found_ptr: int = 0,
                      mode: int = MODE_USER_GEOM, miss: float = float("nan"), stream: int = 0):
        lat, lon, radius = _latlon_arrays(lat, lon, radius)
        _check(lib().irt_sample_latlon(self._h, int(mode), _ptr(lat), lat.size, _ptr(lon), lon.size,
                                       _ptr(radius), radius.size, C.c_void_p(value_ptr),
                                       C.c_void_p(found_ptr), float(miss), C.c_void_p(stream)),
               "irt_sample_latlon")
        return radius.size, lat.size, lon.size

    def render_levels(self, lp: LaunchParams, width: int, height: int, radii, fb_ptr: int, accum_ptr: int,
                      value_ptr: int = 0, level_ptr: int = 0, back: bool = False,
                      miss: float = float("nan"), stream: int = 0):
        radii = levels_radii(radii)
        _check(lib().irt_render_levels(self._h, C.byref(lp), int(width), int(height), _ptr(radii), radii.size,
                                       LEVELS_BACK if back else 0, C.c_void_p(fb_ptr), C.c_void_p(accum_ptr),
                                       C.c_void_p(value_ptr), C.c_void_p(level_ptr), float(miss),
                                       C.c_void_p(stream)), "irt_render_levels")

    def column_latlon(self, lat, lon, radius, out: dict, weight=None, mode: int = MODE_USER_GEOM,
                      miss: float = float("nan"), stream: int = 0):
        lat, lon, radius = _latlon_arrays(lat, lon, radius)
        w = _weights(weight, radius.size)
        unknown = set(out) - set(COLUMN_OUTPUTS)
        if unknown:
            raise IrtError(f"column_latlon: unknown outputs {sorted(unknown)}", E_INVALID)
# ... 223 lines not shown
```

include/icon_rt_hip_debug.h:

```cpp
#ifndef ICON_RT_HIP_DEBUG_H
#define ICON_RT_HIP_DEBUG_H

#include "icon_rt_hip.h"

#ifdef __cplusplus
extern "C" {
#endif

float irt_debug_asinf(float x);
float irt_debug_atan2f(float y, float x);
int irt_debug_f2i(float x);
void irt_debug_lcg_jump(uint32_t n, uint32_t *mul, uint32_t *add);

float irt_debug_logf_entry(uint32_t k);
void irt_debug_srgb_thresholds(float *out256);

uint32_t irt_debug_logf_mismatches(void);
void irt_debug_host_woodcock_log(float *out);

typedef struct irt_debug_scene irt_debug_scene;
int irt_debug_scene_build(const irt_icon_cell *cells, size_t n, irt_debug_scene **out);
int irt_debug_scene_info(const irt_debug_scene *s, irt_volume_info *info);
int irt_debug_scene_locate(const irt_debug_scene *s, irt_vec3f p, float *value,
                           uint32_t *record);
int irt_debug_scene_locate_binned(const irt_debug_scene *s, irt_vec3f p, float *value,
                                  uint32_t *record, uint32_t *tested);
int irt_debug_scene_values(const irt_debug_scene *s, uint32_t rec, float r, float *out2);
int irt_debug_scene_candidates(const irt_debug_scene *s, irt_vec3f p, uint32_t *records,
                               int capacity);
int irt_debug_scene_planes(const irt_debug_scene *s, uint32_t record, float *out12);
void irt_debug_scene_free(irt_debug_scene *s);
int irt_debug_scene_build_wedges(irt_debug_scene *s, const irt_icon_cell *cells, size_t n);
int irt_debug_scene_locate_wedge(irt_debug_scene *s, irt_vec3f p, float *value);
int irt_debug_scene_locate_triangle(irt_debug_scene *s, irt_vec3f p, float *value,
                                    uint32_t *record);
int irt_debug_intersect_wedge(const float *v24, irt_vec3f p, float *value);

enum {
  IRT_DEBUG_ARRAY_BIN_HDR = 0,
  IRT_DEBUG_ARRAY_FAT = 1,
  IRT_DEBUG_ARRAY_BLOCKS = 2,
  IRT_DEBUG_ARRAY_SPH_R = 3,
  IRT_DEBUG_ARRAY_SPH_OFF = 4,
  IRT_DEBUG_ARRAY_SPH_REC = 5,
  IRT_DEBUG_ARRAY_SPH_BITS = 6,
  IRT_DEBUG_ARRAY_SLOTS = 7,
  IRT_DEBUG_ARRAY_GRID_BITS = 8
};
int irt_debug_context_array(const irt_context *ctx, int which, void *dst, size_t capacity,
                            size_t *bytes);
int irt_debug_scene_array(const irt_debug_scene *s, int which, void *dst, size_t capacity,
                          size_t *bytes);

int irt_debug_set_variant(irt_context *ctx, int variant);
int irt_debug_default_variant(void);
int irt_debug_slot_use(const irt_context *ctx, double *tfSamples);
int irt_debug_get_variant(const irt_context *ctx);
int irt_debug_variants(int *out, int capacity);
int irt_debug_set_queue(irt_context *ctx, int on);
int irt_debug_get_queue(const irt_context *ctx);
int irt_debug_queue_wgs(const irt_context *ctx);
int irt_debug_counters(irt_context *ctx, unsigned long long *out16);

int irt_debug_device_math(int device, const float *a, const float *y, const float *x, int n,
                          float *out_asinf, float *out_atan2f);
int irt_debug_fast_math_bounds(int device, double *out4);
void irt_debug_fast_spherical_consts(float *out2);
int irt_debug_device_woodcock_log(int device, float *out);
int irt_debug_device_srgb(int device, const float *x, uint32_t *out, int n);
int irt_debug_locate(irt_context *ctx, const float *xyz, int n, int *found, float *value);
int irt_debug_locate_wave(irt_context *ctx, const float *xyz, int n, int *found, float *value);
int irt_debug_locate_sampler(irt_context *ctx, int mode, const float *xyz, int n, int *found,
                             float *value);
int irt_debug_sample_admits(float x, float y, float z);
int irt_debug_sched(irt_context *ctx, int *policy, int *lastApplied, long long *applied);
int irt_debug_set_wg_trace(irt_context *ctx, uint32_t *trace);
long long irt_debug_launch_workgroups(const irt_context *ctx, int numTiles, int numFrames);
long long irt_debug_variant_workgroups(int variant, int sched, int numTiles, int numFrames);
enum {
  IRT_DEBUG_PLAN_SLOTS = 1,
  IRT_DEBUG_PLAN_VOID_BITS = 2,
  IRT_DEBUG_PLAN_VOID_LIST = 4,
  IRT_DEBUG_PLAN_QUEUE = 8,
  IRT_DEBUG_PLAN_CHAIN = 16
};
int irt_debug_plan(int variant, int sampler, int accelMode, int flags, int numTiles, int numFrames,
                   uint32_t numSplit, uint32_t voidLive, uint32_t voidRow, int queueWG, int out[5]);
int irt_debug_last_plan(const irt_context *ctx, int out[5]);
int irt_debug_sched_split(const irt_context *ctx, int *numSplit, int *splitLg);
int irt_debug_sched_order(const uint32_t *cost, int numBlocks, int tilesX, int tileStride, int policy,
                          int splitLg, float splitFactor, int numCU, int wavewg, size_t capacity,
                          uint32_t maxSplit, uint32_t *out, uint32_t *numSplit);
typedef struct irt_debug_void_cache irt_debug_void_cache;
irt_debug_void_cache *irt_debug_void_cache_create(void);
void irt_debug_void_cache_free(irt_debug_void_cache *cache);
int irt_debug_void_packets(irt_debug_void_cache *cache, const irt_launch_params *lp, const irt_volume_info *info,
                           int W, int H, int tileBegin, int tileStride, const int32_t *tileList, int listCount,
                           uint32_t *bits, size_t capacity, uint32_t *numVoid, long long *computations);
long long irt_debug_void_use(const irt_context *ctx);
int irt_debug_void_lists(irt_debug_void_cache *cache, const irt_launch_params *lp, const irt_volume_info *info,
                         int W, int H, int tileBegin, int tileStride, const int32_t *tileList, int listCount,
                         int numFrames, uint32_t *items, size_t capacity, uint32_t *numLive, uint32_t *voidPerRow,
                         uint32_t *numVoid);
long long irt_debug_last_workgroups(const irt_context *ctx);
int irt_debug_set_chain(irt_context *ctx, int on);
int irt_debug_chain_errors(irt_context *ctx);
int irt_debug_set_chain_fault(irt_context *ctx, uint32_t spins, int withholdFrame);

#ifdef __cplusplus
}
#endif
#endif
```

Measured before the change: 18410 Mray/s.

## Classify interior ray packets on host and skip box/sphere setup on device

Adds a host-side conservative geometric test that marks 8x8 ray packets whose rays provably enter the spherical shell inside the bounding box. The result is shipped either as a second bitmask or as a high bit on void-list items. Flagged packets skip the box test and general range setup on the GPU and use a direct two-sphere interior intersection instead. This trades extra host classification work and upload size, plus some risk from the error-bound reasoning, for less per-ray setup on the GPU.

```diff
diff --git a/icon-ray-tracing_amd/csrc/irt_context.h b/icon-ray-tracing_amd/csrc/irt_context.h
--- a/icon-ray-tracing_amd/csrc/irt_context.h
+++ b/icon-ray-tracing_amd/csrc/irt_context.h
@@ -138,6 +138,7 @@
   long long voidOnDevice = 0;
   bool voidOnDeviceList = false;
   long long lastVoid = 0;
+  long long lastInterior = 0;
   long long lastWorkgroups = 0;
   irt::RenderPlan lastPlan{};
   bool queueOn = false;
diff --git a/icon-ray-tracing_amd/csrc/irt_debug_hooks.hip b/icon-ray-tracing_amd/csrc/irt_debug_hooks.hip
--- a/icon-ray-tracing_amd/csrc/irt_debug_hooks.hip
+++ b/icon-ray-tracing_amd/csrc/irt_debug_hooks.hip
@@ -304,6 +304,7 @@
 }
 
 extern "C" long long irt_debug_void_use(const irt_context *c) { return c ? c->lastVoid : -1; }
+extern "C" long long irt_debug_interior_use(const irt_context *c) { return c ? c->lastInterior : -1; }
 extern "C" long long irt_debug_last_workgroups(const irt_context *c) { return c ? c->lastWorkgroups : -1; }
 
 extern "C" int irt_debug_context_array(const irt_context *c, int which, void *dst, size_t capacity,
diff --git a/icon-ray-tracing_amd/csrc/irt_device.h b/icon-ray-tracing_amd/csrc/irt_device.h
--- a/icon-ray-tracing_amd/csrc/irt_device.h
+++ b/icon-ray-tracing_amd/csrc/irt_device.h
@@ -106,6 +106,25 @@
   hitB = one(radiusB, nearB, farB);
 }
 
+__device__ __forceinline__ void intersect_spheres_interior(const Ray &r, float radiusA, float radiusB, float &nearA,
+                                                           float &farA, float &nearB, float &farB) {
+  const float A = dot3(r.dx, r.dy, r.dz, r.dx, r.dy, r.dz);
+  const float B = dot3(r.dx, r.dy, r.dz, r.ox, r.oy, r.oz) * 2.f;
+  const float OO = dot3(r.ox, r.oy, r.oz, r.ox, r.oy, r.oz);
+  const double rA = recip_d(A);
+  auto one = [&](float radius, float &tnear, float &tfar) {
+    const float C = OO - radius * radius;
+    const float d = sqrtf(B * B - 4.f * A * C);
+    const float q = B < 0.f ? -0.5f * (B - d) : -0.5f * (B + d);
+    const float t1 = div_recip(q, rA);
+    const float t2 = div_recip(C, recip_d(q));
+    tnear = fminf(t1, t2);
+    tfar = fmaxf(t1, t2);
+  };
+  one(radiusA, nearA, farA);
+  one(radiusB, nearB, farB);
+}
+
 __device__ __forceinline__ int project_axis(float s, float lo, float hi, int dim) {
   return f2i_x86((s - lo) / (hi - lo) * (float)(dim - 1));
 }
diff --git a/icon-ray-tracing_amd/csrc/irt_internal.h b/icon-ray-tracing_amd/csrc/irt_internal.h
--- a/icon-ray-tracing_amd/csrc/irt_internal.h
+++ b/icon-ray-tracing_amd/csrc/irt_internal.h
@@ -141,12 +141,15 @@
 inline uint32_t void_row(uint32_t count, int F) {
   return (uint32_t)((((uint64_t)count + (uint64_t)F - 1) / (uint64_t)F + 7) & ~(uint64_t)7);
 }
-uint32_t void_packets(const VoidRequest &q, uint32_t *bits, VoidLists *lists = nullptr);
+uint32_t void_packets(const VoidRequest &q, uint32_t *bits, VoidLists *lists = nullptr, uint32_t *interior = nullptr,
+                      uint32_t *numInterior = nullptr);
 struct VoidCache {
   std::vector<unsigned char> key;
   std::vector<uint32_t> bits;
   VoidLists lists;
   uint32_t count = 0;
+  std::vector<uint32_t> interior;
+  uint32_t interiorCount = 0;
   bool keyed = false, valid = false;
   long long generation = 0;
   bool lookup(const VoidRequest &q, bool defer = false);
diff --git a/icon-ray-tracing_amd/csrc/irt_kernels.h b/icon-ray-tracing_amd/csrc/irt_kernels.h
--- a/icon-ray-tracing_amd/csrc/irt_kernels.h
+++ b/icon-ray-tracing_amd/csrc/irt_kernels.h
@@ -80,7 +80,9 @@
   const uint32_t *voidBits;
   const uint32_t *voidList;
   uint32_t voidLive, voidRow, voidCount;
-};
+  uint32_t interior;
+};
+constexpr uint32_t kItemInterior = 1u << 31;
 constexpr int kQueueLine = 32;
 constexpr uint32_t kChainSpinsDefault = 1u << 20;
 constexpr int kQueueWords = 9 * kQueueLine;
diff --git a/icon-ray-tracing_amd/csrc/irt_launch.hip b/icon-ray-tracing_amd/csrc/irt_launch.hip
--- a/icon-ray-tracing_amd/csrc/irt_launch.hip
+++ b/icon-ray-tracing_amd/csrc/irt_launch.hip
@@ -516,6 +516,7 @@
 int prepare_void(irt_context *c, const irt_launch_params *lp, const RenderRequest &r, Launch &L) {
   RenderArgs &A = L.A;
   c->lastVoid = 0;
+  c->lastInterior = 0;
   if (!(A.chain && !r.seq && r.numFrames > 1 && r.numFrames <= 65535 && L.numTiles > 0 &&
         c->chainWithhold < 0 && c->probeExit == 0 && !stats_variant(c) &&
         lp->raygen == IRT_RAYGEN_WITH_ACCEL && lp->accelMode == IRT_ACCEL_SPHERE &&
@@ -526,7 +527,7 @@
   if (!c->voidCache.count || vl.items.empty()) return IRT_OK;
   const bool list = c->forms->voidList.fn != nullptr &&
                     (size_t)vl.live + void_row(vl.count, r.numFrames) < (size_t)L.numTiles * 64;
-  const size_t words = list ? vl.items.size() : void_words(L.numTiles);
+  const size_t words = list ? vl.items.size() : 2 * void_words(L.numTiles);
   if (words > c->voidCap) {
     int rc = grow(c, Retire::SlotsThenStream, L.s, &c->voidCap, words,
                   {{(void **)&c->d_voidList, [](size_t n) { return n * sizeof(uint32_t); }, false},
@@ -537,7 +538,16 @@
   }
   if (c->voidOnDevice != c->voidCache.generation || c->voidOnDeviceList != list) {
     uint32_t *h = c->h_voidList + (size_t)L.slot * c->voidCap;
-    memcpy(h, list ? vl.items.data() : c->voidCache.bits.data(), words * sizeof(uint32_t));
+    if (list) {
+      const std::vector<uint32_t> &in = c->voidCache.interior;
+      for (size_t k = 0; k < words; ++k) {
+        const uint32_t p = vl.items[k];
+        h[k] = k < vl.live && p != kVoidEmpty && ((in[p >> 5] >> (p & 31)) & 1u) ? p | kItemInterior : p;
+      }
+    } else {
+      memcpy(h, c->voidCache.bits.data(), words / 2 * sizeof(uint32_t));
+      memcpy(h + words / 2, c->voidCache.interior.data(), words / 2 * sizeof(uint32_t));
+    }
     c->voidOnDeviceList = list;
     IRT_HIP(hipMemcpyAsync(c->d_voidList, h, words * sizeof(uint32_t), hipMemcpyHostToDevice, L.s));
     c->voidOnDevice = c->voidCache.generation;
@@ -550,7 +560,9 @@
   } else {
     A.voidBits = c->d_voidList;
   }
+  A.interior = c->voidCache.interiorCount;
   c->lastVoid = c->voidCache.count;
+  c->lastInterior = c->voidCache.interiorCount;
   return IRT_OK;
 }
 
diff --git a/icon-ray-tracing_amd/csrc/irt_raygen.h b/icon-ray-tracing_amd/csrc/irt_raygen.h
--- a/icon-ray-tracing_amd/csrc/irt_raygen.h
+++ b/icon-ray-tracing_amd/csrc/irt_raygen.h
@@ -459,7 +459,7 @@
                                                   const float *s_th, int4 *s_dda, float4 *s_entry,
                                                   float4 *s_acc, CoopWave &W, ScanWave *SW, const uint2 *jmp,
                                                   int tid, int accumID, uint32_t blk, int pwave, int frame,
-                                                  int partSel = -1) {
+                                                  int partSel = -1, uint32_t interior = 0u) {
   constexpr bool kRecompute = ((OPT >> 8) & 15) >= 5;
   const int ptid = pwave * 64 + (tid & 63);
   const int wbase = __builtin_amdgcn_readfirstlane(tid) & ~63;
@@ -502,6 +502,35 @@
     gen_ray(A, accumID, px.x, px.y, st, dx, dy, dz, frame);
     const float3 O = cam_org(A, frame);
     const Ray ray = {O.x, O.y, O.z, 0.f, dx, dy, dz, 1e10f};
+    bool setUp = false;
+    if constexpr ((OPT & OPT_VOID) != 0) {
+      uint32_t iu = __builtin_amdgcn_readfirstlane(interior);
+      if constexpr ((OPT & OPT_VLIST) == 0) {
+        const RenderArgs &BA = fresh_args();
+        const uint32_t pkt = (uint32_t)opaque_u((int)blk) * 4u + (uint32_t)opaque_u(pwave);
+        iu = BA.voidBits && BA.interior
+                 ? (scalar_word(BA.voidBits, 2u * (uint32_t)BA.numTiles + (pkt >> 5)) >> (pkt & 31u)) & 1u
+                 : 0u;
+        iu = __builtin_amdgcn_readfirstlane(iu);
+      }
+      asm volatile("" : "+s"(iu));
+      if (iu) {
+        setUp = true;
+        inBox = true;
+        phase = kRange;
+        if (!toSample && !chainLate && (OPT & OPT_LEAN) == 0)
+          __builtin_amdgcn_global_load_lds((const void *)(A.accum + px.outIdx),
+                                           (__attribute__((address_space(3))) void *)(s_acc + (tid & ~63)),
+                                           16, 0, kRecompute ? 2 : 0);
+        const RenderArgs &IA = fresh_args();
+        float st1, st2, st3, st4;
+        intersect_spheres_interior(ray, IA.sbHi.x, IA.sbLo.x, st1, st4, st2, st3);
+        rlo0 = st1; rhi0 = st2;
+        rlo1 = st3; rhi1 = st4;
+        numRanges = 2;
+      }
+    }
+    if (!setUp) {
     float t0, t1;
     const bool boxHit = box_test(ray, A, t0, t1);
 #ifdef IRT_PROBE_BUILD
@@ -545,6 +574,7 @@
       }
     } else if (toSample) {
       *sample_slot() = make_float4(0.f, 0.f, 0.f, kNoSample);
+    }
     }
   }
   const bool chainReady = !chainLate || __builtin_amdgcn_readfirstlane(chainSeen) == A.chainEpoch + (uint32_t)frame;
diff --git a/icon-ray-tracing_amd/csrc/irt_render.hip b/icon-ray-tracing_amd/csrc/irt_render.hip
--- a/icon-ray-tracing_amd/csrc/irt_render.hip
+++ b/icon-ray-tracing_amd/csrc/irt_render.hip
@@ -70,6 +70,7 @@
   constexpr bool kList = kVoid && (OPT & OPT_VLIST) != 0;
   static_assert(kVoid || (OPT & OPT_VLIST) == 0, "OPT_VLIST: a form of the OPT_VOID kernels");
   uint32_t vitem = 0u;
+  uint32_t interior = 0u;
   static_assert(!kVoid || (wavewg && lean && Tracer<OPT>::kCoop &&
                            (OPT & (OPT_SPLIT | OPT_SLOT | OPT_STATS | OPT_TIMING | OPT_QUEUE | OPT_GRID | OPT_WEDGE)) == 0),
                 "void packets: the default kernels' plain grid form");
@@ -98,6 +99,8 @@
       void_packet(VA, some ? vitem >> 2 : 0u, (int)(some ? vitem & 3u : 0u), some, some ? (uint32_t)VA.numSamples : 0u);
       return;
     }
+    interior = vitem >> 31;
+    vitem &= ~kItemInterior;
   }
   uint64_t tStart = 0;
   if constexpr ((OPT & OPT_TIMING) != 0) tStart = __builtin_amdgcn_s_memtime();
@@ -228,7 +231,7 @@
         T.frame = frame;
         render_pixel_coop<OPT>(A, T, ppx, th_p, s_dda, s_entry, s_acc, s_coop[ltid >> 6],
                                &s_scan[Tracer<OPT>::kWaveScan ? ltid >> 6 : 0], s_jmp, ltid, cam_accum_id(A, frame),
-                               pblk, pw, frame, partSel);
+                               pblk, pw, frame, partSel, interior);
         if (A.chain && frame < A.numSamples - 1 && frame != A.chainWithhold) {
 #ifdef IRT_PROBE_BUILD
           if (A.probeExit != 16)
diff --git a/icon-ray-tracing_amd/host/irt_debug.cpp b/icon-ray-tracing_amd/host/irt_debug.cpp
--- a/icon-ray-tracing_amd/host/irt_debug.cpp
+++ b/icon-ray-tracing_amd/host/irt_debug.cpp
@@ -237,6 +237,34 @@
   return IRT_OK;
 }
 
+int irt_debug_interior_packets(irt_debug_void_cache *cache, const irt_launch_params *lp, const irt_volume_info *info,
+                               int W, int H, int tileBegin, int tileStride, const int32_t *tileList, int listCount,
+                               uint32_t *bits, size_t capacity, uint32_t *numInterior, long long *computations) {
+  if (!lp || !info || !numInterior || W <= 0 || H <= 0 || tileBegin < 0 || tileStride <= 0 || listCount < 0) {
+    set_error("irt_debug_interior_packets: bad argument");
+    return IRT_E_INVALID;
+  }
+  const int total = ((W + 63) / 64) * ((H + 63) / 64);
+  const int numTiles = tileList ? listCount : tileBegin < total ? (total - tileBegin + tileStride - 1) / tileStride : 0;
+  for (int k = 0; tileList && k < listCount; ++k)
+    if (tileList[k] < 0 || tileList[k] >= total) {
+      set_error("irt_debug_interior_packets: tile id %d at %d outside [0, %d)", tileList[k], k, total);
+      return IRT_E_INVALID;
+    }
+  if (void_words(numTiles) > capacity || (!bits && capacity)) {
+    set_error("irt_debug_interior_packets: %zu words needed", void_words(numTiles));
+    return IRT_E_INVALID;
+  }
+  const VoidRequest q = void_request(*lp, *info, W, H, tileBegin, tileStride, numTiles, tileList);
+  VoidCache local;
+  VoidCache &vc = cache ? cache->c : local;
+  vc.lookup(q);
+  if (void_words(numTiles)) memcpy(bits, vc.interior.data(), void_words(numTiles) * sizeof(uint32_t));
+  *numInterior = vc.interiorCount;
+  if (computations) *computations = vc.generation;
+  return IRT_OK;
+}
+
 int irt_debug_void_lists(irt_debug_void_cache *cache, const irt_launch_params *lp, const irt_volume_info *info,
                          int W, int H, int tileBegin, int tileStride, const int32_t *tileList, int listCount,
                          int numFrames, uint32_t *items, size_t capacity, uint32_t *numLive, uint32_t *voidPerRow,
diff --git a/icon-ray-tracing_amd/host/irt_void.cpp b/icon-ray-tracing_amd/host/irt_void.cpp
--- a/icon-ray-tracing_amd/host/irt_void.cpp
+++ b/icon-ray-tracing_amd/host/irt_void.cpp
@@ -68,10 +68,64 @@
          sphere_clear(v, {r.a0, am, bm, r.b1}, depth + 1) && sphere_clear(v, {am, r.a1, bm, r.b1}, depth + 1);
 }
 
-}
-
-uint32_t void_packets(const VoidRequest &q, uint32_t *bits, VoidLists *lists) {
+struct Shell {
+  double P, r, R, eps;
+  double o[3], lo[3], hi[3];
+};
+bool interior_rect(const View &v, const Shell &g, const Rect &r, double &delta) {
+  const double u = ldexp(1.0, -24);
+  const double ha = 0.5 * (r.a1 - r.a0), hb = 0.5 * (r.b1 - r.b0);
+  const V3 c = v.dir(r.a0 + ha, r.b0 + hb);
+  const double lc = norm(c), h = sqrt(ha * ha * v.uu + hb * hb * v.vv + 2.0 * ha * hb * v.uv), dmin = lc - h;
+  if (!(lc > 0.0) || !(h < 0.16 * lc)) return false;
+  delta = 8.0 * u * (v.m0 + r.a1 * v.mu + r.b1 * v.mv) / dmin + 4e-5;
+  const double ct = dot(c, v.axis) / lc, x = 1.01 * h / dmin + delta + 1e-9;
+  if (!(ct > 0.0) || !(ct <= 1.0)) return false;
+  const double st = sqrt(std::max(0.0, 1.0 - ct * ct));
+  const double cl = ct * (1.0 - 0.5 * x * x) - st * x;
+  if (!(cl > 0.0)) return false;
+  const double P2 = g.P * g.P, gg = g.r * g.r - P2 * (1.0 - cl * cl);
+  if (!(gg >= 4.0 * g.eps * P2)) return false;
+  const double rho = g.eps * P2 / gg;
+  const double eq = 3.1 * u / cl + rho * g.R / (g.P * cl) + 2.0 * u;
+  const double eC = 5.1 * u * P2 / (P2 - g.R * g.R);
+  const double err = eq + eC + 8.0 * u;
+  if (!(err < 0.5)) return false;
+  const V3 cn[4] = {v.dir(r.a0, r.b0), v.dir(r.a1, r.b0), v.dir(r.a0, r.b1), v.dir(r.a1, r.b1)};
+  double cmax = 0.0;
+  for (const V3 &q : cn) cmax = std::max(cmax, norm(q));
+  const double cu = std::min(1.0, ct + st * x);
+  const double sLow = g.P * cu - sqrt(std::max(0.0, g.r * g.r - P2 * (1.0 - cu * cu)));
+  for (int k = 0; k < 3; ++k) {
+    const bool above = g.o[k] > g.hi[k], below = g.o[k] < g.lo[k];
+    if (!above && !below) continue;
+    const double gap = above ? g.o[k] - g.hi[k] : g.lo[k] - g.o[k];
+    const double side = above ? g.hi[k] : -g.lo[k];
+    if (side > g.r) {
+      const double m = (side - g.r) / gap;
+      if ((1.0 + m) * (1.0 - err) > 1.0 + 4.0 * u) continue;
+    }
+    double kmin = INFINITY, kaway = INFINITY;
+    for (const V3 &q : cn) {
+      const double ck = k == 0 ? q.x : k == 1 ? q.y : q.z, toward = above ? -ck : ck;
+      kmin = std::min(kmin, toward);
+      kaway = std::min(kaway, -toward);
+    }
+    if (kaway > delta * cmax * 1.0001 + 2e-5 * cmax) continue;
+    const double wk = kmin / cmax - delta;
+    if (!(wk > 0.0) || !(gap / wk * (1.0 + 4.0 * u) < (1.0 - err) * sLow)) return false;
+  }
+  if (!(dmin > 1e-30) || !(cmax < 1e30) || !(g.P < 1e12) || !(g.P * cl > 1e-20)) return false;
+  return true;
+}
+
+}
+
+uint32_t void_packets(const VoidRequest &q, uint32_t *bits, VoidLists *lists, uint32_t *interior,
+                      uint32_t *numInterior) {
   memset(bits, 0, void_words(q.numTiles) * sizeof(uint32_t));
+  if (interior) memset(interior, 0, void_words(q.numTiles) * sizeof(uint32_t));
+  if (numInterior) *numInterior = 0;
   if (lists) *lists = VoidLists();
   if (q.raygen != IRT_RAYGEN_WITH_ACCEL || q.accelMode != IRT_ACCEL_SPHERE || q.mode != IRT_MODE_USER_GEOM) return 0;
   if (q.W <= 0 || q.H <= 0 || q.tileStride <= 0 || q.tileBegin < 0) return 0;
@@ -97,7 +151,9 @@
   const View v = {org, d00, du, dv, axis, dot(du, du), dot(dv, dv), fabs(dot(du, dv)), abs1(d00), abs1(du), abs1(dv),
                   cos(need), sin(need)};
   const int tilesX = (q.W + 63) / 64, total = tilesX * ((q.H + 63) / 64);
-  uint32_t count = 0;
+  const bool wantInterior = interior != nullptr && r > 0.0;
+  const Shell shell = {P, r, R, eps, {org.x, org.y, org.z}, {q.bmin[0], q.bmin[1], q.bmin[2]}, {q.bmax[0], q.bmax[1], q.bmax[2]}};
+  uint32_t count = 0, countInterior = 0;
   std::vector<uint32_t> res[8], voids;
   auto in_box = [&](double a0, double a1, double b0, double b1, double delta) {
     const double s = T * (delta + 4e-7);
@@ -117,7 +173,10 @@
     double delta = 0.0;
     const Rect tile = {tx0 + 0.5, std::min(tx0 + 64, q.W) + 0.5, ty0 + 0.5, std::min(ty0 + 64, q.H) + 0.5};
     const int whole = sphere_rect(v, tile, delta);
-    if (whole == kAllHit && !lists) continue;
+    if (whole == kAllHit && !lists && !wantInterior) continue;
+    double tdelta = 0.0;
+    const bool tileInterior = wantInterior && (whole == kAllHit || whole == kCentreHits) &&
+                              interior_rect(v, shell, tile, tdelta) && in_box(tile.a0, tile.a1, tile.b0, tile.b1, tdelta);
     const bool tileVoid = whole == kClear && in_box(tile.a0, tile.a1, tile.b0, tile.b1, delta);
     for (int j = 0; j < 64; ++j) {
       const size_t p = (size_t)k * 64 + j;
@@ -125,13 +184,23 @@
       const int x0 = tx0 + (((sub & 3) << 4) | ((wave & 1) << 3)), y0 = ty0 + (((sub >> 2) << 4) | ((wave >> 1) << 3));
       if (x0 >= q.W || y0 >= q.H) continue;
       bool isVoid = tileVoid;
-      if (!tileVoid && whole != kAllHit) {
+      if (!tileVoid && whole != kAllHit && !tileInterior) {
         const Rect r = {x0 + 0.5, std::min(x0 + 8, q.W) + 0.5, y0 + 0.5, std::min(y0 + 8, q.H) + 0.5};
         double pd = 0.0;
         isVoid = !(sphere_rect(v, r, pd) < 0 || pd == 0.0) && sphere_clear(v, r, 0) && in_box(r.a0, r.a1, r.b0, r.b1, pd);
       }
       if (!isVoid) {
         if (lists) res[(p >> 2) & 7].push_back((uint32_t)p);
+        bool isInterior = tileInterior;
+        if (wantInterior && !tileInterior && !tileVoid) {
+          const Rect r = {x0 + 0.5, std::min(x0 + 8, q.W) + 0.5, y0 + 0.5, std::min(y0 + 8, q.H) + 0.5};
+          double pd = 0.0;
+          isInterior = interior_rect(v, shell, r, pd) && in_box(r.a0, r.a1, r.b0, r.b1, pd);
+        }
+        if (isInterior) {
+          interior[p >> 5] |= 1u << (p & 31);
+          ++countInterior;
+        }
         continue;
       }
       bits[p >> 5] |= 1u << (p & 31);
@@ -149,6 +218,7 @@
       for (size_t k = 0; k < res[x].size(); ++k) lists->items[8 * k + x] = res[x][k];
     std::copy(voids.begin(), voids.end(), lists->items.begin() + 8 * len);
   }
+  if (numInterior) *numInterior = countInterior;
   return count;
 }
 
@@ -165,10 +235,12 @@
     keyed = true;
     valid = false;
     count = 0;
+    interiorCount = 0;
     if (defer) return false;
   }
   bits.assign(void_words(q.numTiles), 0u);
-  count = void_packets(q, bits.data(), &lists);
+  interior.assign(void_words(q.numTiles), 0u);
+  count = void_packets(q, bits.data(), &lists, interior.data(), &interiorCount);
   valid = true;
   ++generation;
   return true;
diff --git a/icon-ray-tracing_amd/python/irt.py b/icon-ray-tracing_amd/python/irt.py
--- a/icon-ray-tracing_amd/python/irt.py
+++ b/icon-ray-tracing_amd/python/irt.py
@@ -418,6 +418,7 @@
             v |= 128
         elif ctx.void_use() > 0:
             v |= 16
+            v |= ctx.last_plan()[0] & 64
         return v
     return int(L.irt_debug_default_variant()) & ~4096
 
@@ -672,6 +673,29 @@
     return out
 
 
+def interior_packets(lp: LaunchParams, info: VolumeInfo, w: int, h: int, tile_begin: int = 0,
+                     tile_stride: int = 1, tiles=None, cache: VoidCache = None) -> np.ndarray:
+    L = lib()
+    L.irt_debug_interior_packets.argtypes = [C.c_void_p, C.POINTER(LaunchParams), C.POINTER(VolumeInfo), C.c_int,
+                                             C.c_int, C.c_int, C.c_int, C.c_void_p, C.c_int, C.c_void_p,
+                                             C.c_size_t, C.POINTER(C.c_uint32), C.POINTER(C.c_longlong)]
+    total = num_tiles(w, h)
+    t = None if tiles is None else np.ascontiguousarray(tiles, dtype=np.int32)
+    nt = len(t) if t is not None else (max(0, (total - tile_begin + tile_stride - 1) // tile_stride)
+                                       if tile_begin < total else 0)
+    bits = np.zeros(max(2 * nt, 1), np.uint32)
+    n, comp = C.c_uint32(), C.c_longlong()
+    _check(L.irt_debug_interior_packets(cache._h if cache else None, C.byref(lp), C.byref(info), w, h, tile_begin,
+                                        tile_stride, _ptr(t) if t is not None else None, nt if t is not None else 0,
+                                        _ptr(bits), bits.size, C.byref(n), C.byref(comp)),
+           "irt_debug_interior_packets")
+    if cache:
+        cache.computations = comp.value
+    out = ((bits[:2 * nt, None] >> np.arange(32, dtype=np.uint32)[None, :]) & 1).astype(bool).reshape(-1)
+    assert int(out.sum()) == n.value
+    return out
+
+
 def void_lists(lp: LaunchParams, info: VolumeInfo, w: int, h: int, frames: int, tile_begin: int = 0,
                tile_stride: int = 1, tiles=None, cache: VoidCache = None):
     L = lib()
@@ -886,6 +910,14 @@
         L.irt_debug_void_use.restype = C.c_longlong
         return L.irt_debug_void_use(self._h)
 
+    def interior_use(self) -> int:
+        L = lib()
+        if not hasattr(L, "irt_debug_interior_use"):
+            return 0
+        L.irt_debug_interior_use.argtypes = [C.c_void_p]
+        L.irt_debug_interior_use.restype = C.c_longlong
+        return L.irt_debug_interior_use(self._h)
+
     def last_workgroups(self) -> int:
         L = lib()
         L.irt_debug_last_workgroups.argtypes = [C.c_void_p]
diff --git a/include/icon_rt_hip_debug.h b/include/icon_rt_hip_debug.h
--- a/include/icon_rt_hip_debug.h
+++ b/include/icon_rt_hip_debug.h
@@ -98,6 +98,10 @@
                            int W, int H, int tileBegin, int tileStride, const int32_t *tileList, int listCount,
                            uint32_t *bits, size_t capacity, uint32_t *numVoid, long long *computations);
 long long irt_debug_void_use(const irt_context *ctx);
+int irt_debug_interior_packets(irt_debug_void_cache *cache, const irt_launch_params *lp, const irt_volume_info *info,
+                               int W, int H, int tileBegin, int tileStride, const int32_t *tileList, int listCount,
+                               uint32_t *bits, size_t capacity, uint32_t *numInterior, long long *computations);
+long long irt_debug_interior_use(const irt_context *ctx);
 int irt_debug_void_lists(irt_debug_void_cache *cache, const irt_launch_params *lp, const irt_volume_info *info,
                          int W, int H, int tileBegin, int tileStride, const int32_t *tileList, int listCount,
                          int numFrames, uint32_t *items, size_t capacity, uint32_t *numLive, uint32_t *voidPerRow,
```

Result: faster. 18900 Mray/s, median of 6 (+2.6%).
